# cold-deuu/Quadrotor_Manipulator_MPPI

Measured on AMD Instinct MI355X. Metric: MPPI rollouts/sec (K x H state-steps) + control-step p50 latency, K=4096 H=32, higher is better.
Workload: dtype f32

## Files before the change

quadrotor_manipulator_mppi_amd/csrc/mppi_aql.cpp:

```cpp
#include "mppi_aql.h"

#include <dlfcn.h>
#include <hip/hip_runtime.h>
#include <hsa/hsa.h>
#include <hsa/hsa_ext_amd.h>
#include <immintrin.h>
#include <stdio.h>
#include <stdlib.h>
#include <string.h>

#include <algorithm>
#include <atomic>
#include <chrono>
#include <map>
#include <mutex>
#include <unordered_map>
#include <vector>

namespace {

thread_local mppi::LaunchDesc* t_capture = nullptr;

struct Kern {
    uint64_t obj = 0;
// ... 36 lines not shown
    if (hsa_amd_memory_pool_get_info(pool, HSA_AMD_MEMORY_POOL_INFO_SEGMENT, &seg) != HSA_STATUS_SUCCESS ||
        seg != HSA_AMD_SEGMENT_GLOBAL)
        return HSA_STATUS_SUCCESS;
    if (hsa_amd_memory_pool_get_info(pool, HSA_AMD_MEMORY_POOL_INFO_GLOBAL_FLAGS, &flags) != HSA_STATUS_SUCCESS ||
        hsa_amd_memory_pool_get_info(pool, HSA_AMD_MEMORY_POOL_INFO_RUNTIME_ALLOC_ALLOWED, &alloc) != HSA_STATUS_SUCCESS ||
        !alloc)
        return HSA_STATUS_SUCCESS;
    if (hsa_amd_agent_memory_pool_get_info(pk->cpu, pool, HSA_AMD_AGENT_MEMORY_POOL_INFO_ACCESS, &acc) !=
            HSA_STATUS_SUCCESS || acc == HSA_AMD_MEMORY_POOL_ACCESS_NEVER_ALLOWED)
        return HSA_STATUS_SUCCESS;
    const int rank = (flags & HSA_AMD_MEMORY_POOL_GLOBAL_FLAG_KERNARG_INIT) ? 3
                     : (flags & HSA_AMD_MEMORY_POOL_GLOBAL_FLAG_FINE_GRAINED) ? 2 : 1;
    if (rank > pk->best_rank) { pk->best_rank = rank; pk->pool = pool; }
    return HSA_STATUS_SUCCESS;
}
std::mutex g_mu;
std::map<int, Device> g_dev;

const char* const kUnits[] = {"mppi_rollout_drone", "mppi_rollout_arm", "mppi_rollout_arm_h32", "mppi_rollout_arm32",
                              "mppi_rollout_wb",
                              "mppi_rollout_quad", "mppi_finalize"};

std::string hsa_msg(hsa_status_t s) {
    const char* m = nullptr;
    if (hsa_status_string(s, &m) != HSA_STATUS_SUCCESS || !m) return "HSA status " + std::to_string((int)s);
    return m;
}

struct AgentMatch {
    uint32_t domain, bdf;
    bool found;
    hsa_agent_t agent;
};
hsa_status_t match_agent(hsa_agent_t a, void* data) {
    auto* m = (AgentMatch*)data;
    hsa_device_type_t t;
    if (hsa_agent_get_info(a, HSA_AGENT_INFO_DEVICE, &t) != HSA_STATUS_SUCCESS || t != HSA_DEVICE_TYPE_GPU)
        return HSA_STATUS_SUCCESS;
    uint32_t bdf = 0, dom = 0;
    if (hsa_agent_get_info(a, (hsa_agent_info_t)HSA_AMD_AGENT_INFO_BDFID, &bdf) != HSA_STATUS_SUCCESS) return HSA_STATUS_SUCCESS;
    if (hsa_agent_get_info(a, (hsa_agent_info_t)HSA_AMD_AGENT_INFO_DOMAIN, &dom) != HSA_STATUS_SUCCESS) dom = 0;
    if (bdf == m->bdf && dom == m->domain && !m->found) { m->agent = a; m->found = true; }
    return HSA_STATUS_SUCCESS;
}

bool library_stem(std::string* stem) {
    Dl_info info;
    if (!dladdr((void*)&match_agent, &info) || !info.dli_fname) return false;
    std::string p = info.dli_fname;
    if (p.size() > 3 && p.compare(p.size() - 3, 3, ".so") == 0) p.resize(p.size() - 3);
    *stem = p;
    return true;
}

bool read_file(const std::string& path, std::vector<char>* out) {
    FILE* f = fopen(path.c_str(), "rb");
    if (!f) return false;
    char buf[1 << 16];
    size_t r;
    while ((r = fread(buf, 1, sizeof buf, f)) > 0) out->insert(out->end(), buf, buf + r);
    fclose(f);
    return !out->empty();
}

Device* device_for(int ordinal) {
    Device& d = g_dev[ordinal];
    if (d.tried) return &d;
    d.tried = true;
    char bus[64] = {0};
    unsigned dom = 0, b = 0, dv = 0, fn = 0;
    if (hipDeviceGetPCIBusId(bus, (int)sizeof bus, ordinal) != hipSuccess ||
        sscanf(bus, "%x:%x:%x.%x", &dom, &b, &dv, &fn) != 4) {
        d.why = "no PCI bus id for HIP device " + std::to_string(ordinal);
        return &d;
    }
    hsa_status_t st = hsa_init();
    if (st != HSA_STATUS_SUCCESS) { d.why = "hsa_init: " + hsa_msg(st); return &d; }
    AgentMatch m{dom, (b << 8) | (dv << 3) | fn, false, {}};
    hsa_iterate_agents(match_agent, &m);
    if (!m.found) { d.why = std::string("no HSA agent at ") + bus; return &d; }
    d.agent = m.agent;
    std::string stem;
    if (!library_stem(&stem)) { d.why = "cannot locate the library's own path"; return &d; }
    for (const char* u : kUnits) {
        const std::string path = stem + "." + u + ".co";
        std::vector<char> co;
        if (!read_file(path, &co)) { d.why = "missing code object " + path + " (python -m quadrotor_manipulator_mppi_amd.build)"; return &d; }
        hsa_code_object_reader_t rd;
        hsa_executable_t ex;
        if ((st = hsa_code_object_reader_create_from_memory(co.data(), co.size(), &rd)) != HSA_STATUS_SUCCESS ||
            (st = hsa_executable_create_alt(HSA_PROFILE_FULL, HSA_DEFAULT_FLOAT_ROUNDING_MODE_DEFAULT, nullptr, &ex)) !=
                HSA_STATUS_SUCCESS) {
            d.why = "loading " + path + ": " + hsa_msg(st);
            return &d;
        }
        static std::vector<std::vector<char>> keep;
        keep.push_back(std::move(co));
        if ((st = hsa_executable_load_agent_code_object(ex, d.agent, rd, nullptr, nullptr)) != HSA_STATUS_SUCCESS ||
            (st = hsa_executable_freeze(ex, nullptr)) != HSA_STATUS_SUCCESS) {
            d.why = "loading " + path + ": " + hsa_msg(st);
            return &d;
        }
        d.exes.push_back(ex);
    }
    hsa_agent_t cpu{};
    if (hsa_iterate_agents(first_cpu, &cpu) == HSA_STATUS_INFO_BREAK && !getenv("MPPI_AQL_CALL_HOSTMEM")) {
        PoolPick pk{cpu, 0, {}};
        hsa_amd_agent_iterate_memory_pools(d.agent, pick_pool, &pk);
        if (pk.best_rank > 0 &&
            hsa_agent_get_info(d.agent, (hsa_agent_info_t)HSA_AMD_AGENT_INFO_HDP_FLUSH, &d.hdp) == HSA_STATUS_SUCCESS &&
            d.hdp.HDP_MEM_FLUSH_CNTL) {
            d.vis_pool_ok = true;
            d.vis_pool = pk.pool;
            d.cpu = cpu;
            d.vis_pool_kind = pk.best_rank == 3 ? "device kernarg pool" : pk.best_rank == 2 ? "device fine-grained"
                                                                                             : "device coarse-grained";
        }
    }
    d.ok = true;
    return &d;
}

bool lookup(Device* d, const char* name, Kern* k, std::string* err) {
    std::string sym = std::string(name) + ".kd";
    auto it = d->syms.find(sym);
    if (it != d->syms.end()) { *k = it->second; return true; }
    for (hsa_executable_t ex : d->exes) {
        hsa_executable_symbol_t s;
        if (hsa_executable_get_symbol_by_name(ex, sym.c_str(), &d->agent, &s) != HSA_STATUS_SUCCESS) continue;
        Kern r;
        if (hsa_executable_symbol_get_info(s, HSA_EXECUTABLE_SYMBOL_INFO_KERNEL_OBJECT, &r.obj) != HSA_STATUS_SUCCESS ||
            hsa_executable_symbol_get_info(s, HSA_EXECUTABLE_SYMBOL_INFO_KERNEL_KERNARG_SEGMENT_SIZE, &r.kas) != HSA_STATUS_SUCCESS ||
            hsa_executable_symbol_get_info(s, HSA_EXECUTABLE_SYMBOL_INFO_KERNEL_GROUP_SEGMENT_SIZE, &r.gss) != HSA_STATUS_SUCCESS ||
            hsa_executable_symbol_get_info(s, HSA_EXECUTABLE_SYMBOL_INFO_KERNEL_PRIVATE_SEGMENT_SIZE, &r.pss) != HSA_STATUS_SUCCESS)
            break;
        d->syms[sym] = r;
        *k = r;
        return true;
    }
    *err = "kernel " + sym + " not in the code objects";
    return false;
}

}

extern "C" mppi::LaunchDesc* mppi_capture_target(void) { return t_capture; }

namespace mppi_aql {

constexpr uint32_t kQueueSize = 4096;
constexpr size_t kArgSlot = 4096;
constexpr uint32_t kCallSlots = 16;
constexpr uint32_t kBatchSlots = 4;
constexpr uint32_t kBatchBlocks = 3;

struct Step {
    Device* dev = nullptr;
    hsa_queue_t* q = nullptr;
    hsa_signal_t done{0};
    std::atomic<int> qerr{0};
    unsigned char* d_args = nullptr;
    uint32_t batch_slot = 0;
    unsigned char* h_call = nullptr;
    unsigned char* h_call_dev = nullptr;
    bool call_vis = false;
    uint32_t call_slot = 0;
    mppi::LaunchDesc fin_call{};
    Kern kc_r, kc_f;
    bool call_valid = false;
    bool call_unread = false;
    mppi::LaunchDesc roll{}, fin{};
    mppi::LaunchDesc fin_quiet{};
    Kern kr, kf, kfq;
    uint32_t step_off = 0, step_word = 0;
    bool valid = false;
    int64_t outstanding = 0;
    unsigned char* d_touch = nullptr;
    Kern kt;
    std::recursive_mutex mu;
};

void set_capture(mppi::LaunchDesc* d) { t_capture = d; }

static void queue_error(hsa_status_t status, hsa_queue_t*, void* data) {
    ((Step*)data)->qerr.store((int)status);
}

static bool probe_dispatch_ids(Step* s, std::string* why);

Step* step_create(int device, std::string* why) {
    Device* d = nullptr;
    {
        std::lock_guard<std::mutex> lk(g_mu);
        d = device_for(device);
        if (!d->ok) { *why = d->why; return nullptr; }
    }
    Step* s = new Step();
    s->dev = d;
    hsa_status_t st = hsa_queue_create(d->agent, kQueueSize, HSA_QUEUE_TYPE_SINGLE, queue_error, s, UINT32_MAX,
                                       UINT32_MAX, &s->q);
    if (st != HSA_STATUS_SUCCESS) { *why = "hsa_queue_create: " + hsa_msg(st); delete s; return nullptr; }
    if ((st = hsa_signal_create(0, 0, nullptr, &s->done)) != HSA_STATUS_SUCCESS) {
        *why = "hsa_signal_create: " + hsa_msg(st);
        hsa_queue_destroy(s->q);
        delete s;
        return nullptr;
    }
    if (d->vis_pool_ok) {
        void* p = nullptr;
        if (hsa_amd_memory_pool_allocate(d->vis_pool, kCallSlots * kArgSlot, 0, &p) == HSA_STATUS_SUCCESS) {
            if (hsa_amd_agents_allow_access(1, &d->cpu, nullptr, p) == HSA_STATUS_SUCCESS) {
                s->h_call = s->h_call_dev = (unsigned char*)p;
                s->call_vis = true;
            } else {
                hsa_amd_memory_pool_free(p);
            }
        }
    }
    if (hipMalloc(&s->d_args, (1 + kBatchBlocks * kBatchSlots) * kArgSlot) != hipSuccess ||
        (!s->call_vis &&
         (hipHostMalloc((void**)&s->h_call, kCallSlots * kArgSlot, hipHostMallocMapped | hipHostMallocCoherent) != hipSuccess ||
          hipHostGetDevicePointer((void**)&s->h_call_dev, s->h_call, 0) != hipSuccess))) {
        *why = "allocating the argument blocks failed";
        if (s->d_args) (void)hipFree(s->d_args);
        if (s->h_call) { if (s->call_vis) hsa_amd_memory_pool_free(s->h_call); else (void)hipHostFree(s->h_call); }
        hsa_signal_destroy(s->done);
        hsa_queue_destroy(s->q);
        delete s;
        return nullptr;
    }
    if (!probe_dispatch_ids(s, why)) {
        if (!step_destroy(s)) *why += " (and the probe's queue did not drain)";
        return nullptr;
    }
    {
        std::lock_guard<std::mutex> lk(g_mu);
        if (!lookup(s->dev, "k_dispatch_probe", &s->kt, why)) { (void)step_destroy(s); return nullptr; }
    }
    unsigned char h[128] = {};
    if (hipMalloc(&s->d_touch, 3 * 64) != hipSuccess) {
        s->d_touch = nullptr;
        *why = "touch buffer";
        (void)step_destroy(s);
        return nullptr;
    }
    unsigned char* outs[2] = {s->d_touch + 128, s->d_touch + 136};
    memcpy(h, &outs[0], 8);
    memcpy(h + 64, &outs[1], 8);
    if (hipMemcpy(s->d_touch, h, sizeof h, hipMemcpyHostToDevice) != hipSuccess) {
        *why = "touch upload";
        (void)step_destroy(s);
        return nullptr;
    }
    return s;
}

bool step_destroy(Step* s) {
    if (!s) return true;
    std::string e;
    if (s->outstanding && step_wait(s, 60000, &e) != 0) {
        hsa_queue_inactivate(s->q);
        fprintf(stderr, "[mppi aql] queue did not drain at destroy (%s): its buffers are leaked\n", e.c_str());
        return false;
    }
    hsa_signal_destroy(s->done);
    hsa_queue_destroy(s->q);
    (void)hipFree(s->d_args);
    if (s->d_touch) (void)hipFree(s->d_touch);
    if (s->call_vis) hsa_amd_memory_pool_free(s->h_call); else (void)hipHostFree(s->h_call);
    delete s;
    return true;
}

bool step_busy(Step* s) {
    if (!s) return false;
    std::lock_guard<std::recursive_mutex> qlk(s->mu);
    return s->outstanding > 0;
}

static bool check_launch(const mppi::LaunchDesc& l, const Kern& k, std::string* err) {
    if (k.kas < l.arg_bytes || k.kas - l.arg_bytes >= 16 || k.kas > kArgSlot) {
        *err = std::string(l.symbol) + ": kernel-argument segment " + std::to_string(k.kas) + " B vs " +
               std::to_string(l.arg_bytes) + " B packed";
        return false;
    }
    if (k.gss + l.lds > 160 * 1024) { *err = std::string(l.symbol) + ": LDS over 160 KB"; return false; }
    for (int i = 0; i < 3; ++i)
        if (l.grid[i] == 0 || l.block[i] == 0) { *err = std::string(l.symbol) + ": empty grid"; return false; }
    if ((uint64_t)l.block[0] * l.block[1] * l.block[2] > 1024) { *err = "block over 1024 threads"; return false; }
    return true;
}

static bool same_launch(const mppi::LaunchDesc& a, const mppi::LaunchDesc& b, uint32_t skip_off) {
    if (strcmp(a.symbol, b.symbol) != 0 || memcmp(a.grid, b.grid, sizeof a.grid) != 0 ||
        memcmp(a.block, b.block, sizeof a.block) != 0 || a.lds != b.lds || a.arg_bytes != b.arg_bytes)
        return false;
    if (skip_off >= a.arg_bytes || a.arg_bytes - skip_off < 4) return memcmp(a.args, b.args, a.arg_bytes) == 0;
    return memcmp(a.args, b.args, skip_off) == 0 &&
           memcmp(a.args + skip_off + 4, b.args + skip_off + 4, a.arg_bytes - skip_off - 4) == 0;
}

static unsigned char* batch_args(Step* s) { return s->d_args + (1 + kBatchBlocks * (size_t)s->batch_slot) * kArgSlot; }

int step_prepare(Step* s, const mppi::LaunchDesc& roll, const mppi::LaunchDesc& fin, const mppi::LaunchDesc& fin_quiet,
                 uint32_t step, uint32_t step_off, std::string* err) {
    std::lock_guard<std::recursive_mutex> qlk(s->mu);
    const uint32_t word = step - (uint32_t)(hsa_queue_load_write_index_relaxed(s->q) >> 1);
    if (s->valid && s->step_word == word && s->step_off == step_off && same_launch(roll, s->roll, step_off) &&
        same_launch(fin, s->fin, ~0u) && same_launch(fin_quiet, s->fin_quiet, ~0u))
        return 0;
    if (getenv("MPPI_AQL_PROFILE") && s->valid) {
        int first = -1;
        for (uint32_t i = 0; i < roll.arg_bytes && i < s->roll.arg_bytes; ++i)
            if ((i < step_off || i >= step_off + 4) && roll.args[i] != s->roll.args[i]) { first = (int)i; break; }
        int ffirst = -1;
        for (uint32_t i = 0; i < fin.arg_bytes && i < s->fin.arg_bytes; ++i)
            if (fin.args[i] != s->fin.args[i]) { ffirst = (int)i; break; }
        fprintf(stderr, "[mppi aql] re-upload: word %u vs %u, rollout args differ at %d, finalize at %d, sym %d/%d\n", word,
                s->step_word, first, ffirst, strcmp(roll.symbol, s->roll.symbol), strcmp(fin.symbol, s->fin.symbol));
    }
    Kern kr, kf, kfq;
    {
        std::lock_guard<std::mutex> lk(g_mu);
        if (!lookup(s->dev, roll.symbol, &kr, err) || !lookup(s->dev, fin.symbol, &kf, err) ||
            !lookup(s->dev, fin_quiet.symbol, &kfq, err))
            return -2;
    }
    if (!check_launch(roll, kr, err) || !check_launch(fin, kf, err) || !check_launch(fin_quiet, kfq, err)) return -2;
    if (step_off + 4 > roll.arg_bytes) { *err = "step counter outside the rollout's arguments"; return -2; }
    if (s->outstanding && step_wait(s, 60000, err) != 0) return -1;
    std::vector<unsigned char> h(kBatchBlocks * kArgSlot, 0);
    memcpy(h.data(), roll.args, roll.arg_bytes);
    memcpy(h.data() + step_off, &word, 4);
    memcpy(h.data() + kArgSlot, fin.args, fin.arg_bytes);
    memcpy(h.data() + 2 * kArgSlot, fin_quiet.args, fin_quiet.arg_bytes);
    s->batch_slot = (s->batch_slot + 1) % kBatchSlots;
    if (hipMemcpy(batch_args(s), h.data(), h.size(), hipMemcpyHostToDevice) != hipSuccess) {
        *err = "uploading the argument blocks failed";
        s->valid = false;
        return -1;
    }
    s->roll = roll;
    s->fin = fin;
    s->fin_quiet = fin_quiet;
    s->kr = kr;
    s->kf = kf;
    s->kfq = kfq;
    s->step_off = step_off;
    s->step_word = word;
    s->valid = true;
    return 0;
}

static int g_fence[4] = {-1, -1, -1, -1};
static void load_fences() {
    if (g_fence[0] >= 0) return;
    const char* f = getenv("MPPI_AQL_FENCES");
    const char* def = "0000";
    for (int i = 0; i < 4; ++i) g_fence[i] = (f && strlen(f) == 4 && f[i] >= '0' && f[i] <= '2') ? f[i] - '0' : def[i] - '0';
}
static const int kScope[3] = {HSA_FENCE_SCOPE_NONE, HSA_FENCE_SCOPE_AGENT, HSA_FENCE_SCOPE_SYSTEM};

static inline void put(hsa_queue_t* q, const Kern& k, const mppi::LaunchDesc& l, void* args, hsa_signal_t sig,
                       int acquire, int release, bool barrier = true) {
    const uint64_t idx = hsa_queue_add_write_index_relaxed(q, 1);
    while (idx - hsa_queue_load_read_index_scacquire(q) >= q->size) _mm_pause();
    auto* p = (hsa_kernel_dispatch_packet_t*)q->base_address + (idx & (q->size - 1));
    p->workgroup_size_x = (uint16_t)l.block[0];
    p->workgroup_size_y = (uint16_t)l.block[1];
    p->workgroup_size_z = (uint16_t)l.block[2];
    p->reserved0 = 0;
    p->grid_size_x = l.grid[0] * l.block[0];
    p->grid_size_y = l.grid[1] * l.block[1];
    p->grid_size_z = l.grid[2] * l.block[2];
    p->private_segment_size = k.pss;
    p->group_segment_size = k.gss + l.lds;
    p->kernel_object = k.obj;
    p->kernarg_address = args;
    p->reserved2 = 0;
    p->completion_signal = sig;
    const uint16_t header =
        (uint16_t)((HSA_PACKET_TYPE_KERNEL_DISPATCH << HSA_PACKET_HEADER_TYPE) | ((barrier ? 1 : 0) << HSA_PACKET_HEADER_BARRIER) |
                   (kScope[acquire] << HSA_PACKET_HEADER_SCACQUIRE_FENCE_SCOPE) |
                   (kScope[release] << HSA_PACKET_HEADER_SCRELEASE_FENCE_SCOPE));
    const uint32_t setup = 3u << HSA_KERNEL_DISPATCH_PACKET_SETUP_DIMENSIONS;
    __atomic_store_n((uint32_t*)p, (uint32_t)header | (setup << 16), __ATOMIC_RELEASE);
}

static bool probe_dispatch_ids(Step* s, std::string* why) {
    Kern k;
    {
        std::lock_guard<std::mutex> lk(g_mu);
        if (!lookup(s->dev, "k_dispatch_probe", &k, why)) return false;
    }
    unsigned long long* d_ids = nullptr;
    if (hipMalloc(&d_ids, 2 * sizeof(unsigned long long)) != hipSuccess) { *why = "probe buffer"; return false; }
    unsigned long long* args[2] = {d_ids, d_ids + 1};
    std::vector<unsigned char> h(2 * kArgSlot, 0);
    memcpy(h.data(), &args[0], 8);
    memcpy(h.data() + kArgSlot, &args[1], 8);
    bool ok = hipMemset(d_ids, 0xFF, 2 * sizeof(unsigned long long)) == hipSuccess &&
              hipMemcpy(s->d_args + kArgSlot, h.data(), h.size(), hipMemcpyHostToDevice) == hipSuccess;
    if (!ok) { (void)hipFree(d_ids); *why = "probe upload"; return false; }
    mppi::LaunchDesc l{};
    snprintf(l.symbol, sizeof l.symbol, "k_dispatch_probe");
    l.grid[0] = l.grid[1] = l.grid[2] = 1;
    l.block[0] = 64; l.block[1] = l.block[2] = 1;
    l.arg_bytes = 8;
    uint64_t idx[2];
    hsa_signal_add_relaxed(s->done, 1);
    ++s->outstanding;
    for (int i = 0; i < 2; ++i) {
        idx[i] = hsa_queue_load_write_index_relaxed(s->q);
        put(s->q, k, l, s->d_args + (1 + i) * kArgSlot, i == 1 ? s->done : hsa_signal_t{0}, 2, i == 1 ? 2 : 0);
    }
    hsa_signal_store_screlease(s->q->doorbell_signal, (hsa_signal_value_t)idx[1]);
    std::string err;
    unsigned long long got[2] = {~0ull, ~0ull};
    if (step_wait(s, 10000, &err) != 0) {
        char b[160];
        snprintf(b, sizeof b, " [signal %ld, read index %llu, write index %llu]", (long)hsa_signal_load_relaxed(s->done),
                 (unsigned long long)hsa_queue_load_read_index_relaxed(s->q),
                 (unsigned long long)hsa_queue_load_write_index_relaxed(s->q));
        *why = "dispatch-id probe: " + err + b;
        return false;
    }
    ok = hipMemcpy(got, d_ids, sizeof got, hipMemcpyDeviceToHost) == hipSuccess;
    (void)hipFree(d_ids);
    if (!ok) { *why = "dispatch-id probe readback"; return false; }
    if (const char* sk = getenv("MPPI_AQL_PROBE_SKEW")) {
        got[0] += (unsigned long long)atoll(sk);
        got[1] += (unsigned long long)atoll(sk);
    }
    if (got[0] != idx[0] || got[1] != idx[1]) {
        char b[256];
        snprintf(b, sizeof b, "the queue's dispatch ids (%llu, %llu) are not its packet indices (%llu, %llu): "
                 "intercepted by a tool", got[0], got[1], (unsigned long long)idx[0], (unsigned long long)idx[1]);
        *why = b;
        return false;
    }
    return true;
}

std::unique_lock<std::recursive_mutex> step_guard(Step* s) { return std::unique_lock<std::recursive_mutex>(s->mu); }

int step_dispatch(Step* s, int n, std::string* err, bool overlap) {
    std::lock_guard<std::recursive_mutex> qlk(s->mu);
    if (!s->valid) { *err = "step_dispatch before step_prepare"; return -1; }
    if (n <= 0) return 0;
    if (s->qerr.load()) { *err = "native queue error: " + hsa_msg((hsa_status_t)s->qerr.load()); return -1; }
    hsa_signal_add_relaxed(s->done, 1);
    ++s->outstanding;
    const hsa_signal_t none{0};
    void* ra = batch_args(s);
    void* fa = batch_args(s) + kArgSlot;
    void* fqa = batch_args(s) + 2 * kArgSlot;
    load_fences();
    for (int i = 0; i < n; ++i) {
        const bool last = i == n - 1;
        put(s->q, s->kr, s->roll, ra, none, i == 0 ? std::max(1, g_fence[0]) : g_fence[0], g_fence[1],
            !(overlap && i > 0));
        if (last) put(s->q, s->kf, s->fin, fa, s->done, g_fence[2], 2);
        else put(s->q, s->kfq, s->fin_quiet, fqa, none, g_fence[2], g_fence[3]);
        hsa_signal_store_screlease(s->q->doorbell_signal, (hsa_signal_value_t)hsa_queue_load_write_index_relaxed(s->q) - 1);
    }
    return 0;
}

int step_call(Step* s, const mppi::LaunchDesc& roll, const mppi::LaunchDesc& fin, uint32_t step,
              uint32_t step_off, uint32_t seq_off, uint32_t* seq, std::string* err) {
    std::lock_guard<std::recursive_mutex> qlk(s->mu);
    if (s->qerr.load()) { *err = "native queue error: " + hsa_msg((hsa_status_t)s->qerr.load()); return -1; }
    static const bool prof = getenv("MPPI_AQL_PROFILE") != nullptr;
    static double pacc[4] = {0, 0, 0, 0};
    static long pcn = 0;
    auto now = [] { return std::chrono::steady_clock::now(); };
    const auto p0 = now();
    Kern kr, kf;
    {
        std::lock_guard<std::mutex> lk(g_mu);
        if (!lookup(s->dev, roll.symbol, &kr, err) || !lookup(s->dev, fin.symbol, &kf, err)) return -2;
    }
    if (!check_launch(roll, kr, err) || !check_launch(fin, kf, err)) return -2;
    if (step_off + 4 > roll.arg_bytes || seq_off + 4 > roll.arg_bytes) { *err = "call words outside the arguments"; return -2; }
    if (s->call_unread && s->outstanding && step_wait(s, 60000, err) != 0) return -1;
    if (!s->call_valid || !same_launch(fin, s->fin_call, ~0u)) {
        if (s->outstanding && step_wait(s, 60000, err) != 0) return -1;
        std::vector<unsigned char> h(kArgSlot, 0);
        memcpy(h.data(), fin.args, fin.arg_bytes);
        if (hipMemcpy(s->d_args, h.data(), kArgSlot, hipMemcpyHostToDevice) != hipSuccess) {
            *err = "uploading the call's finalize arguments failed";
            s->call_valid = false;
            return -1;
        }
        s->fin_call = fin;
        s->call_valid = true;
    }
    s->kc_r = kr;
    s->kc_f = kf;
    const uint64_t r = hsa_queue_load_write_index_relaxed(s->q);
    const uint32_t word = step - (uint32_t)(r >> 1);
    *seq = 0x80000000u | (uint32_t)(r >> 1);
    const uint32_t slot = s->call_slot++ % kCallSlots;
    unsigned char* blk = s->h_call + (size_t)slot * kArgSlot;
    alignas(16) unsigned char tmp[kArgSlot];
    memcpy(tmp, roll.args, roll.arg_bytes);
    memcpy(tmp + step_off, &word, 4);
    memcpy(tmp + seq_off, seq, 4);
    const uint32_t nb = (roll.arg_bytes + 63) & ~63u;
    memset(tmp + roll.arg_bytes, 0, nb - roll.arg_bytes);
    const auto p1 = now();
    memcpy(blk, tmp, nb);
    const auto p2 = now();
    if (s->call_vis) {
        _mm_sfence();
        volatile uint32_t* f = s->dev->hdp.HDP_MEM_FLUSH_CNTL;
        *f = 1u;
        (void)*f;
    }
    std::atomic_thread_fence(std::memory_order_release);
    const auto p3 = now();
    hsa_signal_add_relaxed(s->done, 1);
    ++s->outstanding;
    s->call_unread = true;
    const hsa_signal_t none{0};
    load_fences();
    put(s->q, kr, roll, s->h_call_dev + (size_t)slot * kArgSlot, none, std::max(1, g_fence[0]), g_fence[1]);
    put(s->q, kf, fin, s->d_args, s->done, g_fence[2], 2);
    hsa_signal_store_screlease(s->q->doorbell_signal, (hsa_signal_value_t)hsa_queue_load_write_index_relaxed(s->q) - 1);
    if (prof) {
        const auto p4 = now();
        pacc[0] += std::chrono::duration<double, std::micro>(p1 - p0).count();
        pacc[1] += std::chrono::duration<double, std::micro>(p2 - p1).count();
        pacc[2] += std::chrono::duration<double, std::micro>(p3 - p2).count();
        pacc[3] += std::chrono::duration<double, std::micro>(p4 - p3).count();
        if (++pcn % 1000 == 0)
            fprintf(stderr, "[mppi aql] step_call (us): lookups+checks %.2f  block write %.2f  flush+readback %.2f  packets %.2f\n",
                    pacc[0] / pcn, pacc[1] / pcn, pacc[2] / pcn, pacc[3] / pcn);
    }
    return 0;
}

int step_touch(Step* s, bool if_free, std::string* err) {
    std::unique_lock<std::recursive_mutex> qlk(s->mu, std::defer_lock);
    if (if_free) {
        if (!qlk.try_lock()) return 1;
    } else {
        qlk.lock();
    }
    if (s->qerr.load()) { *err = "native queue error: " + hsa_msg((hsa_status_t)s->qerr.load()); return -1; }
    mppi::LaunchDesc l{};
    l.grid[0] = l.grid[1] = l.grid[2] = 1;
    l.block[0] = 64; l.block[1] = l.block[2] = 1;
    l.arg_bytes = 8;
    hsa_signal_add_relaxed(s->done, 1);
    ++s->outstanding;
    put(s->q, s->kt, l, s->d_touch, hsa_signal_t{0}, 1, 0);
    put(s->q, s->kt, l, s->d_touch + 64, s->done, 0, 0);
    hsa_signal_store_screlease(s->q->doorbell_signal, (hsa_signal_value_t)hsa_queue_load_write_index_relaxed(s->q) - 1);
    return 0;
}

void step_ring(Step* s) {
    const uint64_t w = hsa_queue_load_write_index_relaxed(s->q);
    if (w) hsa_signal_store_screlease(s->q->doorbell_signal, (hsa_signal_value_t)(w - 1));
}

int step_error(Step* s) { return s ? s->qerr.load() : 0; }

const char* step_call_memory(Step* s) {
    return !s ? "" : s->call_vis ? s->dev->vis_pool_kind.c_str() : "pinned host memory";
}

void step_call_read(Step* s) {
    if (!s) return;
    std::lock_guard<std::recursive_mutex> qlk(s->mu);
    s->call_unread = false;
}

int step_wait(Step* s, int timeout_ms, std::string* err) {
    if (!s) return 0;
    std::lock_guard<std::recursive_mutex> qlk(s->mu);
    if (!s->outstanding) return 0;
    const auto t0 = std::chrono::steady_clock::now();
    for (;;) {
        if (hsa_signal_load_scacquire(s->done) == 0) break;
        if (s->qerr.load()) {
            *err = "native queue error: " + hsa_msg((hsa_status_t)s->qerr.load());
            return -1;
        }
        if (std::chrono::steady_clock::now() - t0 > std::chrono::milliseconds(timeout_ms)) {
            *err = "native dispatch: no completion after " + std::to_string(timeout_ms) + " ms";
            return -1;
        }
        _mm_pause();
    }
    s->outstanding = 0;
    s->call_unread = false;
    return 0;
}

}
```

quadrotor_manipulator_mppi_amd/csrc/mppi_aql.h:

```cpp
#pragma once
#include <stdint.h>

#include <mutex>
#include <string>

#include "mppi_dev.h"

namespace mppi_aql {

struct Step;

Step* step_create(int device, std::string* why);
bool step_destroy(Step* s);

int step_prepare(Step* s, const mppi::LaunchDesc& roll, const mppi::LaunchDesc& fin, const mppi::LaunchDesc& fin_quiet,
                 uint32_t step, uint32_t step_off, std::string* err);
int step_dispatch(Step* s, int n, std::string* err, bool overlap = false);
std::unique_lock<std::recursive_mutex> step_guard(Step* s);
int step_call(Step* s, const mppi::LaunchDesc& roll, const mppi::LaunchDesc& fin, uint32_t step,
              uint32_t step_off, uint32_t seq_off, uint32_t* seq, std::string* err);
void step_call_read(Step* s);
const char* step_call_memory(Step* s);
int step_touch(Step* s, bool if_free, std::string* err);
void step_ring(Step* s);
int step_error(Step* s);
int step_wait(Step* s, int timeout_ms, std::string* err);
bool step_busy(Step* s);

void set_capture(mppi::LaunchDesc* d);

}
```

quadrotor_manipulator_mppi_amd/csrc/mppi_dev.h:

```cpp
#pragma once
#include <stddef.h>
#include <stdint.h>

#include "../../include/mppi_hip.h"

namespace mppi {

constexpr int kMaxA = MPPI_MAX_ACTION;
constexpr int kMaxJ = MPPI_MAX_JOINTS;
constexpr int kMaxW = MPPI_MAX_SAVGOL;
constexpr int kHdr = 4;
constexpr int kMaxCostRun = 4096;
constexpr inline int cost_run_stride(int nS) { return (nS + 3) & ~3; }

struct JointDev {
    int32_t type;
    int32_t q_index;
    int32_t axis_z;
    int32_t _pad;
    float O[12];
    float ax[3];
    float axx[9];
};

struct VehicleConst {
    double pos0[kMaxA];
    double vel0[kMaxA];
    float pos0f[kMaxA];
    float vel0f[kMaxA];
    float base[12];
    float tpos[3];
    float tR[9];
    float _pad[4];
    float qc[kMaxJ];
    float qlo[kMaxJ];
    float qhi[kMaxJ];
};
static_assert(sizeof(VehicleConst) % 16 == 0, "VehicleConst must be a 16-byte multiple");

struct KinOrigin { int p[3]; int s[3]; int tmask; };
constexpr KinOrigin kKinova[7] = {
    {{0, 1, 2}, {-1, 1, -1}, 4},
    {{0, 2, 1}, {-1, -1, -1}, 6},
    {{0, 2, 1}, {1, -1, 1}, 2},
    {{0, 2, 1}, {-1, 1, 1}, 4},
    {{0, 2, 1}, {-1, -1, -1}, 6},
    {{0, 2, 1}, {-1, 1, 1}, 4},
    {{0, 2, 1}, {-1, -1, -1}, 2},
};

struct DevParams {
    int32_t model, V, K, H, A;
    int32_t L;
    int32_t R;
    int32_t nch;
    int32_t nb;
    int32_t iters;
    int32_t nq;
    int32_t qoff;
    int32_t nj;
    int32_t noise_mode, state_f64, store_traj, store_noise;
    int32_t sigma_diag;
    int32_t j0;
    int32_t chain_fast;
    int32_t P;
    int32_t C;
    int32_t hp;
    uint32_t seed_lo, seed_hi;
    int64_t k_offset;
    float dt, dt2;
    double dt_d;
    float coef;
    float w_sp, w_so, w_tp, w_to;
    float sdiag[kMaxA];
    VehicleConst vc0;
    const JointDev* joints;
    const float* sigma;
    const VehicleConst* vc;
    const float* u_prev;
    const float* noise_in;
    uint32_t step_ctr;
    float* traj;
    float* noise_out;
    float* S;
    float* hdr;
    float* rdata;
    unsigned long long* stamps;
    int32_t cost_terms;
    float w_cov;
    float w_cen, w_jt, w_act, lim_pen;
    const float* sinv;
    const float* gamma_t;
    const float* jtraj;
    float q_inv_m;
    float q_iinv[3];
    float q_kd;
    float q_g;
    int32_t q_literal_jinv;
    const uint32_t* ovl;
    int32_t ovl_n;
    int32_t kern;
};
constexpr int kStamps = 16;

struct FinTail {
    float coef, dt, dt2;
    int32_t mode, model, qoff, nq, state_f64, out_dim, window;
    float* u_prev;
    const VehicleConst* vc;
    double* out;
    float* u0;
    float* stats;
    uint32_t* flags;
    float* wraw;
    float* wsmooth;
    float* dst;
    float* xbase;
    int64_t xslot;
    int32_t nslots, myslot, P, pad_;
    unsigned long long* const* xpeers;
    unsigned long long* xlocal;
    int32_t xn, xme;
    uint32_t* xerr;
    uint32_t* xstall;
    uint32_t* xovl;
    unsigned long long* xdec;
    float sg[kMaxW];
};
enum { kTailFinal = 0, kTailPack = 1, kTailScratch = 2, kTailReadback = 3, kTailSlots = 4 };

constexpr int kMaxPeers = 8;
constexpr int kXW = kHdr + 64;
constexpr int kXCtl = 16;
constexpr uint32_t kDecCommit = 1u;
constexpr uint64_t kDecGraceTicks = 10000ull;
constexpr int kVcStepWord = (int)(offsetof(VehicleConst, _pad) / 4) + 1;
constexpr int kVcEpochWord = kVcStepWord + 1;
constexpr uint32_t kTagValid = 0x80000000u;
constexpr inline uint32_t peer_tag(uint32_t step, uint32_t epoch) {
    return kTagValid | ((epoch & 0x3FFu) << 20) | (step & 0xFFFFFu);
}
constexpr uint64_t kPeerWaitTicks = 200000000ull;
constexpr uint32_t kSeqFromVc = 0xFFFFFFFFu;

struct LaunchDesc {
    char symbol[192];
    uint32_t grid[3];
    uint32_t block[3];
    uint32_t lds;
    uint32_t arg_bytes;
    alignas(16) unsigned char args[2048];
};

constexpr int32_t kFinKernGeneric = 1, kFinKernQuiet = 2;

struct FinParams {
    int32_t model, V, H, A, nq, qoff, state_f64;
    int32_t nrec;
    int32_t ts, tsz;
    const float* hdr;
    int64_t hdr_vs, hdr_rs;
    const float* dat;
    int64_t d_vs, d_as, d_rs;
    int32_t P;
    int32_t mode;
    int32_t window, half;
    float coef, dt, dt2;
    double dt_d;
    float sg[kMaxW];
    float* dst;
    float* xbase;
    int64_t xslot;
    int32_t nslots, myslot;
    unsigned long long* const* xpeers;
    unsigned long long* xlocal;
    int32_t xn, xme;
    uint32_t* xerr;
    uint32_t* xstall;
    uint32_t* xovl;
    unsigned long long* xdec;
    float* u_prev;
    const VehicleConst* vc;
    double* out;
    float* u0;
    float* stats;
    uint32_t* flags;
    uint32_t seq;
    float* wraw;
    float* wsmooth;
    int32_t out_dim;
    int32_t dbg;
    int32_t kern;
    unsigned long long* stamps;
    const FinTail* tail;
};

}

extern "C" {
int mppi_launch_rollout(const mppi::DevParams* p, int block_threads, void* stream);
int mppi_launch_rollout_arm64(const mppi::DevParams* p, int block_threads, void* stream);
int mppi_launch_rollout_arm64_h32(const mppi::DevParams* p, int block_threads, void* stream);
int mppi_launch_rollout_arm32(const mppi::DevParams* p, int block_threads, void* stream);
int mppi_launch_rollout_wb(const mppi::DevParams* p, int block_threads, void* stream);
int mppi_launch_rollout_quad(const mppi::DevParams* p, int block_threads, void* stream);
int mppi_launch_finalize(const mppi::FinParams* p, void* stream);
int mppi_launch_peer_probe(unsigned long long* const* peers, unsigned long long* local, int n, int me,
                           unsigned long long slot_words, uint32_t tag, unsigned long long ticks,
                           unsigned long long* out, void* stream);
int mppi_launch_weights(const float* S, const float* stats, float* w, int V, int K, float coef,
                        void* stream);
int mppi_launch_philox(uint64_t seed, uint32_t step, int vehicle, int64_t k0, int K, int H, int A,
                       float* z, uint32_t* raw, void* stream);
mppi::LaunchDesc* mppi_capture_target(void);
}
```

quadrotor_manipulator_mppi_amd/csrc/mppi_engine.cpp:

```cpp
#include <algorithm>
#include <cmath>
#include <cstdio>
#include <cstdlib>
#include <cstring>
#include <vector>

#include "mppi_engine.h"

using namespace mppi;

namespace mppi_host {

FinTail tail_of(const FinParams& f, int32_t mode) {
    FinTail t;
    std::memset(&t, 0, sizeof(t));
    t.coef = f.coef; t.dt = f.dt; t.dt2 = f.dt2;
    t.mode = mode; t.model = f.model; t.qoff = f.qoff; t.nq = f.nq; t.state_f64 = f.state_f64;
    t.out_dim = f.out_dim; t.window = f.window;
    t.u_prev = f.u_prev; t.vc = f.vc;
    t.out = f.out; t.u0 = f.u0; t.stats = f.stats; t.flags = f.flags; t.wraw = f.wraw; t.wsmooth = f.wsmooth;
    t.dst = f.dst; t.xbase = f.xbase; t.xslot = f.xslot; t.nslots = f.nslots; t.myslot = f.myslot; t.P = f.P;
    t.xpeers = f.xpeers; t.xlocal = f.xlocal; t.xn = f.xn; t.xme = f.xme; t.xerr = f.xerr;
    t.xstall = f.xstall; t.xovl = f.xovl; t.xdec = f.xdec;
    std::memcpy(t.sg, f.sg, sizeof(t.sg));
// ... 247 lines not shown
    CREATE_TRY(hipEventCreateWithFlags(&e->ev_vc, hipEventDisableTiming));
    CREATE_TRY(hipEventCreateWithFlags(&e->ev_out, hipEventDisableTiming));
    const size_t KH = (size_t)e->V * e->K * H;
    CREATE_TRY(hipMalloc(&e->d_joints, sizeof(JointDev) * kMaxJ));
    CREATE_TRY(hipMalloc(&e->d_vc, sizeof(VehicleConst) * e->V));
    CREATE_TRY(hipMalloc(&e->d_u_prev, sizeof(float) * e->V * H * e->A));
    CREATE_TRY(hipMalloc(&e->d_S, sizeof(float) * e->V * e->K));
    CREATE_TRY(hipMalloc(&e->d_w, sizeof(float) * e->V * e->K));
    CREATE_TRY(hipMalloc(&e->d_hdr, sizeof(float) * (size_t)e->V * nb * 4));
    CREATE_TRY(hipMalloc(&e->d_rdata, sizeof(float) * (size_t)e->V * e->A * nb * H));
    CREATE_TRY(hipMalloc(&e->d_wraw, sizeof(float) * e->V * H * e->A));
    CREATE_TRY(hipMalloc(&e->d_wsmooth, sizeof(float) * e->V * H * e->A));
    if (c.store_trajectory) CREATE_TRY(hipMalloc(&e->d_traj, sizeof(float) * traj_floats(e)));
    if (c.store_noise) CREATE_TRY(hipMalloc(&e->d_noise_out, sizeof(float) * KH * e->A));
    e->out_bytes = (int64_t)(off_xerr(e) + 16);
    CREATE_TRY(hipMalloc(&e->d_out, e->out_bytes));
    CREATE_TRY(hipHostMalloc((void**)&e->h_out, e->out_bytes, hipHostMallocMapped | hipHostMallocCoherent));
    CREATE_TRY(hipHostGetDevicePointer((void**)&e->h_out_dev, e->h_out, 0));
    std::memset(e->h_out, 0, e->out_bytes);
    CREATE_TRY(hipMalloc(&e->d_sigma, sizeof(float) * kMaxA * kMaxA));
    CREATE_TRY(hipMemcpy(e->d_sigma, c.sigma, sizeof(float) * e->A * e->A, hipMemcpyHostToDevice));
    if (c.cost_terms) {
        std::vector<double> m(e->A * 2 * e->A, 0.0);
        const int A = e->A, W2 = 2 * A;
        for (int i = 0; i < A; ++i) {
            for (int j = 0; j < A; ++j) m[i * W2 + j] = c.sigma[i * A + j];
            m[i * W2 + A + i] = 1.0;
        }
        for (int col = 0; col < A; ++col) {
            int piv = col;
            for (int r = col + 1; r < A; ++r)
                if (std::fabs(m[r * W2 + col]) > std::fabs(m[piv * W2 + col])) piv = r;
            if (std::fabs(m[piv * W2 + col]) < 1e-30) { mppi_destroy(e); return fail(MPPI_ERR_INVALID_ARG, "Sigma is singular"); }
            for (int j = 0; j < W2; ++j) std::swap(m[col * W2 + j], m[piv * W2 + j]);
            const double d = m[col * W2 + col];
            for (int j = 0; j < W2; ++j) m[col * W2 + j] /= d;
            for (int r = 0; r < A; ++r)
                if (r != col) {
                    const double f2 = m[r * W2 + col];
                    for (int j = 0; j < W2; ++j) m[r * W2 + j] -= f2 * m[col * W2 + j];
                }
        }
        std::vector<float> sinv(A * A), gam(H);
        for (int i = 0; i < A; ++i)
            for (int j = 0; j < A; ++j) sinv[i * A + j] = (float)m[i * W2 + A + j];
        for (int t = 0; t < H; ++t) gam[t] = std::pow(c.cost_gamma, (float)t);
        CREATE_TRY(hipMalloc(&e->d_sinv, sizeof(float) * A * A));
        CREATE_TRY(hipMalloc(&e->d_gamma, sizeof(float) * H));
        CREATE_TRY(hipMalloc(&e->d_jtraj, sizeof(float) * (size_t)e->V * H * std::max(1, e->nq)));
        CREATE_TRY(hipMemcpy(e->d_sinv, sinv.data(), sizeof(float) * A * A, hipMemcpyHostToDevice));
        CREATE_TRY(hipMemcpy(e->d_gamma, gam.data(), sizeof(float) * H, hipMemcpyHostToDevice));
        CREATE_TRY(hipMemset(e->d_jtraj, 0, sizeof(float) * (size_t)e->V * H * std::max(1, e->nq)));
    }
    CREATE_TRY(hipHostMalloc((void**)&e->h_vc, sizeof(VehicleConst) * e->V, hipHostMallocDefault));
    CREATE_TRY(hipMemsetAsync(e->d_u_prev, 0, sizeof(float) * e->V * H * e->A, e->stream));
    CREATE_TRY(hipMemsetAsync(e->d_out, 0, e->out_bytes, e->stream));

    std::vector<JointDev> jd(kMaxJ);
    for (int j = 0; j < c.n_joints; ++j) bake_joint(c.joints[j], jd[j]);
    const float I12[12] = {1, 0, 0, 0, 0, 1, 0, 0, 0, 0, 1, 0};
    std::memcpy(e->fixedM, I12, sizeof(I12));
    int j0 = 0;
    while (c.model != MPPI_MODEL_DRONE && j0 < c.n_joints && jd[j0].type == MPPI_JOINT_FIXED) {
        mul34(e->fixedM, jd[j0].O, e->fixedM);
        ++j0;
    }
    CREATE_TRY(hipMemcpy(e->d_joints, jd.data(), sizeof(JointDev) * kMaxJ, hipMemcpyHostToDevice));
    CREATE_TRY(hipStreamSynchronize(e->stream));
#undef CREATE_TRY

    DevParams& p = e->dp;
    std::memset(&p, 0, sizeof(p));
    p.model = c.model; p.V = e->V; p.K = e->K; p.H = H; p.A = e->A;
    p.L = L; p.R = R; p.nch = nch; p.nb = nb; p.iters = iters;
    p.nq = e->nq; p.qoff = e->qoff; p.nj = c.n_joints;
    p.noise_mode = c.noise_mode | (c.vehicle_offset << 16); p.state_f64 = c.state_f64;
    p.store_traj = c.store_trajectory; p.store_noise = c.store_noise;
    bool diag = true;
    for (int a = 0; a < e->A; ++a)
        for (int b = 0; b < e->A; ++b) {
            if (a == b) p.sdiag[a] = c.sigma[a * e->A + b];
            else if (c.sigma[a * e->A + b] != 0.0f) diag = false;
        }
    p.sigma_diag = diag;
    p.sigma = e->d_sigma;
    p.j0 = j0;
    {
        bool fast = c.model != MPPI_MODEL_DRONE && (c.n_joints - j0) == e->nq;
        for (int j = j0; fast && j < c.n_joints; ++j)
            fast = jd[j].type == MPPI_JOINT_REVOLUTE && jd[j].axis_z && jd[j].q_index == j - j0;
        p.chain_fast = fast;
        if (fast && e->nq == 7 && c.n_joints - j0 == 7) {
            bool kin = true;
            for (int j = 0; kin && j < 7; ++j) {
                const float* O = jd[j0 + j].O;
                const KinOrigin& k = kKinova[j];
                for (int col = 0; kin && col < 3; ++col)
                    for (int row = 0; kin && row < 3; ++row) {
                        const float want = (row == k.p[col]) ? (float)k.s[col] : 0.0f;
                        kin = std::fabs(O[4 * row + col] - want) <= 1e-6f;
                    }
                for (int d = 0; kin && d < 3; ++d) kin = ((k.tmask >> d) & 1) ? true : (O[4 * d + 3] == 0.0f);
            }
            if (kin && !getenv("MPPI_NO_KINOVA_PATH")) p.chain_fast = 2;
        }
    }
    p.P = P; p.C = e->C; p.hp = traj_pitch(e);
    p.seed_lo = (uint32_t)c.seed; p.seed_hi = (uint32_t)(c.seed >> 32);
    p.k_offset = (int64_t)c.shard_rank * e->K;
    p.dt = (float)c.dt; p.dt2 = (float)(c.dt * c.dt); p.dt_d = c.dt;
    p.coef = (float)(-1.0 / c.lambda_);
    p.w_sp = c.w_stage_pos; p.w_so = c.w_stage_ori; p.w_tp = c.w_term_pos; p.w_to = c.w_term_ori;
    p.joints = e->d_joints;
    p.cost_terms = c.cost_terms;
    p.w_cov = (float)((double)c.w_covar * (c.lambda_ * (1.0 - (double)c.cost_alpha)));
    p.w_cen = c.w_center; p.w_jt = c.w_joint_track; p.w_act = c.w_action; p.lim_pen = c.joint_limit_penalty;
    p.sinv = e->d_sinv; p.gamma_t = e->d_gamma; p.jtraj = e->d_jtraj;
    p.q_inv_m = (float)(1.0 / (double)c.quad_mass);
    for (int d = 0; d < 3; ++d) p.q_iinv[d] = (float)(1.0 / (double)c.quad_inertia[d]);
    p.q_kd = c.quad_kd; p.q_g = c.quad_gravity; p.q_literal_jinv = c.quad_literal_jinv ? 1 : 0;
    p.vc = e->d_vc; p.u_prev = e->d_u_prev;
    p.traj = e->d_traj; p.noise_out = e->d_noise_out; p.S = e->d_S; p.hdr = e->d_hdr; p.rdata = e->d_rdata;
#ifdef MPPI_STAMPS
    if (getenv("MPPI_STAMPS")) {
        const size_t nwaves = (size_t)e->V * nb * (e->threads / 64);
        if (hipMalloc(&e->d_stamps, nwaves * kStamps * 8) == hipSuccess) p.stamps = e->d_stamps;
        e->stamp_sum.assign(kStamps, 0.0);
        (void)hipMalloc(&e->d_fstamps, 2 * (size_t)e->V * e->A * ((H + 7) / 8) * kStamps * 8);
        e->fstamp_sum.assign(kStamps, 0.0);
    }
#endif

    FinParams& f = e->fp;
    std::memset(&f, 0, sizeof(f));
    f.model = c.model; f.V = e->V; f.H = H; f.A = e->A; f.nq = e->nq; f.qoff = e->qoff;
    f.state_f64 = c.state_f64; f.P = P;
    if (const char* z = getenv("MPPI_FIN_TSZ")) {
        const int tz = atoi(z);
        if (tz >= 1 && tz + 2 * (c.savgol_window / 2) <= 64) e->fin_tsz = tz;
    }
    f.tsz = e->fin_tsz; f.ts = e->fin_ts = (H + e->fin_tsz - 1) / e->fin_tsz;
    f.window = c.savgol_window; f.half = c.savgol_window / 2;
    for (int j = 0; j < c.savgol_window; ++j) f.sg[j] = e->sg_taps[c.savgol_window - 1 - j];
    f.coef = p.coef; f.dt = p.dt; f.dt2 = p.dt2; f.dt_d = c.dt;
    f.u_prev = e->d_u_prev; f.vc = e->d_vc;
    f.out = (double*)e->h_out_dev;
    f.u0 = (float*)(e->h_out_dev + off_u0(e));
    f.stats = (float*)(e->h_out_dev + off_stats(e));
    f.flags = (uint32_t*)(e->h_out_dev + off_flags(e));
    f.xerr = (uint32_t*)(e->h_out_dev + off_xerr(e));
    f.wraw = e->d_wraw; f.wsmooth = e->d_wsmooth; f.out_dim = e->out_dim;
    if (const char* dbg = getenv("MPPI_FIN_DEBUG")) f.dbg = atoi(dbg);
    if (const char* g = getenv("MPPI_GENERIC_KERNELS"))
        e->generic = !strcmp(g, "finalize") ? 1 : !strcmp(g, "quiet") ? 2 : !strcmp(g, "rollout") ? 4 : atoi(g) != 0 ? 7 : 0;
    f.kern = (e->generic & 1) ? kFinKernGeneric : 0;
    p.kern = (e->generic & 4) ? 1 : 0;
    e->event_wait = getenv("MPPI_EVENT_WAIT") && atoi(getenv("MPPI_EVENT_WAIT")) != 0;
    e->no_flag_dbg = e->event_wait && getenv("MPPI_DEBUG_NO_FLAG") && atoi(getenv("MPPI_DEBUG_NO_FLAG")) != 0;
    e->out_dbg = getenv("MPPI_DEBUG_OUT") ? atoi(getenv("MPPI_DEBUG_OUT")) : 0;
    if (const char* d = getenv("MPPI_DISPATCH")) e->aql_mode = !strcmp(d, "hip") ? 0 : !strcmp(d, "aql") ? 1 : 2;
    f.stamps = e->d_fstamps;
    e->overlap = getenv("MPPI_OVERLAP") && atoi(getenv("MPPI_OVERLAP")) != 0 && c.model != MPPI_MODEL_QUADROTOR;
    if (e->overlap) {
        const size_t n = (size_t)e->V * e->A * e->fin_ts;
        if (hipMalloc(&e->d_ovl, n * sizeof(uint32_t)) != hipSuccess || hipMemset(e->d_ovl, 0, n * sizeof(uint32_t)) != hipSuccess) {
            fail(MPPI_ERR_HIP, "overlap counters");
            mppi_destroy(e);
            return MPPI_ERR_HIP;
        }
        f.xovl = e->d_ovl;
        p.ovl = e->d_ovl;
        p.ovl_n = e->A * e->fin_ts;
    }
    {
        FinTail t[kTailSlots];
        t[kTailFinal] = tail_of(f, 0);
        t[kTailPack] = tail_of(f, 1);
        t[kTailScratch] = tail_of(f, 0);
        t[kTailScratch].out = (double*)e->d_out;
        t[kTailScratch].u0 = (float*)(e->d_out + off_u0(e));
        t[kTailScratch].stats = (float*)(e->d_out + off_stats(e));
        t[kTailScratch].flags = (uint32_t*)(e->d_out + off_flags(e));
        t[kTailScratch].xerr = (uint32_t*)(e->d_out + off_xerr(e));
        t[kTailScratch].wraw = nullptr;
        t[kTailScratch].wsmooth = nullptr;
        t[kTailFinal].wraw = nullptr;
        t[kTailFinal].wsmooth = nullptr;
        t[kTailReadback] = tail_of(f, 2);
        hipError_t te = hipMalloc(&e->d_tail, sizeof(t));
        if (te == hipSuccess) te = hipMemcpy(e->d_tail, t, sizeof(t), hipMemcpyHostToDevice);
        if (te != hipSuccess) {
            fail(MPPI_ERR_HIP, "finalize tail parameters: %s", hipGetErrorString(te));
            mppi_destroy(e);
            return MPPI_ERR_HIP;
        }
        f.tail = e->d_tail + kTailFinal;
    }
    *out = e;
    return MPPI_OK;
}

void mppi_destroy(mppi_engine* e) {
    if (!e) return;
    prewarm_stop(e);
    (void)hipSetDevice(e->cfg.device);
    if (e->aql && !mppi_aql::step_destroy(e->aql)) {
        fprintf(stderr, "[mppi] mppi_destroy: the engine's native queue did not drain; its device buffers are leaked\n");
        return;
    }
    e->aql = nullptr;
    if (e->d_stamps && e->stamp_n) {
        fprintf(stderr, "[mppi stamps] rollout avg cycles per wave over %lld waves:", (long long)e->stamp_n);
        for (size_t i = 1; i < kRollStampOrder.size(); ++i)
            fprintf(stderr, " %s=%.0f", kRollStampNames[i], e->stamp_sum[i] / e->stamp_n);
        fprintf(stderr, "\n[mppi stamps] finalize avg cycles per block over %lld blocks:", (long long)e->fstamp_n);
        for (size_t i = 1; i < kFinStampOrder.size(); ++i)
            fprintf(stderr, " %s=%.0f", kFinStampNames[i], e->fstamp_sum[i] / std::max<int64_t>(1, e->fstamp_n));
        fprintf(stderr, "\n");
    }
    if (e->stream) (void)hipStreamSynchronize(e->stream);
    for (auto& pr : e->roll_pairs) { (void)hipEventDestroy(pr.first); (void)hipEventDestroy(pr.second); }
    for (auto& pr : e->fin_pairs) { (void)hipEventDestroy(pr.first); (void)hipEventDestroy(pr.second); }
    for (auto ev : e->ev_pool) (void)hipEventDestroy(ev);
    exchange_release(e);
    void* dev[] = {e->d_xregion, e->d_xpeers, e->d_sigma, e->d_joints, e->d_vc, e->d_u_prev, e->d_noise_in, e->d_traj, e->d_noise_out,
                   e->d_S, e->d_hdr, e->d_rdata, e->d_out, e->d_wraw, e->d_wsmooth, e->d_w,
                   e->d_sinv, e->d_gamma, e->d_jtraj, e->d_xown, e->d_tail, e->d_stamps, e->d_fstamps, e->d_xstall, e->d_ovl, e->d_xdec};
    for (void* p : dev) if (p) (void)hipFree(p);
    if (e->h_out) (void)hipHostFree(e->h_out);
    if (e->h_vc) (void)hipHostFree(e->h_vc);
    if (e->ev_vc) (void)hipEventDestroy(e->ev_vc);
    if (e->ev_out) (void)hipEventDestroy(e->ev_out);
    if (e->own_stream) (void)hipStreamDestroy(e->own_stream);
    delete e;
}

mppi_status mppi_set_stream(mppi_engine* e, void* s) {
    if (!e) return fail(MPPI_ERR_INVALID_ARG, "null engine");
    if (use_device(e)) return MPPI_ERR_HIP;
    HIP_TRY(hipStreamSynchronize(e->stream));
    e->stream = s ? (hipStream_t)s : e->own_stream;
    return MPPI_OK;
}

mppi_status mppi_set_joint_trajectory(mppi_engine* e, int32_t v, const float* traj) {
    if (!e || v < 0 || v >= e->V) return fail(MPPI_ERR_INVALID_ARG, "mppi_set_joint_trajectory: bad arguments");
    if (!e->d_jtraj) return fail(MPPI_ERR_STATE, "engine created without cost_terms");
    if (use_device(e)) return MPPI_ERR_HIP;
    const size_t n = (size_t)e->H * e->nq;
    float* dst = e->d_jtraj + (size_t)v * n;
    if (traj) HIP_TRY(hipMemcpyAsync(dst, traj, n * sizeof(float), hipMemcpyHostToDevice, e->stream));
    else HIP_TRY(hipMemsetAsync(dst, 0, n * sizeof(float), e->stream));
    HIP_TRY(hipStreamSynchronize(e->stream));
    return MPPI_OK;
}

mppi_status mppi_set_target(mppi_engine* e, int32_t v, const float* pos, const float* quat) {
    if (!e || !pos || v < 0 || v >= e->V) return fail(MPPI_ERR_INVALID_ARG, "mppi_set_target: bad arguments");
    std::memcpy(&e->tpos[3 * v], pos, 3 * sizeof(float));
    if (quat) std::memcpy(&e->tquat[4 * v], quat, 4 * sizeof(float));
    if (e->state_set) {
        if (use_device(e)) return MPPI_ERR_HIP;
        return upload_consts(e);
    }
    return MPPI_OK;
}

mppi_status mppi_set_u_prev(mppi_engine* e, const float* u) {
    if (!e || !u) return fail(MPPI_ERR_INVALID_ARG, "null argument");
    if (use_device(e)) return MPPI_ERR_HIP;
    HIP_TRY(hipMemcpyAsync(e->d_u_prev, u, sizeof(float) * e->V * e->H * e->A, hipMemcpyHostToDevice, e->stream));
    HIP_TRY(hipStreamSynchronize(e->stream));
    return MPPI_OK;
}

mppi_status mppi_get_u_prev(mppi_engine* e, float* u) {
    if (!e || !u) return fail(MPPI_ERR_INVALID_ARG, "null argument");
    if (use_device(e)) return MPPI_ERR_HIP;
    HIP_TRY(hipMemcpyAsync(u, e->d_u_prev, sizeof(float) * e->V * e->H * e->A, hipMemcpyDeviceToHost, e->stream));
    HIP_TRY(hipStreamSynchronize(e->stream));
    return MPPI_OK;
}

mppi_status mppi_set_state(mppi_engine* e, const double* state) {
    if (!e || !state) return fail(MPPI_ERR_INVALID_ARG, "null argument");
    if (use_device(e)) return MPPI_ERR_HIP;
    std::memcpy(e->state.data(), state, sizeof(double) * e->state.size());
    e->state_set = true;
    return upload_consts(e);
}

mppi_status mppi_set_step_counter(mppi_engine* e, uint32_t step) {
    if (!e) return fail(MPPI_ERR_INVALID_ARG, "null engine");
    if (use_device(e)) return MPPI_ERR_HIP;
    e->step_ctr = step;
    if (e->peer) {
        ++e->x_epoch;
        return build_vehicle_consts(e);
    }
    return MPPI_OK;
}

mppi_status mppi_get_step_counter(mppi_engine* e, uint32_t* step) {
    if (!e || !step) return fail(MPPI_ERR_INVALID_ARG, "null argument");
    *step = e->step_ctr;
    return MPPI_OK;
}

mppi_status mppi_kernel_timing_ex(mppi_engine* e, int32_t n, double* rollout_us, double* finalize_us,
// ... 222 lines not shown
```

quadrotor_manipulator_mppi_amd/csrc/mppi_engine.h:

```cpp
#pragma once
#include <hip/hip_runtime.h>
#include <rccl/rccl.h>

#include <atomic>
#include <condition_variable>
#include <mutex>
#include <string>
#include <thread>
#include <utility>
#include <vector>

#include "mppi_aql.h"
#include "mppi_dev.h"

struct mppi_engine {
    mppi_config cfg;
    int K, H, A, V, nq, qoff, state_dim, out_dim, C, threads;
    int64_t out_bytes;
    mppi::DevParams dp;
    mppi::FinParams fp;
    float sg_taps[mppi::kMaxW];
    float fixedM[12];
    hipStream_t own_stream = nullptr, stream = nullptr;
    float* d_sigma = nullptr;
    mppi::JointDev* d_joints = nullptr;
    mppi::VehicleConst* d_vc = nullptr;
    float* d_u_prev = nullptr;
    float* d_noise_in = nullptr;
    uint32_t step_ctr = 0;
    uint32_t out_seq = 0;
    bool call_cached = false;
    int call_threads = 0;
    mppi::DevParams call_p{};
    mppi::FinParams call_f{};
    mppi::LaunchDesc call_roll{}, call_fin{};
    bool batch_cached = false;
    int batch_threads = 0;
    mppi::DevParams batch_p{};
    mppi::FinParams batch_f{};
    mppi::LaunchDesc batch_roll{}, batch_fin{};
    mppi::LaunchDesc batch_fin_quiet{};
    int generic = 0;
    std::string kern_batch = "none", kern_call = "none";
    int kern_batch_state = 0;
    bool kern_call_hip = false, kern_call_peer = false;
    std::vector<double> rec_out;
    std::vector<float> rec_u0, rec_stats;
    std::vector<float> fk_O, fk_ax;
    uint32_t seq_ctr = 0;
    bool event_wait = false;
    bool no_flag_dbg = false;
    int out_dbg = 0;
    float* d_traj = nullptr;
    float* d_noise_out = nullptr;
    float* d_S = nullptr;
    float* d_hdr = nullptr;
    float* d_rdata = nullptr;
    int fin_ts = 1, fin_tsz = 8;
    unsigned char* d_out = nullptr;
    mppi::FinTail* d_tail = nullptr;
    float* d_wraw = nullptr;
    float* d_wsmooth = nullptr;
    float* d_w = nullptr;
    float* d_sinv = nullptr;
    float* d_gamma = nullptr;
    float* d_jtraj = nullptr;
    float* d_exchange = nullptr;
    ncclComm_t comm = nullptr;
    float* d_xown = nullptr;
    bool peer = false;
    int x_connected = 0;
    unsigned long long* d_xregion = nullptr;
    size_t x_bytes = 0;
    std::vector<void*> x_opened;
    unsigned long long** d_xpeers = nullptr;
    uint32_t x_epoch = 0;
    uint32_t* d_xstall = nullptr;
    unsigned long long* d_xdec = nullptr;
    bool overlap = false;
    uint32_t* d_ovl = nullptr;
    mppi::VehicleConst* h_vc = nullptr;
    unsigned char* h_out = nullptr;
    unsigned char* h_out_dev = nullptr;
    hipEvent_t ev_vc = nullptr, ev_out = nullptr;
    bool vc_pending = false, state_set = false, out_pending = false;
    std::vector<float> tpos, tquat;
    std::vector<double> state;
    bool timing = false;
    std::vector<hipEvent_t> ev_pool;
    std::vector<std::pair<hipEvent_t, hipEvent_t>> roll_pairs, fin_pairs;
    double roll_ms = 0.0, fin_ms = 0.0;
    unsigned long long* d_stamps = nullptr;
    unsigned long long* d_fstamps = nullptr;
    std::vector<double> fstamp_sum;
    int64_t fstamp_n = 0;
    std::vector<double> stamp_sum;
    int64_t stamp_n = 0;
    double clk_sum = 0.0;
    int64_t roll_n = 0, fin_n = 0;
    mppi_aql::Step* aql = nullptr;
    int aql_mode = 2;
    bool aql_tried = false;
    bool aql_off = false;
    std::string aql_why = "no mppi_run_steps yet";
    bool aql_out = false;
    bool aql_call = false;
    bool calls_native = false;
    double call_wait_us = 0.0;
    std::thread pw_thr;
    std::mutex pw_mu;
    std::condition_variable pw_cv;
    std::atomic<int32_t> pw_us{0};
    std::atomic<bool> pw_stop{false};
    std::atomic<int64_t> pw_touches{0};
    std::atomic<int64_t> call_t[8];
    std::atomic<int64_t> call_n{0};
    bool pw_spin = false;
    std::atomic<bool> pw_native{false};
};

namespace mppi_host {

mppi_status fail(mppi_status st, const char* fmt, ...) __attribute__((format(printf, 2, 3)));

#define HIP_TRY(expr)                                                                              \
    do {                                                                                           \
        hipError_t _e = (expr);                                                                    \
        if (_e != hipSuccess)                                                                      \
            return ::mppi_host::fail(MPPI_ERR_HIP, "%s failed: %s (%s:%d)", #expr,                \
                                     hipGetErrorString(_e), __FILE__, __LINE__);                   \
    } while (0)

int nq_of(const mppi_config& c);
mppi_status validate(const mppi_config& c);
void rpy_to_R(float r, float p, float y, float* R);
void joint_origin(const mppi_joint& j, float* T16);
void unit_axis(const mppi_joint& j, float* a);
void base_from_xyzquat(const double* b, bool f64, float* T16);
void quat_xyzw_to_R(const float* q, float* R);
void euler_zyx(const float* m, float* ypr);
int savgol_taps(int window, int order, float* c);
void bake_joint(const mppi_joint& j, mppi::JointDev& d);
void mul34(const float* A, const float* B, float* C);
void fk_consts(const mppi_joint* joints, int nj, float* O16s, float* axes);
void host_fk_c(const mppi_joint* joints, int nj, const float* O16s, const float* axes, const double* q,
               const double* xyzquat, bool f64, float* out16);
void host_fk(const mppi_joint* joints, int nj, const double* q, const double* xyzquat, bool f64, float* out16);

inline bool sharded(const mppi_engine* e) { return (e->cfg.shard_count > 1 || e->comm) && !e->peer; }
mppi::FinTail tail_of(const mppi::FinParams& f, int32_t mode);
void pack_fields(const mppi_engine* e, mppi::FinParams& f);
mppi_status upload_pack_tail(mppi_engine* e);
int traj_pitch(const mppi_engine* e);
size_t traj_floats(const mppi_engine* e);
mppi_status aql_join(mppi_engine* e);
mppi_status use_device(mppi_engine* e);
mppi_status build_vehicle_consts(mppi_engine* e);
void quad_outputs(const mppi_engine* e, const double* s, const float* u0, double* out);
mppi_status upload_consts(mppi_engine* e);
hipEvent_t pool_event(mppi_engine* e);
mppi_status drain_timing(mppi_engine* e);

inline size_t off_u0(const mppi_engine* e) { return ((size_t)e->V * e->out_dim * sizeof(double) + 15) & ~size_t(15); }
inline size_t off_stats(const mppi_engine* e) {
    return (off_u0(e) + (size_t)e->V * e->A * sizeof(float) + 15) & ~size_t(15);
}
inline size_t off_flags(const mppi_engine* e) { return off_stats(e) + (size_t)e->V * 16; }
inline size_t rec_count(const mppi_engine* e) { return (size_t)e->V * (2 * e->A + 1); }
inline size_t off_xerr(const mppi_engine* e) { return off_flags(e) + rec_count(e) * 16; }
inline uint32_t sticky_timeout(const mppi_engine* e) {
    return e->h_out ? *(const volatile uint32_t*)(e->h_out + off_xerr(e)) : 0u;
}
inline unsigned long long* xdata(const mppi_engine* e) { return e->d_xregion + mppi::kXCtl; }

void block_records(const mppi_engine* e, mppi::FinParams& f);
void final_records(const mppi_engine* e, mppi::FinParams& f);

struct Rccl {
    bool ok = false;
    std::string why;
    ncclResult_t (*get_unique_id)(ncclUniqueId*) = nullptr;
    ncclResult_t (*init_rank)(ncclComm_t*, int, ncclUniqueId, int) = nullptr;
    ncclResult_t (*all_reduce)(const void*, void*, size_t, ncclDataType_t, ncclRedOp_t, ncclComm_t,
                               hipStream_t) = nullptr;
    ncclResult_t (*destroy)(ncclComm_t) = nullptr;
    const char* (*err)(ncclResult_t) = nullptr;
    ncclResult_t (*init_rank_config)(ncclComm_t*, int, ncclUniqueId, int, ncclConfig_t*) = nullptr;
    ncclResult_t (*async_error)(ncclComm_t, ncclResult_t*) = nullptr;
    ncclResult_t (*abort)(ncclComm_t) = nullptr;
    ncclResult_t (*count)(const ncclComm_t, int*) = nullptr;
    ncclResult_t (*user_rank)(const ncclComm_t, int*) = nullptr;
};
const Rccl& rccl();
void exchange_release(mppi_engine* e);
// ... 15 lines not shown
```

quadrotor_manipulator_mppi_amd/csrc/mppi_rollout.h:

```cpp
#pragma once
#include "mppi_device.h"

#ifndef MPPI_KO
#define MPPI_KO 0
#endif
#ifndef MPPI_ROLL_OCC_NCH2
#define MPPI_ROLL_OCC_NCH2 4
#endif
#ifndef MPPI_ROLL_OCC_NCH2_XC
#define MPPI_ROLL_OCC_NCH2_XC 2
#endif
#ifndef MPPI_ROLL_OCC_XC
#define MPPI_ROLL_OCC_XC 4
#endif
#ifndef MPPI_ROLL_OCC
#define MPPI_ROLL_OCC 4
#endif
#ifndef MPPI_PRIO
#define MPPI_PRIO 1
#endif
#ifndef MPPI_S_PLAIN
#define MPPI_S_PLAIN 0
#endif
#ifndef MPPI_EPS_STASH
// ... 320 lines not shown
#define STAMP(i) do { } while (0)
#define STAMPW(i) do { } while (0)
#define STAMPRT(i) do { } while (0)
#endif

#ifdef MPPI_SECTIONS
#define SECTION(name)                                        \
    do {                                                     \
        __builtin_amdgcn_sched_barrier(0);                   \
        asm volatile("; MPPI_SECTION " name ::: "memory");   \
        __builtin_amdgcn_sched_barrier(0);                   \
    } while (0)
#else
#define SECTION(name) do { } while (0)
#endif

template <int L>
__device__ __forceinline__ float seg_scan_f32(float x) {
    x += __int_as_float(__builtin_amdgcn_update_dpp(0, __float_as_int(x), 0x111, 0xF, 0xF, true));
    x += __int_as_float(__builtin_amdgcn_update_dpp(0, __float_as_int(x), 0x112, 0xF, 0xF, true));
    x += __int_as_float(__builtin_amdgcn_update_dpp(0, __float_as_int(x), 0x114, 0xF, 0xF, true));
    x += __int_as_float(__builtin_amdgcn_update_dpp(0, __float_as_int(x), 0x118, 0xF, 0xF, true));
    if (L >= 32) x += dpp_f32<0x142, 0xA>(x);
    if (L >= 64) x += dpp_f32<0x143, 0xC>(x);
    return x;
}


#ifndef MPPI_TRAJ_AUX
#define MPPI_TRAJ_AUX 18
#endif
__device__ __forceinline__ __amdgpu_buffer_rsrc_t traj_rsrc(float* planes_v, uint32_t plane_b, int C) {
    return __builtin_amdgcn_make_buffer_rsrc(planes_v, 0, (int)(plane_b * (uint32_t)C), 0x00020000);
}
__device__ __forceinline__ void traj_store(__amdgpu_buffer_rsrc_t rs, uint32_t voff, uint32_t soff, float x) {
    if (MPPI_KO & 16) return;
    __builtin_amdgcn_raw_buffer_store_b32(__float_as_uint(x), rs, (int)voff, (int)soff, MPPI_TRAJ_AUX);
}
#ifndef MPPI_REC_AUX
#define MPPI_REC_AUX 16
#endif
__device__ __forceinline__ void wt_store(float* base_uniform, uint32_t byte_off, float x) {
    const __amdgpu_buffer_rsrc_t rs = __builtin_amdgcn_make_buffer_rsrc(base_uniform, 0, (int)0xFFFFFFFFu, 0x00020000);
    __builtin_amdgcn_raw_buffer_store_b32(__float_as_uint(x), rs, (int)byte_off, 0, MPPI_REC_AUX);
}
__device__ __forceinline__ void wt_store4(float* base_uniform, uint32_t byte_off, float4 x) {
    const __amdgpu_buffer_rsrc_t rs = __builtin_amdgcn_make_buffer_rsrc(base_uniform, 0, (int)0xFFFFFFFFu, 0x00020000);
    typedef uint32_t u32x4 __attribute__((ext_vector_type(4)));
    const u32x4 v = {__float_as_uint(x.x), __float_as_uint(x.y), __float_as_uint(x.z), __float_as_uint(x.w)};
    __builtin_amdgcn_raw_buffer_store_b128(v, rs, (int)byte_off, 0, MPPI_REC_AUX);
}
__device__ __forceinline__ void drain_stores() {
    if (!(MPPI_KO & 512)) asm volatile("s_waitcnt vmcnt(0)" ::: "memory");
}

template <int L, int NA>
__device__ __forceinline__ void seg_scan_f32_multi(float (&x)[NA]) {
    if (MPPI_KO & 1) return;
#define MPPI_SCAN_STEP(CTRL, RM, BC)                                                    \
    _Pragma("unroll") for (int a = 0; a < NA; ++a) x[a] += __int_as_float(             \
        __builtin_amdgcn_update_dpp(0, __float_as_int(x[a]), CTRL, RM, 0xF, BC));
    MPPI_SCAN_STEP(0x111, 0xF, true)
    MPPI_SCAN_STEP(0x112, 0xF, true)
    MPPI_SCAN_STEP(0x114, 0xF, true)
    MPPI_SCAN_STEP(0x118, 0xF, true)
#undef MPPI_SCAN_STEP
    if (L >= 32) {
#pragma unroll
        for (int a = 0; a < NA; ++a)
            asm volatile("s_nop 1\n\tv_add_f32_dpp %0, %0, %0 row_bcast:15 row_mask:0xa bank_mask:0xf" : "+v"(x[a]));
    }
    if (L >= 64) {
#pragma unroll
        for (int a = 0; a < NA; ++a)
            asm volatile("s_nop 1\n\tv_add_f32_dpp %0, %0, %0 row_bcast:31 row_mask:0xc bank_mask:0xf" : "+v"(x[a]));
    }
}

template <int R>
__device__ __forceinline__ float seg_pick(float x, int sub, int l_in_seg, int L) {
    float r = read_lane_f32(x, l_in_seg);
#pragma unroll
    for (int s = 1; s < R; ++s) r = (sub == s) ? read_lane_f32(x, s * L + l_in_seg) : r;
    return r;
}

template <int L, int NA>
struct IntegGeom {
    static constexpr int R = 64 / L;
    static constexpr int S = R * NA;
    static constexpr int CPS = (S <= 4) ? 16 : (S <= 8) ? 8 : (S <= 16) ? 4 : (S <= 32) ? 2 : 1;
    static constexpr int CL = L / CPS;
    static constexpr int P = NA | 1;
    static_assert(S * CPS <= 64 && CPS <= L, "integrator lane map");
};

template <int NA, int NCH, int L>
constexpr int wave_slot_floats() {
    return (NCH == 1 && 64 * IntegGeom<L, NA>::P > 4 + NCH * 64 * NA) ? 64 * IntegGeom<L, NA>::P
                                                                     : 4 + NCH * 64 * NA;
}

template <int CTRL>
__device__ __forceinline__ float row_shr_f32(float x) {
    return __int_as_float(__builtin_amdgcn_update_dpp(0, __float_as_int(x), CTRL, 0xF, 0xF, true));
}

template <int L, int NA>
__device__ __forceinline__ void integrate_lds(const float (&act)[NA], float* xw, const int lane, const float dt,
                                              const float dt2h, const float* vel0f, float (&inc)[NA]) {
    using G = IntegGeom<L, NA>;
    constexpr int P = G::P, CPS = G::CPS, CL = G::CL, S = G::S;
#pragma unroll
    for (int a = 0; a < NA; ++a) xw[lane * P + a] = act[a];
    wave_lds_handoff();
    const int sr = lane / CPS, ch = lane & (CPS - 1);
    const bool on = sr < S;
    const int seg = sr / NA, a = sr - seg * NA;
    const int rb = on ? (seg * L + ch * CL) * P + a : 0;
    float lv = 0.0f, lp = 0.0f, loc[CL];
#pragma unroll
    for (int i = 0; i < CL; ++i) {
        const float x = xw[rb + i * P];
        lp += fmaf(lv, dt, x * dt2h);
        lv = fmaf(x, dt, lv);
        loc[i] = lp;
    }
    float V = lv, Q = lp;
#define MPPI_ISCAN(D, CTRL)                                                                if (CPS > D) {                                                                             const float vs = row_shr_f32<CTRL>(V), qs = row_shr_f32<CTRL>(Q);                       if (ch >= D) { Q = Q + fmaf((float)(D * CL) * dt, vs, qs); V = V + vs; }            }
    MPPI_ISCAN(1, 0x111)
    MPPI_ISCAN(2, 0x112)
    MPPI_ISCAN(4, 0x114)
    MPPI_ISCAN(8, 0x118)
#undef MPPI_ISCAN
    float Vx = row_shr_f32<0x111>(V), Qx = row_shr_f32<0x111>(Q);
    if (ch == 0) { Vx = 0.0f; Qx = 0.0f; }
    const float v0 = on ? vel0f[a] : 0.0f;
    const float q0 = fmaf((float)(ch * CL) * dt, v0, Qx);
    const float vb = dt * (Vx + v0);
    wave_lds_handoff();
    if (on) {
#pragma unroll
        for (int i = 0; i < CL; ++i) xw[rb + i * P] = fmaf((float)(i + 1), vb, q0 + loc[i]);
    }
    wave_lds_handoff();
#pragma unroll
    for (int a2 = 0; a2 < NA; ++a2) inc[a2] = xw[lane * P + a2];
}

template <int NCH, bool F64, bool XC, bool ONEG>
constexpr int roll_occ() {
    return (ONEG && !F64) ? 8 : (NCH >= 4 ? 2 : NCH == 2 ? (XC ? MPPI_ROLL_OCC_NCH2_XC : MPPI_ROLL_OCC_NCH2) : (XC ? MPPI_ROLL_OCC_XC : MPPI_ROLL_OCC));
}
template <int MODEL, int NA, int NCH, int LSEG, bool F64, bool VONE, bool XC, bool ONEG, bool B512>
__device__ __forceinline__ void rollout_body(const uint32_t seed_lo, const uint32_t seed_hi,
                                             const uint32_t step_arg, const uint32_t k_off,
                                             const int32_t noise_arg, const int32_t H_arg,
                                             const int32_t geo_arg,
                                             const float* __restrict__ u_prev,
                                             const JointDev* __restrict__ jtab, const DevParams& pk) {
    static_assert(!B512 || ONEG, "the fixed-block body is a single-group one");
    constexpr int R = 64 / LSEG;
    constexpr int QOFF = (MODEL == MPPI_MODEL_WHOLEBODY) ? 3 : 0;
    constexpr int NQ = (MODEL == MPPI_MODEL_DRONE) ? 0 : NA - QOFF;
    constexpr int kJW = (int)(sizeof(JointDev) * kMaxJ / 4);
    extern __shared__ __attribute__((aligned(16))) float smem[];
    __shared__ JointDev jnt[kMaxJ];
    __shared__ VehicleConst vcv;
    const DevParams& p = pk;
    const int v = blockIdx.y;
    const int nthr = B512 ? 512 : (geo_arg & 0xFFFF), iters = ONEG ? 1 : (geo_arg >> 16);
    const int tid = threadIdx.x, lane = tid & 63, wid = tid >> 6, nw = nthr >> 6;
    const int sub = lane / LSEG, t0 = lane & (LSEG - 1);
    const int32_t noise_mode = noise_arg & 0xFF;
    const uint32_t step_ctr = step_of(step_arg, noise_arg);
    const uint32_t vkey = (uint32_t)v + ((uint32_t)noise_arg >> 16);
    STAMPRT(13);
    STAMP(0);
    float* u_lds = smem;
    const int HA = H_arg * NA;
    const float* usrc = u_prev + (size_t)v * HA;
    constexpr int NU = B512 ? (LSEG * NCH * NA + 511) / 512 : 4, NJ = B512 ? (kJW + 511) / 512 : 2;
    float ur[NU];
    int jr[NJ];
    const bool ovl = !B512 && (noise_arg & kNoiseOverlap) != 0;
    auto load_u = [&]() __attribute__((always_inline)) {
        const __amdgpu_buffer_rsrc_t urs = __builtin_amdgcn_make_buffer_rsrc(
            const_cast<float*>(usrc), 0, (MPPI_KO & 128) ? 0 : HA * 4, 0x00020000);
#pragma unroll
        for (int j = 0; j < NU; ++j)
            ur[j] = __uint_as_float(__builtin_amdgcn_raw_buffer_load_b32(urs, (tid + j * nthr) * 4, 0, kAuxDev));
    };
    if (!ovl) load_u();
    if (MODEL != MPPI_MODEL_DRONE) {
        const int* js = (const int*)jtab;
#pragma unroll
        for (int j = 0; j < NJ; ++j) {
            const int i = tid + j * nthr;
            jr[j] = (i < kJW) ? js[i] : 0;
        }
    }
    constexpr int kVCW = (int)(sizeof(VehicleConst) / 4);
    const int vcr = (tid < kVCW) ? (VONE ? ((const int*)&pk.vc0)[tid] : ((const int*)(pk.vc + v))[tid]) : 0;
    uint32_t kwarm = 0u;
    {
        const uint32_t* kp = (const uint32_t*)&pk;
#pragma unroll
        for (int o = 0; o < (int)(offsetof(DevParams, sigma) / 4); o += 16) kwarm ^= kp[o];
    }
    STAMPW(9);
    float z0[NCH][NA];
    SECTION("prologue_philox");
    if (noise_mode != MPPI_NOISE_INJECTED) {
        const uint32_t kg = k_off + (uint32_t)((blockIdx.x * nw + wid) * R + sub);
#pragma unroll
        for (int c = 0; c < NCH; ++c)
            draw_normals<NA>(z0[c], kg, (uint32_t)(t0 + 64 * c), vkey, step_ctr, seed_lo, seed_hi);
    }
    if (ovl) {
        if (wid == 0) {
            const uint32_t* fl = pk.ovl + (size_t)v * pk.ovl_n;
            const int nfl = pk.ovl_n;
            for (;;) {
                bool ok = true;
                for (int i = lane; i < nfl; i += 64) ok &= (int32_t)(ld_dev(fl + i) - step_ctr) >= 0;
                if (__builtin_amdgcn_ballot_w64(!ok) == 0ull) break;
                __builtin_amdgcn_s_sleep(1);
            }
        }
        lds_barrier();
        load_u();
    }
    SECTION("prologue_staging");
    STAMP(10);
    asm volatile("" :: "s"(kwarm));
#pragma unroll
    for (int j = 0; j < NU; ++j) {
        const int i = tid + j * nthr;
        if (i < HA) u_lds[i] = ur[j];
    }
    if constexpr (!B512)
        for (int i = tid + 4 * nthr; i < HA; i += nthr) u_lds[i] = usrc[i];
    if (MODEL != MPPI_MODEL_DRONE) {
#pragma unroll
        for (int j = 0; j < NJ; ++j) {
            const int i = tid + j * nthr;
            if (i < kJW) ((int*)jnt)[i] = jr[j];
        }
        if constexpr (!B512)
            for (int i = tid + 2 * nthr; i < kJW; i += nthr) ((int*)jnt)[i] = ((const int*)jtab)[i];
    }
    if (tid < kVCW) {
        ((int*)&vcv)[tid] = vcr;
        if (VONE && blockIdx.x == 0)
            __hip_atomic_store((int*)pk.vc + tid, tid == kVcStepWord ? (int)step_ctr : vcr, __ATOMIC_RELAXED,
                               __HIP_MEMORY_SCOPE_AGENT);
    }
    if constexpr (!B512) {
        for (int i = tid + nthr; i < kVCW; i += nthr) {
            const int x = VONE ? ((const int*)&pk.vc0)[i] : ((const int*)(pk.vc + v))[i];
            ((int*)&vcv)[i] = x;
            if (VONE && blockIdx.x == 0)
                __hip_atomic_store((int*)pk.vc + i, i == kVcStepWord ? (int)step_ctr : x, __ATOMIC_RELAXED,
                                   __HIP_MEMORY_SCOPE_AGENT);
        }
    }
    STAMPW(8);
    if (!(MPPI_KO & 256)) lds_barrier();
    const VehicleConst& vc = vcv;
    const float* sdiag = pk.sdiag;
    const int H = H_arg, K = pk.K;
    constexpr int kWs = wave_slot_floats<NA, NCH, LSEG>();
    float* const xw = smem + ((HA + 3) & ~3) + wid * kWs;
    float* const s_stage = smem + ((HA + 3) & ~3) + 8 * kWs;
    STAMP(1);

    const int hp = pk.hp;
    const uint32_t plane_b = (uint32_t)K * (uint32_t)hp * 4u;
    const __amdgpu_buffer_rsrc_t trs = traj_rsrc(pk.traj + (size_t)v * pk.C * K * hp, plane_b, pk.C);

    float acc[NCH][NA];
#pragma unroll
    for (int c = 0; c < NCH; ++c)
#pragma unroll
        for (int a = 0; a < NA; ++a) acc[c][a] = 0.0f;
    float rho_w = INFINITY, eta_w = 0.0f, eta2_w = 0.0f;
    bool nan_w = false;

    auto group = [&](const int it) __attribute__((always_inline)) {
        asm volatile("" ::: "memory");
        SECTION("noise");
        const int g = blockIdx.x + it * p.nb;
        const int k = (g * nw + wid) * R + sub;
        const bool kval = k < K;
        const int kc = kval ? k : K - 1;
        const uint32_t kg = k_off + (uint32_t)k;

        float eps[NCH][NA], act[NCH][NA];
#pragma unroll
        for (int c = 0; c < NCH; ++c) {
            const int t = t0 + 64 * c;
            const bool val = kval && t < H;
            const int tc = (t < H) ? t : H - 1;
            if (noise_mode == MPPI_NOISE_INJECTED) {
                const float* src = p.noise_in + (((size_t)v * K + kc) * H + tc) * NA;
#pragma unroll
                for (int a = 0; a < NA; ++a) eps[c][a] = src[a];
            } else {
                float z[NA];
                if (it == 0) {
#pragma unroll
                    for (int a = 0; a < NA; ++a) z[a] = z0[c][a];
                } else {
                    draw_normals<NA>(z, kg, (uint32_t)t, vkey, step_ctr, seed_lo, seed_hi);
                }
                if (!XC || p.sigma_diag) {
#pragma unroll
                    for (int a = 0; a < NA; ++a) eps[c][a] = z[a] * sdiag[a];
                } else {
#pragma unroll
                    for (int b = 0; b < NA; ++b) {
                        float e = 0.0f;
#pragma unroll
                        for (int a = 0; a < NA; ++a) e += z[a] * p.sigma[a * NA + b];
                        eps[c][b] = e;
                    }
                }
            }
            float ur[NA];
#pragma unroll
            for (int a = 0; a < NA; ++a) ur[a] = u_lds[tc * NA + a];
#pragma unroll
            for (int a = 0; a < NA; ++a) {
                eps[c][a] = val ? eps[c][a] : 0.0f;
                act[c][a] = val ? ur[a] + eps[c][a] : 0.0f;
            }
            if (p.store_noise && val) {
                float* dst = p.noise_out + (((size_t)v * K + k) * H + t) * NA;
#pragma unroll
                for (int a = 0; a < NA; ++a) st_dev(dst + a, eps[c][a]);
            }
        }
        float ecov = 0.0f, eact = 0.0f, gts[NCH];
#pragma unroll
        for (int c = 0; c < NCH; ++c) gts[c] = 0.0f;
        if (XC && p.cost_terms) {
#pragma unroll
            for (int c = 0; c < NCH; ++c) {
                const int t = t0 + 64 * c;
                const bool val = kval && t < H;
                const int tc = (t < H) ? t : H - 1;
                gts[c] = val ? p.gamma_t[tc] : 0.0f;
                if (p.cost_terms & MPPI_COST_COVAR) {
                    float qd = 0.0f;
#pragma unroll
                    for (int a = 0; a < NA; ++a) {
                        float y = 0.0f;
                        if (p.sigma_diag) {
                            y = p.sinv[a * NA + a] * act[c][a];
                        } else {
#pragma unroll
                            for (int b = 0; b < NA; ++b) y = fmaf(p.sinv[a * NA + b], act[c][b], y);
                        }
                        qd = fmaf(u_lds[tc * NA + a], y, qd);
                    }
                    ecov += val ? qd : 0.0f;
                }
                if (p.cost_terms & MPPI_COST_ACTION) {
                    float s2 = 0.0f;
#pragma unroll
                    for (int a = 0; a < NA; ++a) s2 = fmaf(act[c][a], act[c][a], s2);
                    eact += val ? (p.w_act * s2) * gts[c] : 0.0f;
                }
            }
        }
        if (it == 0) STAMP(2);
        SECTION("integrator");

        float posf[NCH][NA];
        double posd[NCH][F64 ? NA : 1];
        if constexpr (NCH == 1 && !(MPPI_KO & 1)) {
            float inc[NA];
            integrate_lds<LSEG, NA>(act[0], xw, lane, p.dt, 0.5f * p.dt2, vc.vel0f, inc);
#pragma unroll
            for (int a = 0; a < NA; ++a) {
                if (!F64) {
                    posf[0][a] = inc[a] + vc.pos0f[a];
                } else {
                    posd[0][a] = (double)inc[a] + vc.pos0[a];
                    posf[0][a] = (float)posd[0][a];
                }
            }
        } else {
#pragma clang fp contract(off)
            float carry1[NA], carry2[NA], lastv[NA];
#pragma unroll
            for (int a = 0; a < NA; ++a) { carry1[a] = 0.0f; carry2[a] = 0.0f; lastv[a] = 0.0f; }
#pragma unroll
            for (int c = 0; c < NCH; ++c) {
                float c1[NA], c2[NA];
#pragma unroll
                for (int a = 0; a < NA; ++a) c1[a] = act[c][a] * p.dt;
                seg_scan_f32_multi<LSEG, NA>(c1);
#pragma unroll
                for (int a = 0; a < NA; ++a) {
                    if (NCH > 1) {
                        c1[a] += carry1[a];
                        carry1[a] = read_lane_f32(c1[a], 63);
                    }
                    const float h2 = act[c][a] * (0.5f * p.dt2);
                    const float velf = c1[a] + vc.vel0f[a];
                    float prev = dpp_f32<0x138, 0xF>(velf);
                    if (t0 == 0) prev = (c == 0) ? vc.vel0f[a] : lastv[a];
                    if (NCH > 1) lastv[a] = read_lane_f32(velf, 63);
                    c2[a] = prev * p.dt + h2;
                }
                seg_scan_f32_multi<LSEG, NA>(c2);
#pragma unroll
                for (int a = 0; a < NA; ++a) {
                    if (NCH > 1) {
                        c2[a] += carry2[a];
                        carry2[a] = read_lane_f32(c2[a], 63);
                    }
                    if (!F64) {
                        posf[c][a] = c2[a] + vc.pos0f[a];
                    } else {
                        posd[c][a] = (double)c2[a] + vc.pos0[a];
                        posf[c][a] = (float)posd[c][a];
                    }
                }
            }
        }
        if (it == 0) STAMP(3);
        SECTION("fk_chain");
        if (ONEG && MPPI_PRIO) set_wave_prio(2);

        constexpr bool kStash = MPPI_EPS_STASH && NA >= 7 && (XC || NCH > 1);
        constexpr int kESP = (NCH == 1) ? IntegGeom<LSEG, NA>::P : NA;
        if constexpr (kStash) {
#pragma unroll
            for (int c = 0; c < NCH; ++c)
#pragma unroll
                for (int a = 0; a < NA; ++a) xw[(c * 64 + lane) * kESP + a] = eps[c][a];
            asm volatile("" ::: "memory");
        }

        float xs[NCH];
        float ecen = 0.0f, ejt = 0.0f, elim = 0.0f;
#pragma unroll
        for (int c = 0; c < NCH; ++c) {
            const int t = t0 + 64 * c;
            const bool val = kval && t < H;
            const bool term = (t == H - 1);
            float x;
            const uint32_t toff = ((uint32_t)k * (uint32_t)hp + (uint32_t)t) * 4u;
            const bool stv = p.store_traj && kval && t < hp;
            if (MODEL == MPPI_MODEL_DRONE) {
                const float dx = posf[c][0] - vc.tpos[0], dy = posf[c][1] - vc.tpos[1],
                            dz = posf[c][2] - vc.tpos[2];
                x = dx * dx + dy * dy + dz * dz;
                if (stv) {
#pragma unroll
                    for (int a = 0; a < 3; ++a) traj_store(trs, toff, (uint32_t)a * plane_b, posf[c][a]);
                }
            } else {
                auto qang = [&](int cc_, int j) {
                    if constexpr (F64) return posd[cc_][QOFF + j]; else return posf[cc_][QOFF + j];
                };
                if (stv) {
#pragma unroll
                    for (int a = 0; a < NA; ++a) traj_store(trs, toff, (uint32_t)a * plane_b, posf[c][a]);
                }
                Mat34 T;
#pragma unroll
                for (int i = 0; i < 12; ++i) T.m[i] = vc.base[i];
                if (MODEL == MPPI_MODEL_WHOLEBODY) {
                    T.m[3] += posf[c][0]; T.m[7] += posf[c][1]; T.m[11] += posf[c][2];
                }
                if (MPPI_KO & 4) {
                    T.m[3] += posf[c][QOFF]; T.m[7] += posf[c][QOFF + 1];
                } else if (NQ == 7 && (!XC || p.chain_fast == 2)) {
                    kin_joint<0>(T, jnt[p.j0 + 0].O, qang(c, 0));
                    kin_joint<1>(T, jnt[p.j0 + 1].O, qang(c, 1));
                    kin_joint<2>(T, jnt[p.j0 + 2].O, qang(c, 2));
                    kin_joint<3>(T, jnt[p.j0 + 3].O, qang(c, 3));
                    kin_joint<4>(T, jnt[p.j0 + 4].O, qang(c, 4));
                    kin_joint<5>(T, jnt[p.j0 + 5].O, qang(c, 5));
                    kin_joint<6>(T, jnt[p.j0 + 6].O, qang(c, 6));
                } else if (!XC) {
                } else if (p.chain_fast) {
#pragma unroll
                    for (int j = 0; j < NQ; ++j) {
                        const JointDev& J = jnt[p.j0 + j];
                        mul_affine(T, J.O);
                        float s, cc;
                        sincos_joint(qang(c, j), s, cc);
                        const float omc = 1.0f - cc, r22 = cc + omc;
#pragma unroll
                        for (int i = 0; i < 3; ++i) {
                            const float a0 = T.m[4 * i], a1 = T.m[4 * i + 1];
                            T.m[4 * i] = a0 * cc + a1 * s;
                            T.m[4 * i + 1] = a1 * cc - a0 * s;
                            T.m[4 * i + 2] = T.m[4 * i + 2] * r22;
                        }
                    }
                } else {
                    for (int jn = p.j0; jn < p.nj; ++jn) {
                        const JointDev& J = jnt[jn];
                        mul_affine(T, J.O);
                        if (J.type == MPPI_JOINT_FIXED) continue;
                        double qd = 0.0;
                        float qf = 0.0f;
#pragma unroll
                        for (int a = 0; a < NQ; ++a)
                            if (a == J.q_index) {
                                qd = F64 ? posd[c][QOFF + a] : 0.0;
                                qf = posf[c][QOFF + a];
                            }
                        if (J.type == MPPI_JOINT_REVOLUTE) {
                            float s, cc;
                            if constexpr (F64) sincos_joint(qd, s, cc); else sincos_joint(qf, s, cc);
                            mul_revolute(T, J, cc, s);
                        } else {
                            mul_prismatic(T, J, qf);
                        }
                    }
                }
                const float wsp = uniform_f32(p.w_sp), wso = uniform_f32(p.w_so), wtp = uniform_f32(p.w_tp),
                            wto = uniform_f32(p.w_to);
                SECTION("pose_cost");
                x = (MPPI_KO & 8) ? T.m[3] + T.m[7] + T.m[11] + T.m[0] : pose_cost(T, vc, term ? wtp : wsp, term ? wto : wso);
                SECTION("traj_ee_stores");
                if (stv) {
#pragma unroll
                    for (int i = 0; i < 12; ++i) traj_store(trs, toff, (uint32_t)(NA + i) * plane_b, T.m[i]);
                }
            }
            xs[c] = val ? x : 0.0f;
            if (XC && (p.cost_terms & (MPPI_COST_CENTER | MPPI_COST_JOINT_TRACK | MPPI_COST_JOINT_LIMIT))) {
                const int tc = (t < H) ? t : H - 1;
                const float* jt = p.jtraj ? p.jtraj + ((size_t)v * H + tc) * NQ : nullptr;
                float sc = 0.0f, sj = 0.0f;
                bool out = false;
#pragma unroll
                for (int j = 0; j < NQ; ++j) {
                    const float qj = posf[c][QOFF + j];
                    const float dc = qj - vc.qc[j];
                    sc = fmaf(dc, dc, sc);
                    const float dj = qj - (jt ? jt[j] : 0.0f);
                    sj = fmaf(dj, dj, sj);
                    const double qd = F64 ? posd[c][QOFF + j] : (double)qj;
                    out |= (qd < (double)vc.qlo[j]) | (qd > (double)vc.qhi[j]);
                }
                if (val) {
                    if (p.cost_terms & MPPI_COST_CENTER) ecen += (p.w_cen * sc) * gts[c];
                    if (p.cost_terms & MPPI_COST_JOINT_TRACK) ejt += (p.w_jt * sj) * gts[c];
                    if ((p.cost_terms & MPPI_COST_JOINT_LIMIT) && out) elim += p.lim_pen * gts[c];
                }
            }
        }
        if (it == 0) STAMP(4);
        SECTION("cost_sum_softmin");
        if (ONEG && MPPI_PRIO) set_wave_prio(1);

        float st = 0.0f;
#pragma unroll
        for (int c = 0; c < NCH; ++c) st += (t0 + 64 * c < H - 1) ? xs[c] : 0.0f;
        st = seg_scan_f32<LSEG>(st);
        float xt = 0.0f;
#pragma unroll
        for (int c = 0; c < NCH; ++c)
            if (c == (H - 1) / 64) xt = xs[c];
        float S_seg[R];
#pragma unroll
        for (int s = 0; s < R; ++s) {
            const int ks = (g * nw + wid) * R + s;
            const float stage = read_lane_f32(st, s * LSEG + LSEG - 1);
            const float term = read_lane_f32(xt, s * LSEG + ((H - 1) & 63));
            float S = (MODEL == MPPI_MODEL_DRONE) ? (p.w_sp * stage) + (p.w_tp * term) : stage + term;
            S_seg[s] = (ks < K) ? S : INFINITY;
        }
        if (XC) {
            float tsum[5] = {ecov, ecen, ejt, eact, elim};
            const int bits[5] = {MPPI_COST_COVAR, MPPI_COST_CENTER, MPPI_COST_JOINT_TRACK, MPPI_COST_ACTION,
                                 MPPI_COST_JOINT_LIMIT};
#pragma unroll
            for (int i = 0; i < 5; ++i) {
                if (!(p.cost_terms & bits[i])) continue;
                const float ts = seg_scan_f32<LSEG>(tsum[i]);
#pragma unroll
                for (int s = 0; s < R; ++s) {
                    float add = read_lane_f32(ts, s * LSEG + LSEG - 1);
                    if (i == 0) add = p.w_cov * add;
                    S_seg[s] += add;
                }
            }
        }
        float S_mine = S_seg[0];
#pragma unroll
        for (int s = 1; s < R; ++s) S_mine = (sub == s) ? S_seg[s] : S_mine;
        if (MPPI_S_PLAIN) { if (kval && t0 == 0) p.S[(size_t)v * K + k] = S_mine; }
        else if (kval && t0 == 0) s_stage[it * cost_run_stride(nw * R) + wid * R + sub] = S_mine;

        float m = INFINITY;
#pragma unroll
        for (int s = 0; s < R; ++s) {
            const bool bad = S_seg[s] != S_seg[s];
            nan_w |= bad;
            if (!bad) m = fminf(m, S_seg[s]);
        }
        if (m < INFINITY) {
            const float rn = fminf(rho_w, m);
            const float f = (rho_w == INFINITY) ? 0.0f : __expf(p.coef * (rho_w - rn));
            float es = 0.0f, e2 = 0.0f;
#pragma unroll
            for (int s = 0; s < R; ++s) {
                const float e = (S_seg[s] < INFINITY) ? __expf(p.coef * (S_seg[s] - rn)) : 0.0f;
                es += e;
                e2 += e * e;
            }
            eta_w = eta_w * f + es;
            eta2_w = eta2_w * f * f + e2;
            const float e_mine = (kval && !(S_mine != S_mine)) ? __expf(p.coef * (S_mine - rn)) : 0.0f;
            if constexpr (kStash) {
                asm volatile("" ::: "memory");
#pragma unroll
                for (int c = 0; c < NCH; ++c)
#pragma unroll
                    for (int a = 0; a < NA; ++a) eps[c][a] = xw[(c * 64 + lane) * kESP + a];
            }
#pragma unroll
            for (int c = 0; c < NCH; ++c)
#pragma unroll
                for (int a = 0; a < NA; ++a) acc[c][a] = acc[c][a] * f + e_mine * eps[c][a];
            rho_w = rn;
        }
    };
    if (ONEG) {
        if (MPPI_PRIO) set_wave_prio(3);
        group(0);
        if (MPPI_PRIO) set_wave_prio(0);
    } else if (iters == 1) {
        group(0);
    } else {
        for (int it = 0; it < iters; ++it) {
            if (MPPI_PRIO) set_wave_prio(iters - 1 - it);
            group(it);
        }
        if (MPPI_PRIO) set_wave_prio(0);
    }
    STAMP(5);
    SECTION("block_combine_record");

    float* wsh = smem + ((HA + 3) & ~3);
    const int wstride = kWs;
    float* mine = wsh + wid * wstride;
    if (lane == 0) {
        mine[0] = rho_w; mine[1] = eta_w; mine[2] = eta2_w; mine[3] = nan_w ? 1.0f : 0.0f;
    }
    if constexpr (!B512)
        for (int i = nw * wstride + tid; i < 8 * wstride; i += nthr)
            wsh[i] = ((i - nw * wstride) % wstride == 0) ? INFINITY : 0.0f;
#pragma unroll
    for (int c = 0; c < NCH; ++c)
#pragma unroll
        for (int a = 0; a < NA; ++a) mine[4 + (c * 64 + lane) * NA + a] = acc[c][a];
    STAMPW(11);
    lds_barrier();
    STAMP(6);
    if (!MPPI_S_PLAIN && wid == nw - 1) {
        const int nS = nw * R, q = (nS + 3) >> 2;
        float* const Sv = uniform_ptr(p.S + (size_t)v * K);
        for (int i = lane; i < iters * q; i += 64) {
            const int it = i / q, k0 = (blockIdx.x + it * p.nb) * nS;
            st_dev_run(Sv, (uint32_t)k0, s_stage + it * cost_run_stride(nS), min(nS, K - k0), i - it * q);
        }
    }
    if (MPPI_COMB_EXIT && wid != 0 && wid * 64 >= HA) {
        drain_stores();
        return;
    }
    float rws[8], rho_b = INFINITY;
#pragma unroll
    for (int w = 0; w < 8; ++w) {
        rws[w] = wsh[w * wstride];
        rho_b = fminf(rho_b, rws[w]);
    }
    float fw[8];
    {
        float mine = INFINITY;
#pragma unroll
        for (int w = 0; w < 8; ++w) mine = ((lane & 7) == w) ? rws[w] : mine;
        const float f = (mine < INFINITY) ? __expf(p.coef * (mine - rho_b)) : 0.0f;
#pragma unroll
        for (int w = 0; w < 8; ++w) fw[w] = read_lane_f32(f, w);
    }
    STAMP(12);
    if (tid == 0) {
        float eta = 0.0f, eta2 = 0.0f, nanf = 0.0f;
#pragma unroll
        for (int w = 0; w < 8; ++w) {
            eta += fw[w] * wsh[w * wstride + 1];
            eta2 += fw[w] * fw[w] * wsh[w * wstride + 2];
            nanf = fmaxf(nanf, wsh[w * wstride + 3]);
        }
        wt_store4(uniform_ptr(p.hdr), ((uint32_t)v * (uint32_t)p.nb + blockIdx.x) * 16u, make_float4(rho_b, eta, eta2, nanf));
    }
    const float rH = __builtin_amdgcn_rcpf((float)H);
    float* const rdata_v = uniform_ptr(p.rdata + (size_t)v * NA * p.nb * H);
    const uint32_t rbase = blockIdx.x * (uint32_t)H;
    const uint32_t rstride = (uint32_t)p.nb * (uint32_t)H;
    for (int i = tid; i < ((MPPI_KO & 64) ? 0 : HA); i += nthr) {
        const int a = (int)(((float)i + 0.5f) * rH), t = i - a * H;
        const int c = t >> 6, tl = t & 63;
        float s = 0.0f;
#pragma unroll
        for (int w = 0; w < 8; ++w) {
            float sw = wsh[w * wstride + 4 + (c * 64 + tl) * NA + a];
#pragma unroll
            for (int sg = 1; sg < R; ++sg) sw += wsh[w * wstride + 4 + (c * 64 + sg * LSEG + tl) * NA + a];
            s += fw[w] * sw;
        }
        wt_store(rdata_v, (rbase + (uint32_t)a * rstride + (uint32_t)t) * 4u, s);
    }
    STAMP(7);
    STAMPRT(14);
    drain_stores();
}

template <int MODEL, int NA, int NCH, int LSEG, bool F64, bool VONE, bool XC, bool ONEG>
__global__ void __launch_bounds__(512, (roll_occ<NCH, F64, XC, ONEG>())) k_rollout(const uint32_t seed_lo, const uint32_t seed_hi,
                                                 const uint32_t step_arg, const uint32_t k_off,
                                                 const int32_t noise_arg, const int32_t H_arg,
                                                 const int32_t geo_arg,
                                                 const float* __restrict__ u_prev,
                                                 const JointDev* __restrict__ jtab, const DevParams pk) {
    rollout_body<MODEL, NA, NCH, LSEG, F64, VONE, XC, ONEG, false>(seed_lo, seed_hi, step_arg, k_off, noise_arg, H_arg,
                                                                   geo_arg, u_prev, jtab, pk);
}
template <int MODEL, int NA, int NCH, int LSEG, bool F64, bool VONE, bool XC>
__global__ void __launch_bounds__(512, (roll_occ<NCH, F64, XC, true>())) k_rollout_s(const uint32_t seed_lo, const uint32_t seed_hi,
                                                 const uint32_t step_arg, const uint32_t k_off,
                                                 const int32_t noise_arg, const int32_t H_arg,
                                                 const int32_t geo_arg,
                                                 const float* __restrict__ u_prev,
                                                 const JointDev* __restrict__ jtab, const DevParams pk) {
    rollout_body<MODEL, NA, NCH, LSEG, F64, VONE, XC, true, true>(seed_lo, seed_hi, step_arg, k_off, noise_arg, H_arg,
                                                                  geo_arg, u_prev, jtab, pk);
}

template <int MODEL, int NA, int NCH, int LSEG, bool F64, bool VONE, bool XC, bool ONEG>
inline void rollout_symbol(char* buf, size_t n) {
    snprintf(buf, n, "_Z9k_rolloutILi%dELi%dELi%dELi%dELb%dELb%dELb%dELb%dEEvjjjjiiiPKfPKN4mppi8JointDevENS2_9DevParamsE",
             MODEL, NA, NCH, LSEG, (int)F64, (int)VONE, (int)XC, (int)ONEG);
}

template <int MODEL, int NA, int NCH, int LSEG, bool F64, bool VONE, bool XC>
inline void rollout_s_symbol(char* buf, size_t n) {
    snprintf(buf, n, "_Z11k_rollout_sILi%dELi%dELi%dELi%dELb%dELb%dELb%dEEvjjjjiiiPKfPKN4mppi8JointDevENS2_9DevParamsE",
             MODEL, NA, NCH, LSEG, (int)F64, (int)VONE, (int)XC);
}

template <int MODEL, int NA, int NCH, int LSEG, bool F64, bool XC, bool ONEG>
inline int launch_rollout_g(const DevParams& p, int threads, hipStream_t s) {
    const int iters = ONEG ? 1 : p.iters;
    const int s_run = iters * cost_run_stride((threads / 64) * (64 / LSEG));
    if (threads <= 0 || threads > 512 || iters < 1 || s_run > kMaxCostRun) return -1;
    const size_t lds = (size_t)(((p.H * NA + 3) & ~3) + 8 * wave_slot_floats<NA, NCH, LSEG>() + s_run) * sizeof(float);
    const int32_t geo = threads | (iters << 16);
    if (p.V == 1)
        return go(k_rollout<MODEL, NA, NCH, LSEG, F64, true, XC, ONEG>,
                  rollout_symbol<MODEL, NA, NCH, LSEG, F64, true, XC, ONEG>, dim3(p.nb, p.V), dim3(threads), lds, s,
                  p.seed_lo, p.seed_hi, p.step_ctr, (uint32_t)p.k_offset, p.noise_mode, p.H, geo, p.u_prev,
                  p.joints, p);
    return go(k_rollout<MODEL, NA, NCH, LSEG, F64, false, XC, ONEG>,
              rollout_symbol<MODEL, NA, NCH, LSEG, F64, false, XC, ONEG>, dim3(p.nb, p.V), dim3(threads), lds, s,
              p.seed_lo, p.seed_hi, p.step_ctr, (uint32_t)p.k_offset, p.noise_mode, p.H, geo, p.u_prev, p.joints,
              p);
}

template <int MODEL, int NA, int NCH, int LSEG, bool F64, bool XC>
inline int launch_rollout_s(const DevParams& p, hipStream_t s) {
    constexpr int threads = 512;
    const int s_run = cost_run_stride((threads / 64) * (64 / LSEG));
    if (s_run > kMaxCostRun) return -1;
    const size_t lds = (size_t)(((p.H * NA + 3) & ~3) + 8 * wave_slot_floats<NA, NCH, LSEG>() + s_run) * sizeof(float);
    const int32_t geo = threads | (1 << 16);
    if (p.V == 1)
        return go(k_rollout_s<MODEL, NA, NCH, LSEG, F64, true, XC>, rollout_s_symbol<MODEL, NA, NCH, LSEG, F64, true, XC>,
                  dim3(p.nb, p.V), dim3(threads), lds, s, p.seed_lo, p.seed_hi, p.step_ctr, (uint32_t)p.k_offset,
                  p.noise_mode, p.H, geo, p.u_prev, p.joints, p);
    return go(k_rollout_s<MODEL, NA, NCH, LSEG, F64, false, XC>, rollout_s_symbol<MODEL, NA, NCH, LSEG, F64, false, XC>,
              dim3(p.nb, p.V), dim3(threads), lds, s, p.seed_lo, p.seed_hi, p.step_ctr, (uint32_t)p.k_offset,
              p.noise_mode, p.H, geo, p.u_prev, p.joints, p);
}

template <int MODEL, int NA, int NCH, int LSEG, bool F64, bool XC>
inline int launch_rollout_x(const DevParams& p, int threads, hipStream_t s) {
    if constexpr (!XC && NCH == 1)
        if (p.iters == 1) {
            if (threads == 512 && !p.kern && !(p.noise_mode & kNoiseOverlap) && p.H <= LSEG * NCH)
                return launch_rollout_s<MODEL, NA, NCH, LSEG, F64, XC>(p, s);
            return launch_rollout_g<MODEL, NA, NCH, LSEG, F64, XC, true>(p, threads, s);
        }
    return launch_rollout_g<MODEL, NA, NCH, LSEG, F64, XC, false>(p, threads, s);
}

template <int MODEL, int NA, int NCH, int LSEG, bool F64>
inline int launch_rollout_t(const DevParams& p, int threads, hipStream_t s) {
    const bool generic_chain = MODEL != MPPI_MODEL_DRONE && !(NA - (MODEL == MPPI_MODEL_WHOLEBODY ? 3 : 0) == 7 &&
                                                              p.chain_fast == 2);
    if (p.cost_terms || !p.sigma_diag || generic_chain)
        return launch_rollout_x<MODEL, NA, NCH, LSEG, F64, true>(p, threads, s);
    return launch_rollout_x<MODEL, NA, NCH, LSEG, F64, false>(p, threads, s);
}

template <int MODEL, int NA, bool F64>
inline int dispatch_geom(const DevParams& p, int threads, hipStream_t s) {
    if (p.nch == 1 && p.L == 32) return launch_rollout_t<MODEL, NA, 1, 32, F64>(p, threads, s);
    if (p.nch == 1 && p.L == 64) return launch_rollout_t<MODEL, NA, 1, 64, F64>(p, threads, s);
    if (p.nch == 2) return launch_rollout_t<MODEL, NA, 2, 64, F64>(p, threads, s);
    if (p.nch == 4) return launch_rollout_t<MODEL, NA, 4, 64, F64>(p, threads, s);
    return -1;
}
```

quadrotor_manipulator_mppi_amd/csrc/mppi_rollout_quad.hip:

```cpp
#include <type_traits>

#include "mppi_rollout.h"

namespace {

constexpr int kQA = 4;
constexpr int kQR = 16;
constexpr int kQWaves = 4;
constexpr int kQThreads = 64 * kQWaves;
constexpr int kQThreadsWide = 512;

template <int SRC>
__device__ __forceinline__ float qbc(float x) {
    return __int_as_float(__builtin_amdgcn_mov_dpp(__float_as_int(x), SRC * 0x55, 0xF, 0xF, false));
}
__device__ __forceinline__ float lane_sel(float a, float b, uint64_t m) {
    float r;
    asm("v_cndmask_b32_e64 %0, %1, %2, %3" : "=v"(r) : "v"(a), "v"(b), "s"(m));
    return r;
}
__device__ __forceinline__ float qsum(float x) {
    x += __int_as_float(__builtin_amdgcn_mov_dpp(__float_as_int(x), 0xB1, 0xF, 0xF, false));
    x += __int_as_float(__builtin_amdgcn_mov_dpp(__float_as_int(x), 0x4E, 0xF, 0xF, false));
    return x;
}
}

template <bool VONE, bool LIT, int NWD, int NT>
__global__ void __launch_bounds__(NT) k_rollout_quad(const uint32_t seed_lo, const uint32_t seed_hi,
                                                            const uint32_t step_arg, const uint32_t k_off,
                                                            const int32_t noise_arg, const int32_t H,
                                                            const float* __restrict__ u_prev, const DevParams pk) {
    static_assert(NWD == 1 || NWD == kQWaves, "dynamics waves per block");
    static_assert(NT == kQThreads || (NWD == 1 && NT == kQThreadsWide), "block size");
    constexpr int QR = kQR * NWD;
    constexpr int kQPitch = QR * kQA + 1;
    extern __shared__ __attribute__((aligned(16))) float qlds[];
    __shared__ float e_lds[QR];
    __shared__ __attribute__((aligned(16))) float s_lds[QR];
    __shared__ float wred[kQWaves][4];
    __shared__ float4 part[kQWaves][64];
    const DevParams& p = pk;
    const int tid = threadIdx.x, lane = tid & 63, wid = tid >> 6, v = blockIdx.y, b = blockIdx.x;
    const int32_t noise_mode = noise_arg & 0xFF;
    const uint32_t step_ctr = step_of(step_arg, noise_arg);
    const uint32_t vkey = (uint32_t)v + ((uint32_t)noise_arg >> 16);
    const int K = p.K;
    const int kb = b * QR;
    float* const eps_t = qlds;
    float* const u_t = qlds + (H + 1) * kQPitch;
    const VehicleConst& vc = VONE ? pk.vc0 : pk.vc[v];
    if (VONE && b == 0) {
        constexpr int kVCW = (int)(sizeof(VehicleConst) / 4);
        for (int i = tid; i < kVCW; i += NT)
            __hip_atomic_store((int*)pk.vc + i, i == kVcStepWord ? (int)step_ctr : ((const int*)&pk.vc0)[i],
                               __ATOMIC_RELAXED, __HIP_MEMORY_SCOPE_AGENT);
    }
    const float* up = u_prev + (size_t)v * H * kQA;
    const float u_r = (tid < H * kQA) ? ld_dev(up + tid) : 0.0f;
    float x6[6], v6[6], tg3[3], ii3[3];
#pragma unroll
    for (int d = 0; d < 6; ++d) { x6[d] = uniform_f32(vc.pos0f[d]); v6[d] = uniform_f32(vc.vel0f[d]); }
#pragma unroll
    for (int d = 0; d < 3; ++d) { tg3[d] = uniform_f32(vc.tpos[d]); ii3[d] = p.q_iinv[d]; }
    float sdt = p.dt, sim = p.q_inv_m, skd = p.q_kd, sg = p.q_g, swsp = p.w_sp, swtp = p.w_tp, scoef = p.coef;
    const int sstore = p.store_traj;
    asm volatile("" : "+s"(x6[0]), "+s"(x6[1]), "+s"(x6[2]), "+s"(x6[3]), "+s"(x6[4]), "+s"(x6[5]),
                      "+s"(v6[0]), "+s"(v6[1]), "+s"(v6[2]), "+s"(v6[3]), "+s"(v6[4]), "+s"(v6[5]),
                      "+s"(tg3[0]), "+s"(tg3[1]), "+s"(tg3[2]), "+s"(ii3[0]), "+s"(ii3[1]), "+s"(ii3[2]),
                      "+s"(sdt), "+s"(sim), "+s"(skd), "+s"(sg), "+s"(swsp), "+s"(swtp), "+s"(scoef));
    for (int i = tid; i < QR * H; i += NT) {
        const int r = i & (QR - 1), t = i / QR, k = kb + r;
        const bool kval = k < K;
        const int kc = kval ? k : K - 1;
        float eps[kQA];
        if (noise_mode == MPPI_NOISE_INJECTED) {
            const float4 n = *reinterpret_cast<const float4*>(p.noise_in + (((size_t)v * K + kc) * H + t) * kQA);
            eps[0] = n.x; eps[1] = n.y; eps[2] = n.z; eps[3] = n.w;
        } else {
            float z[kQA];
            draw_normals<kQA>(z, k_off + (uint32_t)kc, (uint32_t)t, vkey, step_ctr, seed_lo, seed_hi);
            if (p.sigma_diag) {
#pragma unroll
                for (int a = 0; a < kQA; ++a) eps[a] = z[a] * p.sdiag[a];
            } else {
#pragma unroll
                for (int c = 0; c < kQA; ++c) {
                    float e = 0.0f;
#pragma unroll
                    for (int a = 0; a < kQA; ++a) e += z[a] * p.sigma[a * kQA + c];
                    eps[c] = e;
                }
            }
        }
        float* dst = eps_t + t * kQPitch + r * kQA;
#pragma unroll
        for (int a = 0; a < kQA; ++a) dst[a] = eps[a];
        if (p.store_noise && kval) {
            float* dst = p.noise_out + (((size_t)v * K + k) * H + t) * kQA;
#pragma unroll
            for (int a = 0; a < kQA; ++a) st_dev(dst + a, eps[a]);
        }
    }
    if (tid < H * kQA) u_t[tid] = u_r;
    __syncthreads();
    if (wid >= NWD) { drain_stores(); return; }

    const int r = wid * kQR + (lane >> 2), j = lane & 3, jj = j < 3 ? j : 2;
    const int k = kb + r;
    const bool kval = k < K;
    const int kc = kval ? k : K - 1;
    constexpr uint64_t kM0 = 0x1111111111111111ull, kM1 = 0x2222222222222222ull;
    constexpr uint64_t kM2 = 0xCCCCCCCCCCCCCCCCull;
    auto axis = [&](const float* x3) { return lane_sel(lane_sel(x3[2], x3[1], kM1), x3[0], kM0); };
    const float dt = sdt, im = sim, kd = skd;
    const float gj = (j >= 2) ? -sg : 0.0f;
    const float ij = axis(ii3), tg = axis(tg3);
    float pj = axis(x6), ej = axis(x6 + 3), vj = axis(v6), wj = axis(v6 + 3);
    const float ox0 = v6[3], oy0 = v6[4], oz0 = v6[5];
    const int kp = pk.hp;
    const uint32_t plane_b = (uint32_t)kp * (uint32_t)H * 4u;
    const __amdgpu_buffer_rsrc_t trs = traj_rsrc(pk.traj + (size_t)v * pk.C * kp * H, plane_b, pk.C);
    const uint32_t off_p = (uint32_t)(k < kp ? k : kc) * 4u + (uint32_t)jj * plane_b, off_e = off_p + 3u * plane_b;
    const uint32_t tstep_b = (uint32_t)kp * 4u;
    const bool store = sstore != 0;
    float stage = 0.0f, term = 0.0f;
    const float a0 = (j == 0) ? 1.0f : 0.0f;
    const float* rowp = eps_t + r * kQA;
    const float* urp = u_t;
    float pu0 = urp[0], pe0 = rowp[0], pu1 = urp[1 + jj], pe1 = rowp[1 + jj];
    auto step = [&](const int t, auto first_c, auto last_c) {
        constexpr bool FIRST = decltype(first_c)::value, LAST = decltype(last_c)::value;
        const float thr = pu0 + pe0, tau = pu1 + pe1;
        rowp += kQPitch;
        urp += kQA;
        pu0 = urp[0]; pe0 = rowp[0]; pu1 = urp[1 + jj]; pe1 = rowp[1 + jj];
        wj = wj + dt * (ij * tau);
        float sj, cj;
        sincos_joint(ej, sj, cj);
        const float sr = qbc<0>(sj), cr = qbc<0>(cj), sp = qbc<1>(sj), cp = qbc<1>(cj);
        const float sy = qbc<2>(sj), cy = qbc<2>(cj);
        const float ox = FIRST ? ox0 : qbc<0>(wj), oy = FIRST ? oy0 : qbc<1>(wj), oz = FIRST ? oz0 : qbc<2>(wj);
        float dj;
        if (LIT && !FIRST) {
            const float d0 = ox - sp * oz;
            const float d1 = cr * oy + (sr * cp) * oz;
            const float d2 = (cr * cp) * oz - sr * oy;
            dj = lane_sel(lane_sel(d2, d1, kM1), d0, kM0);
        } else {
            const float ic = __builtin_amdgcn_rcpf(cp);
            const float f = ic * lane_sel(1.0f, sp, kM0);
            const float Bj = lane_sel(sr * f, cr, kM1), Cj = lane_sel(cr * f, -sr, kM1);
            dj = fmaf(Cj, oz, fmaf(Bj, oy, a0 * ox));
        }
        float en = ej + dt * dj;
        if (!FIRST) en = en - 6.283185307179586f * __builtin_rintf(en * 0.15915494309189535f);
        const float Pj = lane_sel(sy, cy, kM0), Qj = lane_sel(-cy, sy, kM0);
        const float rj = lane_sel(fmaf(Pj, sp * cr, Qj * sr), cp * cr, kM2);
        const float aj = gj + im * (rj * thr - kd * vj);
        const float nv = vj + dt * aj;
        pj = pj + dt * (FIRST ? vj : nv);
        vj = nv;
        ej = en;
        if (store) {
            const uint32_t o = (uint32_t)t * tstep_b;
            traj_store(trs, off_p, o, pj);
            traj_store(trs, off_e, o, ej);
        }
        const float dd = pj - tg;
        if (LAST) term = dd * dd; else stage = fmaf(dd, dd, stage);
    };
    using T_ = std::true_type;
    using F_ = std::false_type;
    step(0, T_{}, F_{});
    int t = 1;
    for (; t + 4 <= H - 1; t += 4) {
        step(t, F_{}, F_{}); step(t + 1, F_{}, F_{}); step(t + 2, F_{}, F_{}); step(t + 3, F_{}, F_{});
    }
    for (; t < H - 1; ++t) step(t, F_{}, F_{});
    step(H - 1, F_{}, T_{});
    stage = qbc<0>(stage) + qbc<1>(stage) + qbc<2>(stage);
    term = qbc<0>(term) + qbc<1>(term) + qbc<2>(term);
    const float S = kval ? (swsp * stage) + (swtp * term) : INFINITY;
    if (j == 0) s_lds[r] = S;
    const bool mine = kval && j == 0, bad = S != S;
    float rho = wave_fold_all((mine && !bad) ? S : INFINITY, OpMin());
    float nanf = wave_fold_all(mine && bad ? 1.0f : 0.0f, OpMax());
    if constexpr (NWD > 1) {
        if (lane == 0) { wred[wid][0] = rho; wred[wid][3] = nanf; }
        __syncthreads();
#pragma unroll
        for (int w = 0; w < NWD; ++w) { rho = fminf(rho, wred[w][0]); nanf = fmaxf(nanf, wred[w][3]); }
    }
    const float e = (mine && !bad && rho < INFINITY) ? __expf(scoef * (S - rho)) : 0.0f;
    float eta = wave_fold_all(e, OpAdd()), eta2 = wave_fold_all(e * e, OpAdd());
    if (j == 0) e_lds[r] = e;
    wave_lds_handoff();
    {
        const int k0 = kb + wid * kQR, n = min(kQR, K - k0);
        if (lane < 4) st_dev_run(uniform_ptr(p.S + (size_t)v * K), (uint32_t)k0, s_lds + wid * kQR, n, lane);
    }
    float n[kQA] = {0.0f, 0.0f, 0.0f, 0.0f};
    if (lane < H) {
        const float* row = eps_t + lane * kQPitch + wid * kQR * kQA;
#pragma unroll
        for (int rr = 0; rr < kQR; ++rr) {
            const float w = e_lds[wid * kQR + rr];
#pragma unroll
            for (int a = 0; a < kQA; ++a) n[a] = fmaf(w, row[rr * kQA + a], n[a]);
        }
    }
    if constexpr (NWD > 1) {
        if (lane == 0) { wred[wid][1] = eta; wred[wid][2] = eta2; }
        if (wid > 0 && lane < H) part[wid][lane] = make_float4(n[0], n[1], n[2], n[3]);
        __syncthreads();
        if (wid != 0) { drain_stores(); return; }
        eta = 0.0f; eta2 = 0.0f;
#pragma unroll
        for (int w = 0; w < NWD; ++w) { eta += wred[w][1]; eta2 += wred[w][2]; }
        if (lane < H) {
#pragma unroll
            for (int w = 1; w < NWD; ++w) {
                const float4 x = part[w][lane];
                n[0] += x.x; n[1] += x.y; n[2] += x.z; n[3] += x.w;
            }
        }
    }
    if (lane == 0)
        wt_store4(uniform_ptr(p.hdr), ((uint32_t)v * (uint32_t)p.nb + (uint32_t)b) * 16u, make_float4(rho, eta, eta2, nanf));
    if (lane < H) {
        float* const rdata_v = uniform_ptr(p.rdata + (size_t)v * kQA * p.nb * H);
#pragma unroll
        for (int a = 0; a < kQA; ++a)
            wt_store(rdata_v, (((uint32_t)a * (uint32_t)p.nb + (uint32_t)b) * (uint32_t)H + (uint32_t)lane) * 4u, n[a]);
    }
    drain_stores();
}

extern "C" int mppi_launch_rollout_quad(const DevParams* p, int threads, void* stream) {
    (void)threads;
    const int nwd = p->iters;
    if (p->H > 64 || p->A != kQA || (nwd != 1 && nwd != kQWaves) || p->nb * kQR * nwd < p->K) return -1;
    const size_t lds = (size_t)((p->H + 1) * (kQR * nwd * kQA + 1) + (p->H + 1) * kQA) * sizeof(float);
    hipStream_t s = (hipStream_t)stream;
    const bool wide = nwd == 1 && (size_t)p->nb * p->V <= 512;
#define MPPI_QUAD_GO(VO, LI, NW, NT)                                                                             \
    return go(k_rollout_quad<VO, LI, NW, NT>,                                                                    \
              [](char* b, size_t n) {                                                                            \
                  snprintf(b, n, "_Z14k_rollout_quadILb%dELb%dELi%dELi%dEEvjjjjiiPKfN4mppi9DevParamsE", (int)VO, \
                           (int)LI, NW, NT);                                                                     \
              },                                                                                                 \
              dim3(p->nb, p->V), dim3(NT), lds, s, p->seed_lo, p->seed_hi, p->step_ctr, (uint32_t)p->k_offset,   \
              p->noise_mode, p->H, p->u_prev, *p)
#define MPPI_QUAD_NW(VO, LI)                                                                                     \
    do {                                                                                                         \
        if (wide) MPPI_QUAD_GO(VO, LI, 1, kQThreadsWide);                                                        \
        else if (nwd == 1) MPPI_QUAD_GO(VO, LI, 1, kQThreads);                                                   \
        else MPPI_QUAD_GO(VO, LI, kQWaves, kQThreads);                                                           \
    } while (0)
    if (p->V == 1) {
        if (p->q_literal_jinv) MPPI_QUAD_NW(true, true); else MPPI_QUAD_NW(true, false);
    } else {
        if (p->q_literal_jinv) MPPI_QUAD_NW(false, true); else MPPI_QUAD_NW(false, false);
    }
#undef MPPI_QUAD_NW
#undef MPPI_QUAD_GO
    return -1;
}
```

quadrotor_manipulator_mppi_amd/csrc/mppi_step.cpp:

```cpp
#include <emmintrin.h>

#include <algorithm>
#include <atomic>
#include <chrono>
#include <cmath>
#include <cstddef>
#include <cstdio>
#include <cstdlib>
#include <cstring>
#include <string>
#include <vector>

#include "mppi_engine.h"

using namespace mppi;

namespace mppi_host {

void block_records(const mppi_engine* e, FinParams& f) {
    const int64_t nb = e->dp.nb, H = e->H;
    f.nrec = (int32_t)nb;
    f.hdr = e->d_hdr; f.hdr_vs = nb * 4; f.hdr_rs = 4;
    f.dat = e->d_rdata; f.d_vs = (int64_t)e->A * nb * H; f.d_as = nb * H; f.d_rs = H;
}

void final_records(const mppi_engine* e, FinParams& f) {
    if (sharded(e)) {
        const int64_t P = e->dp.P;
        f.nrec = e->cfg.shard_count;
        f.hdr = e->d_exchange; f.hdr_vs = P; f.hdr_rs = (int64_t)e->V * P;
        f.dat = e->d_exchange + kHdr; f.d_vs = P; f.d_as = e->H; f.d_rs = (int64_t)e->V * P;
    } else {
        block_records(e, f);
    }
}

}

using namespace mppi_host;

extern "C" {

mppi_status mppi_rollout(mppi_engine* e, const float* d_noise) {
    if (!e) return fail(MPPI_ERR_INVALID_ARG, "null engine");
    if (!e->state_set) return fail(MPPI_ERR_STATE, "mppi_rollout before mppi_set_state");
    if (e->cfg.noise_mode == MPPI_NOISE_INJECTED && !d_noise)
        return fail(MPPI_ERR_INVALID_ARG, "INJECTED noise mode needs a device noise buffer");
    if (sharded(e) && !e->d_exchange)
        return fail(MPPI_ERR_STATE, "shard_count > 1 needs mppi_bind_exchange or mppi_comm_init");
    if (use_device(e)) return MPPI_ERR_HIP;
    DevParams p = e->dp;
    p.noise_in = d_noise;
    p.vc0 = e->h_vc[0];
    p.step_ctr = e->step_ctr;
    hipEvent_t e0 = nullptr, e1 = nullptr;
    if (e->timing) { e0 = pool_event(e); e1 = pool_event(e); HIP_TRY(hipEventRecord(e0, e->stream)); }
    int rc = mppi_launch_rollout(&p, e->threads, e->stream);
    if (rc != 0) return fail(MPPI_ERR_HIP, "rollout launch failed (%d: %s)", rc,
                             rc > 0 ? hipGetErrorString((hipError_t)rc) : "no kernel for this model/A/H");
    if (e->timing) {
        HIP_TRY(hipEventRecord(e1, e->stream));
        e->roll_pairs.emplace_back(e0, e1);
        if (e->roll_pairs.size() >= 2048) { mppi_status st = drain_timing(e); if (st) return st; }
    }
    if (sharded(e)) {
        FinParams f = e->fp;
        pack_fields(e, f);
        f.tail = e->d_tail + kTailPack;
        if (f.stamps) f.stamps += (size_t)e->V * e->A * e->fin_ts * kStamps;
        block_records(e, f);
        rc = mppi_launch_finalize(&f, e->stream);
        if (rc != 0) return fail(MPPI_ERR_HIP, "pack launch failed (%d)", rc);
    }
    return MPPI_OK;
}

static bool quiet_steps(const mppi_engine* e) {
    return !(e->generic & 3) && !e->timing && !e->d_stamps && !e->d_fstamps && !e->out_dbg && !e->no_flag_dbg && !e->overlap;
}

static std::string fin_symbol(const FinParams& f) {
    LaunchDesc d{};
    mppi_aql::set_capture(&d);
    const int rc = mppi_launch_finalize(&f, nullptr);
    mppi_aql::set_capture(nullptr);
    return rc == 0 ? d.symbol : "?";
}
static std::string roll_symbol(const DevParams& p, int threads) {
    LaunchDesc d{};
    mppi_aql::set_capture(&d);
    const int rc = mppi_launch_rollout(&p, threads, nullptr);
    mppi_aql::set_capture(nullptr);
    return rc == 0 ? d.symbol : "?";
}
static std::string kernels_text(const std::string& roll, const std::string& fin, const std::string* quiet) {
    std::string s = "rollout " + roll + ", finalize " + fin;
    if (quiet) s += ", quiet finalize " + (*quiet == fin ? std::string("none") : *quiet);
    return s;
}

static mppi_status finalize_impl(mppi_engine* e, bool record_out, bool quiet = false) {
    if (use_device(e)) return MPPI_ERR_HIP;
    FinParams f = e->fp;
    f.mode = 0;
    if (quiet && !record_out && quiet_steps(e)) f.kern |= kFinKernQuiet;
    f.seq = 0u;
    if (record_out && !e->no_flag_dbg) {
        f.seq = ++e->seq_ctr & 0x7FFFFFFFu;
        if (f.seq == 0u) f.seq = ++e->seq_ctr & 0x7FFFFFFFu;
    }
    final_records(e, f);
    if (e->out_dbg == 1 && !record_out) f.tail = e->d_tail + kTailScratch;
    hipEvent_t e0 = nullptr, e1 = nullptr;
    if (e->timing) { e0 = pool_event(e); e1 = pool_event(e); HIP_TRY(hipEventRecord(e0, e->stream)); }
    int rc = mppi_launch_finalize(&f, e->stream);
    if (rc != 0) return fail(MPPI_ERR_HIP, "finalize launch failed (%d)", rc);
    if (e->timing) { HIP_TRY(hipEventRecord(e1, e->stream)); e->fin_pairs.emplace_back(e0, e1); }
    if (record_out) e->out_seq = f.seq;
    if (record_out) HIP_TRY(hipEventRecord(e->ev_out, e->stream));
    ++e->step_ctr;
    e->out_pending = record_out;
    e->aql_out = false;
    e->aql_call = false;
    return MPPI_OK;
}

mppi_status mppi_finalize(mppi_engine* e) {
    if (!e) return fail(MPPI_ERR_INVALID_ARG, "null engine");
    return finalize_impl(e, true);
}

static bool records_tagged(const mppi_engine* e, uint32_t want) {
    const volatile uint32_t* r = (const volatile uint32_t*)(e->h_out + off_flags(e));
    const size_t n = rec_count(e);
    for (size_t i = 0; i < n; ++i)
        if (r[4 * i + 3] != want) return false;
    return true;
}

static inline bool load_record(const mppi_engine* e, size_t i, uint32_t want, uint32_t (&w)[4]) {
    const __m128i x = _mm_load_si128((const __m128i*)(e->h_out + off_flags(e)) + i);
    _mm_storeu_si128((__m128i*)w, x);
    return w[3] == want;
}

static mppi_status wait_outputs(mppi_engine* e) {
    if (e->aql_out) return aql_join(e);
    if (e->aql_call) {
        const uint32_t want = e->out_seq;
        const auto t0 = std::chrono::steady_clock::now();
        for (uint64_t it = 1;; ++it) {
            if (records_tagged(e, want)) break;
            if ((it & 255u) == 0) {
                if (const int q = mppi_aql::step_error(e->aql)) return fail(MPPI_ERR_HIP, "native queue error %d", q);
                if (std::chrono::steady_clock::now() - t0 > std::chrono::seconds(60))
                    return fail(MPPI_ERR_HIP, "native control call: no outputs after 60 s");
            }
            __builtin_ia32_pause();
        }
        std::atomic_thread_fence(std::memory_order_acquire);
        mppi_aql::step_call_read(e->aql);
        e->call_wait_us = std::chrono::duration<double, std::micro>(std::chrono::steady_clock::now() - t0).count();
        return MPPI_OK;
    }
    if (!e->event_wait) {
        const uint32_t want = e->out_seq;
        for (uint64_t it = 1;; ++it) {
            if (records_tagged(e, want)) {
                std::atomic_thread_fence(std::memory_order_acquire);
                return MPPI_OK;
            }
            if ((it & 255u) == 0) {
                const hipError_t q = hipEventQuery(e->ev_out);
                if (q == hipSuccess) break;
                if (q != hipErrorNotReady) return fail(MPPI_ERR_HIP, "waiting for the step: %s", hipGetErrorString(q));
            }
            __builtin_ia32_pause();
        }
    }
    HIP_TRY(hipEventSynchronize(e->ev_out));
    return MPPI_OK;
}

static mppi_status assemble_records(mppi_engine* e) {
    const int V = e->V, A = e->A, od = e->out_dim, model = e->cfg.model;
    const uint32_t want = e->out_seq;
    e->rec_out.assign((const double*)e->h_out, (const double*)e->h_out + (size_t)V * od);
    e->rec_u0.resize((size_t)V * A);
    e->rec_stats.resize((size_t)V * 4);
    const int qoff = (model == MPPI_MODEL_WHOLEBODY) ? 3 : 0, nq = A - qoff;
    uint32_t w[4];
    for (int v = 0; v < V; ++v) {
        const size_t r0 = (size_t)v * (2 * A + 1);
        for (int a = 0; a < A; ++a) {
            double o1, o2;
            if (!load_record(e, r0 + 2 * a, want, w)) return fail(MPPI_ERR_STATE, "output record (%d,%d) not tagged", v, a);
            std::memcpy(&o1, w, 8);
            std::memcpy(&e->rec_u0[(size_t)v * A + a], &w[2], 4);
            if (!load_record(e, r0 + 2 * a + 1, want, w)) return fail(MPPI_ERR_STATE, "output record (%d,%d) not tagged", v, a);
            std::memcpy(&o2, w, 8);
            {
                float nf;
                std::memcpy(&nf, &w[2], 4);
                float& st3 = e->rec_stats[(size_t)v * 4 + 3];
                st3 = (a == 0 || nf > st3 || std::isnan(nf)) ? nf : st3;
            }
            double* ov = e->rec_out.data() + (size_t)v * od;
            if (model == MPPI_MODEL_QUADROTOR) continue;
            if (model == MPPI_MODEL_DRONE || (model == MPPI_MODEL_WHOLEBODY && a < 3)) {
                ov[a] = o1; ov[3 + a] = o2;
            } else {
                const int base = (model == MPPI_MODEL_WHOLEBODY) ? 6 : 0, j = a - qoff;
                ov[base + j] = o1; ov[base + nq + j] = o2;
            }
        }
        if (!load_record(e, r0 + 2 * A, want, w)) return fail(MPPI_ERR_STATE, "stats record %d not tagged", v);
        std::memcpy(&e->rec_stats[(size_t)v * 4], w, 12);
    }
    return MPPI_OK;
}

mppi_status mppi_read_outputs(mppi_engine* e, double* out, float* u0, mppi_stats* stats) {
    if (!e) return fail(MPPI_ERR_INVALID_ARG, "null engine");
    if (!e->out_pending) return fail(MPPI_ERR_STATE, "no finalised step to read");
    if (e->aql_call) HIP_TRY(hipSetDevice(e->cfg.device));
    else if (use_device(e)) return MPPI_ERR_HIP;
    {   mppi_status st = wait_outputs(e);
        if (st != MPPI_OK) return st; }
    if (e->d_stamps) {
        const size_t nwaves = (size_t)e->V * e->dp.nb * (e->threads / 64);
        std::vector<unsigned long long> st(nwaves * kStamps);
        HIP_TRY(hipMemcpy(st.data(), e->d_stamps, st.size() * 8, hipMemcpyDeviceToHost));
        for (size_t w = 0; w < nwaves; ++w) {
            const unsigned long long* x = &st[w * kStamps];
            for (size_t i = 1; i < kRollStampOrder.size(); ++i)
                e->stamp_sum[i] += (double)(x[kRollStampOrder[i]] - x[kRollStampOrder[i - 1]]);
        }
        e->stamp_n += (int64_t)nwaves;
        const size_t nfb = (size_t)e->V * e->A * e->fin_ts;
        std::vector<unsigned long long> fs(nfb * kStamps);
        HIP_TRY(hipMemcpy(fs.data(), e->d_fstamps, fs.size() * 8, hipMemcpyDeviceToHost));
        for (size_t b = 0; b < nfb; ++b) {
            const unsigned long long* x = &fs[b * kStamps];
            for (size_t i = 1; i < kFinStampOrder.size(); ++i)
                e->fstamp_sum[i] += (double)(x[kFinStampOrder[i]] - x[kFinStampOrder[i - 1]]);
        }
        e->fstamp_n += (int64_t)nfb;
    }
    const double* o = (const double*)e->h_out;
    const float* uu = (const float*)(e->h_out + off_u0(e));
    const float* st = (const float*)(e->h_out + off_stats(e));
    if (!e->aql_out && e->out_seq != 0u) {
        mppi_status rs = assemble_records(e);
        if (rs != MPPI_OK) return rs;
        o = e->rec_out.data();
        uu = e->rec_u0.data();
        st = e->rec_stats.data();
    }
    if (out) std::memcpy(out, o, sizeof(double) * e->V * e->out_dim);
    if (out && e->cfg.model == MPPI_MODEL_QUADROTOR)
        for (int v = 0; v < e->V; ++v)
            quad_outputs(e, e->state.data() + (size_t)v * e->state_dim, uu + (size_t)v * e->A, out + (size_t)v * e->out_dim);
    if (u0) std::memcpy(u0, uu, sizeof(float) * e->V * e->A);
    bool nonfinite = false;
    for (int v = 0; v < e->V; ++v) {
        int reach = 0;
        if (e->cfg.check_reach && e->cfg.model == MPPI_MODEL_ARM) {
            const double* s = e->state.data() + (size_t)v * e->state_dim;
            const double* qdes = o + (size_t)v * e->out_dim;
            float T16[16];
            host_fk_c(e->cfg.joints, e->cfg.n_joints, e->fk_O.data(), e->fk_ax.data(), qdes, s, e->cfg.state_f64 != 0,
                      T16);
            const float err = std::fabs(T16[3] - e->tpos[3 * v]) + std::fabs(T16[7] - e->tpos[3 * v + 1]) +
                              std::fabs(T16[11] - e->tpos[3 * v + 2]);
            reach = err < e->cfg.reach_tol;
        }
        const int nf = (st[4 * v + 3] >= 2.0f || (e->peer && sticky_timeout(e) != 0u)) ? 2
                       : ((st[4 * v + 3] > 0.0f) || !std::isfinite(st[4 * v]) || !std::isfinite(uu[(size_t)v * e->A]));
        nonfinite |= nf;
        if (stats) {
            stats[v].rho = st[4 * v];
            stats[v].eta = st[4 * v + 1];
            stats[v].ess = st[4 * v + 2];
            stats[v].nonfinite = nf;
            stats[v].reach = reach;
            stats[v]._pad = 0;
        }
    }
    (void)nonfinite;
    return MPPI_OK;
}

static mppi_status control_call_aql(mppi_engine* e, const double* state, bool* used);

mppi_status mppi_step(mppi_engine* e, const double* state, const float* h_noise, double* out, float* u0,
                      mppi_stats* stats) {
    if (!e) return fail(MPPI_ERR_INVALID_ARG, "null engine");
    note_call(e);
    if (sharded(e) && !e->comm)
        return fail(MPPI_ERR_STATE, "mppi_step on a shard needs mppi_comm_init (or use the split phases)");
    mppi_status st;
    if (e->cfg.noise_mode == MPPI_NOISE_PHILOX && e->V == 1 && !sharded(e)) {
        bool used = false;
        static const bool prof = getenv("MPPI_AQL_PROFILE") != nullptr;
        const auto c0 = std::chrono::steady_clock::now();
        if ((st = control_call_aql(e, state, &used)) != MPPI_OK) return st;
        e->calls_native = used;
        e->pw_native.store(used, std::memory_order_release);
        if (used) {
            if (!prof) return mppi_read_outputs(e, out, u0, stats);
            const auto c1 = std::chrono::steady_clock::now();
            st = mppi_read_outputs(e, out, u0, stats);
            const auto c2 = std::chrono::steady_clock::now();
            static double acc[3] = {0, 0, 0};
            static long cn = 0;
            const double pre = std::chrono::duration<double, std::micro>(c1 - c0).count();
            const double rd = std::chrono::duration<double, std::micro>(c2 - c1).count();
            acc[0] += pre; acc[1] += e->call_wait_us; acc[2] += rd - e->call_wait_us;
            if (++cn % 1000 == 0)
                fprintf(stderr, "[mppi aql] per call (us): before the doorbell %.2f  flag wait %.2f  outputs + check_reach %.2f\n",
                        acc[0] / cn, acc[1] / cn, acc[2] / cn);
            return st;
        }
    }
    e->calls_native = false;
    e->pw_native.store(false, std::memory_order_relaxed);
    if (state && (st = mppi_set_state(e, state)) != MPPI_OK) return st;
    const float* dn = nullptr;
    if (e->cfg.noise_mode == MPPI_NOISE_INJECTED) {
        if (!h_noise) return fail(MPPI_ERR_INVALID_ARG, "INJECTED noise mode needs noise");
        const size_t n = (size_t)e->V * e->K * e->H * e->A;
        if (use_device(e)) return MPPI_ERR_HIP;
        if (!e->d_noise_in) HIP_TRY(hipMalloc(&e->d_noise_in, n * sizeof(float)));
        HIP_TRY(hipMemcpyAsync(e->d_noise_in, h_noise, n * sizeof(float), hipMemcpyHostToDevice, e->stream));
        dn = e->d_noise_in;
    }
    if ((st = mppi_rollout(e, dn)) != MPPI_OK) return st;
    if (e->comm && (st = mppi_exchange(e)) != MPPI_OK) return st;
    if ((st = mppi_finalize(e)) != MPPI_OK) return st;
    if (!e->kern_call_hip || e->kern_call_peer != e->peer) {
        DevParams p = e->dp;
        p.noise_in = dn;
        p.vc0 = e->h_vc[0];
        FinParams f = e->fp;
        f.mode = 0;
        final_records(e, f);
        e->kern_call = kernels_text(roll_symbol(p, e->threads), fin_symbol(f), nullptr);
        e->kern_call_hip = true;
        e->kern_call_peer = e->peer;
    }
    return mppi_read_outputs(e, out, u0, stats);
}

static const char* aql_ineligible(const mppi_engine* e, bool batch = false) {
    if (e->aql_mode == 0) return "MPPI_DISPATCH=hip";
    if (sharded(e)) return "sharded step (its collective runs on the HIP stream)";
    if (e->timing) return "per-launch timing events (mppi_enable_timing)";
    if (e->d_stamps && !batch) return "stamps diagnostics";
    if (e->out_dbg || (e->no_flag_dbg && !batch)) return "output diagnostics";
    return nullptr;
}

constexpr uint32_t kRollStepOff = 8;
constexpr int32_t kNoiseStepFromId = 0x100;
constexpr int32_t kNoiseOverlap = 0x200;

static bool aql_ready(mppi_engine* e) {
    if (e->aql_off) return false;
    if (!e->aql && !e->aql_tried) {
        e->aql_tried = true;
        std::string why;
        if (hipSetDevice(e->cfg.device) == hipSuccess) e->aql = mppi_aql::step_create(e->cfg.device, &why);
        else why = "hipSetDevice failed";
        if (!e->aql) e->aql_why = why;
    }
    if (!e->aql) e->aql_off = true;
    return e->aql != nullptr;
}

static mppi_status run_steps_aql(mppi_engine* e, int32_t n, bool* used) {
    *used = false;
    if (const char* why = aql_ineligible(e, true)) { e->aql_why = why; return MPPI_OK; }
    if (!aql_ready(e)) return e->aql_mode == 1 ? fail(MPPI_ERR_STATE, "native dispatch: %s", e->aql_why.c_str()) : MPPI_OK;
    HIP_TRY(hipSetDevice(e->cfg.device));
    static const bool prof = getenv("MPPI_AQL_PROFILE") != nullptr;
    static double pt[4] = {0, 0, 0, 0};
    static long pn = 0;
    auto now = [] { return std::chrono::steady_clock::now(); };
    const auto c0 = now();
    const hipError_t q = hipStreamQuery(e->stream);
    if (q == hipErrorNotReady) HIP_TRY(hipStreamSynchronize(e->stream));
    else if (q != hipSuccess) return fail(MPPI_ERR_HIP, "engine stream: %s", hipGetErrorString(q));
    const auto c1 = now();
    LaunchDesc& roll = e->batch_roll;
    LaunchDesc& fin = e->batch_fin;
    LaunchDesc& finq = e->batch_fin_quiet;
    DevParams p = e->dp;
    p.noise_in = nullptr;
    p.vc0 = e->h_vc[0];
    p.step_ctr = 0u;
    p.noise_mode |= kNoiseStepFromId;
    const bool ovl = e->overlap && n > 1;
    if (ovl) p.noise_mode |= kNoiseOverlap;
    FinParams f = e->fp;
    f.mode = 0;
    f.seq = 0u;
    final_records(e, f);
    if (!(e->batch_cached && e->batch_threads == e->threads && std::memcmp(&p, &e->batch_p, sizeof(p)) == 0 &&
          std::memcmp(&f, &e->batch_f, sizeof(f)) == 0)) {
        e->batch_cached = false;
        e->kern_batch_state = 0;
        mppi_aql::set_capture(&roll);
        int rc = mppi_launch_rollout(&p, e->threads, e->stream);
        if (rc == 0) {
            mppi_aql::set_capture(&fin);
            rc = mppi_launch_finalize(&f, e->stream);
        }
        if (rc == 0) {
            FinParams fq = f;
            if (quiet_steps(e)) fq.kern |= kFinKernQuiet;
            mppi_aql::set_capture(&finq);
            rc = mppi_launch_finalize(&fq, e->stream);
        }
        mppi_aql::set_capture(nullptr);
        if (rc != 0) return fail(MPPI_ERR_HIP, "describing the step's launches failed (%d)", rc);
        e->batch_p = p;
        e->batch_f = f;
        e->batch_threads = e->threads;
        e->batch_cached = true;
    }
    std::string err;
    const auto c2 = now();
    const auto guard = mppi_aql::step_guard(e->aql);
    const int pr = mppi_aql::step_prepare(e->aql, roll, fin, finq, e->step_ctr, kRollStepOff, &err);
    const auto c3 = now();
    if (pr == -2) {
        e->aql_off = true;
        e->aql_why = err;
        return e->aql_mode == 1 ? fail(MPPI_ERR_STATE, "native dispatch: %s", err.c_str()) : MPPI_OK;
    }
    if (pr == 0 && ovl) {
        HIP_TRY(hipMemsetD32Async((hipDeviceptr_t)e->d_ovl, (int)e->step_ctr, (size_t)e->V * e->A * e->fin_ts,
                                  e->stream));
        HIP_TRY(hipStreamSynchronize(e->stream));
    }
    if (pr != 0 || mppi_aql::step_dispatch(e->aql, n, &err, ovl) != 0)
        return fail(MPPI_ERR_HIP, "native dispatch: %s", err.c_str());
    if (prof) {
        const auto c4 = now();
        const std::chrono::steady_clock::time_point cs[5] = {c0, c1, c2, c3, c4};
        for (int i = 0; i < 4; ++i) pt[i] += std::chrono::duration<double, std::micro>(cs[i + 1] - cs[i]).count();
        if (++pn % 200 == 0)
            fprintf(stderr, "[mppi aql] per batch (us): stream query %.2f  capture %.2f  prepare %.2f  packets %.2f\n",
                    pt[0] / pn, pt[1] / pn, pt[2] / pn, pt[3] / pn);
    }
    e->step_ctr += (uint32_t)n;
    e->out_pending = true;
    e->aql_out = true;
    e->aql_call = false;
    e->aql_why.clear();
    if (e->kern_batch_state != (n > 1 ? 2 : 1)) {
        const std::string q = n > 1 ? finq.symbol : fin.symbol;
        e->kern_batch = kernels_text(roll.symbol, fin.symbol, &q);
        e->kern_batch_state = n > 1 ? 2 : 1;
    }
    *used = true;
    return MPPI_OK;
}

static mppi_status control_call_aql(mppi_engine* e, const double* state, bool* used) {
    *used = false;
    if (aql_ineligible(e) || e->event_wait) return MPPI_OK;
    if (!aql_ready(e)) return e->aql_mode == 1 ? fail(MPPI_ERR_STATE, "native dispatch: %s", e->aql_why.c_str())
                                               : MPPI_OK;
    static const bool prof = getenv("MPPI_AQL_PROFILE") != nullptr;
    static double pacc[4] = {0, 0, 0, 0};
    static long pcn = 0;
    const auto q0 = std::chrono::steady_clock::now();
    HIP_TRY(hipSetDevice(e->cfg.device));
    const auto q1 = std::chrono::steady_clock::now();
    if (state) {
        std::memcpy(e->state.data(), state, sizeof(double) * e->state.size());
        e->state_set = true;
        mppi_status st = build_vehicle_consts(e);
        if (st != MPPI_OK) return st;
    }
    if (!e->state_set) return fail(MPPI_ERR_STATE, "mppi_step before mppi_set_state");
    const auto q2 = std::chrono::steady_clock::now();
    {
        const hipError_t q = hipStreamQuery(e->stream);
        if (q == hipErrorNotReady) HIP_TRY(hipStreamSynchronize(e->stream));
        else if (q != hipSuccess) return fail(MPPI_ERR_HIP, "engine stream: %s", hipGetErrorString(q));
    }
    const auto q3 = std::chrono::steady_clock::now();
    DevParams p = e->dp;
    p.noise_in = nullptr;
    p.vc0 = e->h_vc[0];
    p.step_ctr = 0u;
    p.noise_mode |= kNoiseStepFromId;
    FinParams f = e->fp;
    f.mode = 0;
    f.seq = kSeqFromVc;
    final_records(e, f);
    LaunchDesc& roll = e->call_roll;
    LaunchDesc& fin = e->call_fin;
    constexpr size_t kVo = offsetof(DevParams, vc0), kVn = sizeof(VehicleConst);
    const bool hit = e->call_cached && e->call_threads == e->threads &&
                     std::memcmp(&p, &e->call_p, kVo) == 0 &&
                     std::memcmp((const char*)&p + kVo + kVn, (const char*)&e->call_p + kVo + kVn,
                                 sizeof(DevParams) - kVo - kVn) == 0 &&
                     std::memcmp(&f, &e->call_f, sizeof(FinParams)) == 0;
    if (hit) {
        std::memcpy(roll.args + roll.arg_bytes - sizeof(DevParams) + kVo, &p.vc0, kVn);
    } else {
        e->call_cached = false;
        mppi_aql::set_capture(&roll);
        int rc = mppi_launch_rollout(&p, e->threads, e->stream);
        if (rc == 0) {
            mppi_aql::set_capture(&fin);
            rc = mppi_launch_finalize(&f, e->stream);
        }
        mppi_aql::set_capture(nullptr);
        if (rc != 0) return fail(MPPI_ERR_HIP, "describing the step's launches failed (%d)", rc);
        e->call_p = p;
        e->call_f = f;
        e->call_threads = e->threads;
        e->call_cached = true;
    }
    if (prof) {
        const auto q4 = std::chrono::steady_clock::now();
        const std::chrono::steady_clock::time_point qs[5] = {q0, q1, q2, q3, q4};
        for (int i = 0; i < 4; ++i) pacc[i] += std::chrono::duration<double, std::micro>(qs[i + 1] - qs[i]).count();
        if (++pcn % 1000 == 0)
            fprintf(stderr, "[mppi aql] call setup (us): hipSetDevice %.2f  vehicle constants %.2f  stream query %.2f  "
                            "capture %.2f\n", pacc[0] / pcn, pacc[1] / pcn, pacc[2] / pcn, pacc[3] / pcn);
    }
    const uint32_t seq_off = roll.arg_bytes - (uint32_t)sizeof(DevParams) + (uint32_t)offsetof(DevParams, vc0) +
                             (uint32_t)offsetof(VehicleConst, _pad);
    std::string err;
    uint32_t seq = 0;
    const int pr = mppi_aql::step_call(e->aql, roll, fin, e->step_ctr, kRollStepOff, seq_off, &seq, &err);
    if (pr == -2) {
        e->aql_off = true;
        e->aql_why = err;
        return e->aql_mode == 1 ? fail(MPPI_ERR_STATE, "native dispatch: %s", err.c_str()) : MPPI_OK;
    }
    if (pr != 0) return fail(MPPI_ERR_HIP, "native dispatch: %s", err.c_str());
    ++e->step_ctr;
    e->out_seq = seq;
    e->out_pending = true;
    e->aql_out = false;
    e->aql_call = true;
    if (!hit || e->kern_call_hip) e->kern_call = kernels_text(roll.symbol, fin.symbol, nullptr);
    e->kern_call_hip = false;
    *used = true;
    return MPPI_OK;
}

mppi_status mppi_run_steps(mppi_engine* e, int32_t n) {
    if (!e || n < 0) return fail(MPPI_ERR_INVALID_ARG, "mppi_run_steps: bad arguments");
    if (sharded(e) && !e->comm) return fail(MPPI_ERR_STATE, "mppi_run_steps on a shard needs mppi_comm_init");
    if (e->cfg.noise_mode != MPPI_NOISE_PHILOX) return fail(MPPI_ERR_STATE, "mppi_run_steps needs device noise");
    if (!e->state_set) return fail(MPPI_ERR_STATE, "mppi_run_steps before mppi_set_state");
    if (n == 0) return MPPI_OK;
    bool used = false;
    mppi_status st = run_steps_aql(e, n, &used);
    if (st != MPPI_OK || used) return st;
    for (int i = 0; i < n; ++i) {
        mppi_status st = mppi_rollout(e, nullptr);
        if (st != MPPI_OK) return st;
        if (e->comm && (st = mppi_exchange(e)) != MPPI_OK) return st;
        if ((st = finalize_impl(e, i == n - 1, true)) != MPPI_OK) return st;
    }
    {
        DevParams p = e->dp;
        p.vc0 = e->h_vc[0];
        FinParams f = e->fp;
        f.mode = 0;
        final_records(e, f);
        const std::string full = fin_symbol(f);
        if (n > 1 && quiet_steps(e)) f.kern |= kFinKernQuiet;
        const std::string q = fin_symbol(f);
        e->kern_batch = kernels_text(roll_symbol(p, e->threads), full, &q);
        e->kern_batch_state = 0;
    }
    return MPPI_OK;
}

mppi_status mppi_kernel_info(mppi_engine* e, char* buf, int32_t len) {
    if (!e || !buf || len <= 0) return fail(MPPI_ERR_INVALID_ARG, "mppi_kernel_info: bad arguments");
    snprintf(buf, (size_t)len, "batch: %s; call: %s%s", e->kern_batch.c_str(), e->kern_call.c_str(),
             e->generic == 7 ? "; MPPI_GENERIC_KERNELS" : e->generic ? "; MPPI_GENERIC_KERNELS (in part)" : "");
    return MPPI_OK;
}

mppi_status mppi_dispatch_info(mppi_engine* e, char* buf, int32_t len) {
    if (!e || !buf || len <= 0) return fail(MPPI_ERR_INVALID_ARG, "mppi_dispatch_info: bad arguments");
    snprintf(buf, (size_t)len, "%s%s; calls: %s%s%s", e->aql_why.empty() ? "aql" : "hip: ", e->aql_why.c_str(),
             e->calls_native ? "aql (arguments in " : "hip", e->calls_native ? mppi_aql::step_call_memory(e->aql) : "",
             e->calls_native ? ")" : "");
    return MPPI_OK;
}

int32_t mppi_debug_finalize_kernels(const int32_t* g, char* full, char* quiet, int32_t len) {
    if (!g || !full || !quiet || len <= 0) return MPPI_ERR_INVALID_ARG;
    static const FinTail tail{};
    static unsigned long long* const peers[1] = {nullptr};
    FinParams f;
    std::memset(&f, 0, sizeof(f));
    f.V = 1; f.A = g[0]; f.H = g[1]; f.tsz = g[2]; f.half = g[3]; f.ts = g[4]; f.window = g[5]; f.nrec = g[6];
    f.mode = g[7];
    f.tail = &tail;
    if (g[8]) f.xpeers = peers;
    f.kern = g[9] ? kFinKernGeneric : 0;
    const std::string a = fin_symbol(f);
    if (!g[9]) f.kern |= kFinKernQuiet;
    const std::string b = fin_symbol(f);
    snprintf(full, (size_t)len, "%s", a.c_str());
    snprintf(quiet, (size_t)len, "%s", b.c_str());
    return (a == "?" || b == "?") ? MPPI_ERR_INVALID_ARG : MPPI_OK;
}

mppi_status mppi_synchronize(mppi_engine* e) {
    if (!e) return fail(MPPI_ERR_INVALID_ARG, "null engine");
    if (use_device(e)) return MPPI_ERR_HIP;
    if (e->out_pending && !e->event_wait && !e->aql_out) {
        mppi_status st = wait_outputs(e);
        if (st != MPPI_OK) return st;
    }
    HIP_TRY(hipStreamSynchronize(e->stream));
    if (e->peer)
        if (const uint32_t t = sticky_timeout(e))
            return fail(MPPI_ERR_PEER_TIMEOUT, "peer exchange: a step was given up (tag %08x): this rank's "
                                               "warm start may differ from its peers' until mppi_peer_reset", t);
    return MPPI_OK;
}

int32_t mppi_debug_queue_touch(mppi_engine* e) {
    if (!e || !e->aql) return MPPI_ERR_INVALID_ARG;
    std::string err;
    const int r = mppi_aql::step_touch(e->aql, false, &err);
    return r == 0 ? MPPI_OK : fail(MPPI_ERR_HIP, "queue touch: %s", err.c_str());
}


int64_t mppi_debug_stamps(mppi_engine* e, unsigned long long* out, int64_t max_waves) {
    if (!e || !out) return MPPI_ERR_INVALID_ARG;
    if (!e->d_stamps) return 0;
    if (use_device(e)) return MPPI_ERR_HIP;
    const int64_t nwaves = std::min<int64_t>(max_waves, (int64_t)e->V * e->dp.nb * (e->threads / 64));
    if (hipStreamSynchronize(e->stream) != hipSuccess ||
        hipMemcpy(out, e->d_stamps, (size_t)nwaves * kStamps * 8, hipMemcpyDeviceToHost) != hipSuccess)
        return MPPI_ERR_HIP;
    return nwaves;
}

int64_t mppi_debug_fstamps(mppi_engine* e, unsigned long long* out, int64_t max_blocks, int32_t which) {
    if (!e || !out || which < 0 || which > 1) return MPPI_ERR_INVALID_ARG;
    if (!e->d_fstamps) return 0;
    if (use_device(e)) return MPPI_ERR_HIP;
    const int64_t nb = (int64_t)e->V * e->A * e->fin_ts;
    const int64_t n = std::min<int64_t>(max_blocks, nb);
    if (hipStreamSynchronize(e->stream) != hipSuccess ||
        hipMemcpy(out, e->d_fstamps + (size_t)which * nb * kStamps, (size_t)n * kStamps * 8, hipMemcpyDeviceToHost) !=
            hipSuccess)
        return MPPI_ERR_HIP;
    return n;
}

int32_t mppi_debug_queue_ring(mppi_engine* e) {
    if (!e || !e->aql) return MPPI_ERR_INVALID_ARG;
    if (e->pw_us.load()) return fail(MPPI_ERR_STATE, "mppi_debug_queue_ring: the prewarm thread also writes packets");
    mppi_aql::step_ring(e->aql);
    return MPPI_OK;
}

}
```

Before: 16.61 billion.

## Add quiet rollout kernel variant for non-final steps of batched runs

Adds a compile-time QUIET specialization of the rollout body that skips trajectory stores, per-sample cost writes and the vc handshake stores. Batched multi-step runs dispatch it for every step except the last, through a fourth argument block in the AQL path and a flag in the HIP fallback. The aim is to cut global-memory writes for intermediate steps whose outputs are never read. The cost is another kernel instantiation and argument upload, and a risk that a skipped output is in fact consumed by the quiet finalize.

```diff
diff --git a/quadrotor_manipulator_mppi_amd/csrc/mppi_aql.cpp b/quadrotor_manipulator_mppi_amd/csrc/mppi_aql.cpp
--- a/quadrotor_manipulator_mppi_amd/csrc/mppi_aql.cpp
+++ b/quadrotor_manipulator_mppi_amd/csrc/mppi_aql.cpp
@@ -212,7 +212,7 @@
 constexpr size_t kArgSlot = 4096;
 constexpr uint32_t kCallSlots = 16;
 constexpr uint32_t kBatchSlots = 4;
-constexpr uint32_t kBatchBlocks = 3;
+constexpr uint32_t kBatchBlocks = 4;
 
 struct Step {
     Device* dev = nullptr;
@@ -232,6 +232,8 @@
     mppi::LaunchDesc roll{}, fin{};
     mppi::LaunchDesc fin_quiet{};
     Kern kr, kf, kfq;
+    mppi::LaunchDesc roll_quiet{};
+    Kern krq;
     uint32_t step_off = 0, step_word = 0;
     bool valid = false;
     int64_t outstanding = 0;
@@ -362,12 +364,13 @@
 
 static unsigned char* batch_args(Step* s) { return s->d_args + (1 + kBatchBlocks * (size_t)s->batch_slot) * kArgSlot; }
 
-int step_prepare(Step* s, const mppi::LaunchDesc& roll, const mppi::LaunchDesc& fin, const mppi::LaunchDesc& fin_quiet,
-                 uint32_t step, uint32_t step_off, std::string* err) {
+int step_prepare(Step* s, const mppi::LaunchDesc& roll, const mppi::LaunchDesc& roll_quiet, const mppi::LaunchDesc& fin,
+                 const mppi::LaunchDesc& fin_quiet, uint32_t step, uint32_t step_off, std::string* err) {
     std::lock_guard<std::recursive_mutex> qlk(s->mu);
     const uint32_t word = step - (uint32_t)(hsa_queue_load_write_index_relaxed(s->q) >> 1);
     if (s->valid && s->step_word == word && s->step_off == step_off && same_launch(roll, s->roll, step_off) &&
-        same_launch(fin, s->fin, ~0u) && same_launch(fin_quiet, s->fin_quiet, ~0u))
+        same_launch(roll_quiet, s->roll_quiet, step_off) && same_launch(fin, s->fin, ~0u) &&
+        same_launch(fin_quiet, s->fin_quiet, ~0u))
         return 0;
     if (getenv("MPPI_AQL_PROFILE") && s->valid) {
         int first = -1;
@@ -379,21 +382,28 @@
         fprintf(stderr, "[mppi aql] re-upload: word %u vs %u, rollout args differ at %d, finalize at %d, sym %d/%d\n", word,
                 s->step_word, first, ffirst, strcmp(roll.symbol, s->roll.symbol), strcmp(fin.symbol, s->fin.symbol));
     }
-    Kern kr, kf, kfq;
+    Kern kr, kf, kfq, krq;
     {
         std::lock_guard<std::mutex> lk(g_mu);
         if (!lookup(s->dev, roll.symbol, &kr, err) || !lookup(s->dev, fin.symbol, &kf, err) ||
-            !lookup(s->dev, fin_quiet.symbol, &kfq, err))
+            !lookup(s->dev, fin_quiet.symbol, &kfq, err) || !lookup(s->dev, roll_quiet.symbol, &krq, err))
             return -2;
     }
-    if (!check_launch(roll, kr, err) || !check_launch(fin, kf, err) || !check_launch(fin_quiet, kfq, err)) return -2;
-    if (step_off + 4 > roll.arg_bytes) { *err = "step counter outside the rollout's arguments"; return -2; }
+    if (!check_launch(roll, kr, err) || !check_launch(fin, kf, err) || !check_launch(fin_quiet, kfq, err) ||
+        !check_launch(roll_quiet, krq, err))
+        return -2;
+    if (step_off + 4 > roll.arg_bytes || step_off + 4 > roll_quiet.arg_bytes) {
+        *err = "step counter outside the rollout's arguments";
+        return -2;
+    }
     if (s->outstanding && step_wait(s, 60000, err) != 0) return -1;
     std::vector<unsigned char> h(kBatchBlocks * kArgSlot, 0);
     memcpy(h.data(), roll.args, roll.arg_bytes);
     memcpy(h.data() + step_off, &word, 4);
     memcpy(h.data() + kArgSlot, fin.args, fin.arg_bytes);
     memcpy(h.data() + 2 * kArgSlot, fin_quiet.args, fin_quiet.arg_bytes);
+    memcpy(h.data() + 3 * kArgSlot, roll_quiet.args, roll_quiet.arg_bytes);
+    memcpy(h.data() + 3 * kArgSlot + step_off, &word, 4);
     s->batch_slot = (s->batch_slot + 1) % kBatchSlots;
     if (hipMemcpy(batch_args(s), h.data(), h.size(), hipMemcpyHostToDevice) != hipSuccess) {
         *err = "uploading the argument blocks failed";
@@ -403,6 +413,8 @@
     s->roll = roll;
     s->fin = fin;
     s->fin_quiet = fin_quiet;
+    s->roll_quiet = roll_quiet;
+    s->krq = krq;
     s->kr = kr;
     s->kf = kf;
     s->kfq = kfq;
@@ -515,11 +527,12 @@
     void* ra = batch_args(s);
     void* fa = batch_args(s) + kArgSlot;
     void* fqa = batch_args(s) + 2 * kArgSlot;
+    void* rqa = batch_args(s) + 3 * kArgSlot;
     load_fences();
     for (int i = 0; i < n; ++i) {
         const bool last = i == n - 1;
-        put(s->q, s->kr, s->roll, ra, none, i == 0 ? std::max(1, g_fence[0]) : g_fence[0], g_fence[1],
-            !(overlap && i > 0));
+        put(s->q, last ? s->kr : s->krq, last ? s->roll : s->roll_quiet, last ? ra : rqa, none,
+            i == 0 ? std::max(1, g_fence[0]) : g_fence[0], g_fence[1], !(overlap && i > 0));
         if (last) put(s->q, s->kf, s->fin, fa, s->done, g_fence[2], 2);
         else put(s->q, s->kfq, s->fin_quiet, fqa, none, g_fence[2], g_fence[3]);
         hsa_signal_store_screlease(s->q->doorbell_signal, (hsa_signal_value_t)hsa_queue_load_write_index_relaxed(s->q) - 1);
diff --git a/quadrotor_manipulator_mppi_amd/csrc/mppi_aql.h b/quadrotor_manipulator_mppi_amd/csrc/mppi_aql.h
--- a/quadrotor_manipulator_mppi_amd/csrc/mppi_aql.h
+++ b/quadrotor_manipulator_mppi_amd/csrc/mppi_aql.h
@@ -13,8 +13,8 @@
 Step* step_create(int device, std::string* why);
 bool step_destroy(Step* s);
 
-int step_prepare(Step* s, const mppi::LaunchDesc& roll, const mppi::LaunchDesc& fin, const mppi::LaunchDesc& fin_quiet,
-                 uint32_t step, uint32_t step_off, std::string* err);
+int step_prepare(Step* s, const mppi::LaunchDesc& roll, const mppi::LaunchDesc& roll_quiet, const mppi::LaunchDesc& fin,
+                 const mppi::LaunchDesc& fin_quiet, uint32_t step, uint32_t step_off, std::string* err);
 int step_dispatch(Step* s, int n, std::string* err, bool overlap = false);
 std::unique_lock<std::recursive_mutex> step_guard(Step* s);
 int step_call(Step* s, const mppi::LaunchDesc& roll, const mppi::LaunchDesc& fin, uint32_t step,
diff --git a/quadrotor_manipulator_mppi_amd/csrc/mppi_dev.h b/quadrotor_manipulator_mppi_amd/csrc/mppi_dev.h
--- a/quadrotor_manipulator_mppi_amd/csrc/mppi_dev.h
+++ b/quadrotor_manipulator_mppi_amd/csrc/mppi_dev.h
@@ -101,6 +101,7 @@
     int32_t ovl_n;
     int32_t kern;
 };
+constexpr int32_t kRollKernGeneric = 1, kRollKernQuiet = 2;
 constexpr int kStamps = 16;
 
 struct FinTail {
diff --git a/quadrotor_manipulator_mppi_amd/csrc/mppi_engine.cpp b/quadrotor_manipulator_mppi_amd/csrc/mppi_engine.cpp
--- a/quadrotor_manipulator_mppi_amd/csrc/mppi_engine.cpp
+++ b/quadrotor_manipulator_mppi_amd/csrc/mppi_engine.cpp
@@ -423,9 +423,10 @@
     f.wraw = e->d_wraw; f.wsmooth = e->d_wsmooth; f.out_dim = e->out_dim;
     if (const char* dbg = getenv("MPPI_FIN_DEBUG")) f.dbg = atoi(dbg);
     if (const char* g = getenv("MPPI_GENERIC_KERNELS"))
-        e->generic = !strcmp(g, "finalize") ? 1 : !strcmp(g, "quiet") ? 2 : !strcmp(g, "rollout") ? 4 : atoi(g) != 0 ? 7 : 0;
+        e->generic = !strcmp(g, "finalize") ? 1 : !strcmp(g, "quiet") ? 2 : !strcmp(g, "rollout") ? 4
+                     : !strcmp(g, "quiet_rollout") ? 8 : atoi(g) != 0 ? kGenericAll : 0;
     f.kern = (e->generic & 1) ? kFinKernGeneric : 0;
-    p.kern = (e->generic & 4) ? 1 : 0;
+    p.kern = (e->generic & 4) ? kRollKernGeneric : 0;
     e->event_wait = getenv("MPPI_EVENT_WAIT") && atoi(getenv("MPPI_EVENT_WAIT")) != 0;
     e->no_flag_dbg = e->event_wait && getenv("MPPI_DEBUG_NO_FLAG") && atoi(getenv("MPPI_DEBUG_NO_FLAG")) != 0;
     e->out_dbg = getenv("MPPI_DEBUG_OUT") ? atoi(getenv("MPPI_DEBUG_OUT")) : 0;
diff --git a/quadrotor_manipulator_mppi_amd/csrc/mppi_engine.h b/quadrotor_manipulator_mppi_amd/csrc/mppi_engine.h
--- a/quadrotor_manipulator_mppi_amd/csrc/mppi_engine.h
+++ b/quadrotor_manipulator_mppi_amd/csrc/mppi_engine.h
@@ -12,6 +12,8 @@
 
 #include "mppi_aql.h"
 #include "mppi_dev.h"
+
+constexpr int kGenericAll = 15;
 
 struct mppi_engine {
     mppi_config cfg;
@@ -40,6 +42,7 @@
     mppi::FinParams batch_f{};
     mppi::LaunchDesc batch_roll{}, batch_fin{};
     mppi::LaunchDesc batch_fin_quiet{};
+    mppi::LaunchDesc batch_roll_quiet{};
     int generic = 0;
     std::string kern_batch = "none", kern_call = "none";
     int kern_batch_state = 0;
diff --git a/quadrotor_manipulator_mppi_amd/csrc/mppi_rollout.h b/quadrotor_manipulator_mppi_amd/csrc/mppi_rollout.h
--- a/quadrotor_manipulator_mppi_amd/csrc/mppi_rollout.h
+++ b/quadrotor_manipulator_mppi_amd/csrc/mppi_rollout.h
@@ -496,7 +496,7 @@
 constexpr int roll_occ() {
     return (ONEG && !F64) ? 8 : (NCH >= 4 ? 2 : NCH == 2 ? (XC ? MPPI_ROLL_OCC_NCH2_XC : MPPI_ROLL_OCC_NCH2) : (XC ? MPPI_ROLL_OCC_XC : MPPI_ROLL_OCC));
 }
-template <int MODEL, int NA, int NCH, int LSEG, bool F64, bool VONE, bool XC, bool ONEG, bool B512>
+template <int MODEL, int NA, int NCH, int LSEG, bool F64, bool VONE, bool XC, bool ONEG, bool B512, bool QUIET = false>
 __device__ __forceinline__ void rollout_body(const uint32_t seed_lo, const uint32_t seed_hi,
                                              const uint32_t step_arg, const uint32_t k_off,
                                              const int32_t noise_arg, const int32_t H_arg,
@@ -504,6 +504,10 @@
                                              const float* __restrict__ u_prev,
                                              const JointDev* __restrict__ jtab, const DevParams& pk) {
     static_assert(!B512 || ONEG, "the fixed-block body is a single-group one");
+    static_assert(!QUIET || (!XC && NCH == 1), "the quiet body exists for the common one-chunk kernels");
+    constexpr bool kTraj = !QUIET && !(MPPI_KO & 16);
+    constexpr bool kCosts = !QUIET && !(MPPI_KO & 1024);
+    constexpr bool kHand = !QUIET && !(MPPI_KO & 2048);
     constexpr int R = 64 / LSEG;
     constexpr int QOFF = (MODEL == MPPI_MODEL_WHOLEBODY) ? 3 : 0;
     constexpr int NQ = (MODEL == MPPI_MODEL_DRONE) ? 0 : NA - QOFF;
@@ -596,7 +600,7 @@
     }
     if (tid < kVCW) {
         ((int*)&vcv)[tid] = vcr;
-        if (VONE && blockIdx.x == 0)
+        if (kHand && VONE && blockIdx.x == 0)
             __hip_atomic_store((int*)pk.vc + tid, tid == kVcStepWord ? (int)step_ctr : vcr, __ATOMIC_RELAXED,
                                __HIP_MEMORY_SCOPE_AGENT);
     }
@@ -604,7 +608,7 @@
         for (int i = tid + nthr; i < kVCW; i += nthr) {
             const int x = VONE ? ((const int*)&pk.vc0)[i] : ((const int*)(pk.vc + v))[i];
             ((int*)&vcv)[i] = x;
-            if (VONE && blockIdx.x == 0)
+            if (kHand && VONE && blockIdx.x == 0)
                 __hip_atomic_store((int*)pk.vc + i, i == kVcStepWord ? (int)step_ctr : x, __ATOMIC_RELAXED,
                                    __HIP_MEMORY_SCOPE_AGENT);
         }
@@ -619,9 +623,10 @@
     float* const s_stage = smem + ((HA + 3) & ~3) + 8 * kWs;
     STAMP(1);
 
-    const int hp = pk.hp;
+    const int hp = kTraj ? pk.hp : 0;
     const uint32_t plane_b = (uint32_t)K * (uint32_t)hp * 4u;
-    const __amdgpu_buffer_rsrc_t trs = traj_rsrc(pk.traj + (size_t)v * pk.C * K * hp, plane_b, pk.C);
+    const __amdgpu_buffer_rsrc_t trs = traj_rsrc(kTraj ? pk.traj + (size_t)v * pk.C * K * hp : nullptr, plane_b,
+                                                 kTraj ? pk.C : 0);
 
     float acc[NCH][NA];
 #pragma unroll
@@ -679,7 +684,7 @@
                 eps[c][a] = val ? eps[c][a] : 0.0f;
                 act[c][a] = val ? ur[a] + eps[c][a] : 0.0f;
             }
-            if (p.store_noise && val) {
+            if (!QUIET && p.store_noise && val) {
                 float* dst = p.noise_out + (((size_t)v * K + k) * H + t) * NA;
 #pragma unroll
                 for (int a = 0; a < NA; ++a) st_dev(dst + a, eps[c][a]);
@@ -798,7 +803,7 @@
             const bool term = (t == H - 1);
             float x;
             const uint32_t toff = ((uint32_t)k * (uint32_t)hp + (uint32_t)t) * 4u;
-            const bool stv = p.store_traj && kval && t < hp;
+            const bool stv = kTraj && p.store_traj && kval && t < hp;
             if (MODEL == MPPI_MODEL_DRONE) {
                 const float dx = posf[c][0] - vc.tpos[0], dy = posf[c][1] - vc.tpos[1],
                             dz = posf[c][2] - vc.tpos[2];
@@ -943,7 +948,8 @@
         float S_mine = S_seg[0];
 #pragma unroll
         for (int s = 1; s < R; ++s) S_mine = (sub == s) ? S_seg[s] : S_mine;
-        if (MPPI_S_PLAIN) { if (kval && t0 == 0) p.S[(size_t)v * K + k] = S_mine; }
+        if (!kCosts) { }
+        else if (MPPI_S_PLAIN) { if (kval && t0 == 0) p.S[(size_t)v * K + k] = S_mine; }
         else if (kval && t0 == 0) s_stage[it * cost_run_stride(nw * R) + wid * R + sub] = S_mine;
 
         float m = INFINITY;
@@ -1012,7 +1018,7 @@
     STAMPW(11);
     lds_barrier();
     STAMP(6);
-    if (!MPPI_S_PLAIN && wid == nw - 1) {
+    if (kCosts && !MPPI_S_PLAIN && wid == nw - 1) {
         const int nS = nw * R, q = (nS + 3) >> 2;
         float* const Sv = uniform_ptr(p.S + (size_t)v * K);
         for (int i = lane; i < iters * q; i += 64) {
@@ -1094,6 +1100,27 @@
 }
 
 template <int MODEL, int NA, int NCH, int LSEG, bool F64, bool VONE, bool XC, bool ONEG>
+__global__ void __launch_bounds__(512, (roll_occ<NCH, F64, XC, ONEG>())) k_rollout_ql(const uint32_t seed_lo, const uint32_t seed_hi,
+                                                 const uint32_t step_arg, const uint32_t k_off,
+                                                 const int32_t noise_arg, const int32_t H_arg,
+                                                 const int32_t geo_arg,
+                                                 const float* __restrict__ u_prev,
+                                                 const JointDev* __restrict__ jtab, const DevParams pk) {
+    rollout_body<MODEL, NA, NCH, LSEG, F64, VONE, XC, ONEG, false, true>(seed_lo, seed_hi, step_arg, k_off, noise_arg,
+                                                                         H_arg, geo_arg, u_prev, jtab, pk);
+}
+template <int MODEL, int NA, int NCH, int LSEG, bool F64, bool VONE, bool XC>
+__global__ void __launch_bounds__(512, (F64 ? 7 : roll_occ<NCH, F64, XC, true>())) k_rollout_q(const uint32_t seed_lo, const uint32_t seed_hi,
+                                                 const uint32_t step_arg, const uint32_t k_off,
+                                                 const int32_t noise_arg, const int32_t H_arg,
+                                                 const int32_t geo_arg,
+                                                 const float* __restrict__ u_prev,
+                                                 const JointDev* __restrict__ jtab, const DevParams pk) {
+    rollout_body<MODEL, NA, NCH, LSEG, F64, VONE, XC, true, true, true>(seed_lo, seed_hi, step_arg, k_off, noise_arg,
+                                                                        H_arg, geo_arg, u_prev, jtab, pk);
+}
+
+template <int MODEL, int NA, int NCH, int LSEG, bool F64, bool VONE, bool XC, bool ONEG>
 inline void rollout_symbol(char* buf, size_t n) {
     snprintf(buf, n, "_Z9k_rolloutILi%dELi%dELi%dELi%dELb%dELb%dELb%dELb%dEEvjjjjiiiPKfPKN4mppi8JointDevENS2_9DevParamsE",
              MODEL, NA, NCH, LSEG, (int)F64, (int)VONE, (int)XC, (int)ONEG);
@@ -1103,6 +1130,57 @@
 inline void rollout_s_symbol(char* buf, size_t n) {
     snprintf(buf, n, "_Z11k_rollout_sILi%dELi%dELi%dELi%dELb%dELb%dELb%dEEvjjjjiiiPKfPKN4mppi8JointDevENS2_9DevParamsE",
              MODEL, NA, NCH, LSEG, (int)F64, (int)VONE, (int)XC);
+}
+
+template <int MODEL, int NA, int NCH, int LSEG, bool F64, bool VONE, bool XC, bool ONEG>
+inline void rollout_ql_symbol(char* buf, size_t n) {
+    snprintf(buf, n, "_Z12k_rollout_qlILi%dELi%dELi%dELi%dELb%dELb%dELb%dELb%dEEvjjjjiiiPKfPKN4mppi8JointDevENS2_9DevParamsE",
+             MODEL, NA, NCH, LSEG, (int)F64, (int)VONE, (int)XC, (int)ONEG);
+}
+
+template <int MODEL, int NA, int NCH, int LSEG, bool F64, bool VONE, bool XC>
+inline void rollout_q_symbol(char* buf, size_t n) {
+    snprintf(buf, n, "_Z11k_rollout_qILi%dELi%dELi%dELi%dELb%dELb%dELb%dEEvjjjjiiiPKfPKN4mppi8JointDevENS2_9DevParamsE",
+             MODEL, NA, NCH, LSEG, (int)F64, (int)VONE, (int)XC);
+}
+
+template <int MODEL, int NCH, int LSEG, bool XC>
+constexpr bool quiet_geom() {
+    return !XC && NCH == 1 && LSEG == (MODEL == MPPI_MODEL_WHOLEBODY ? 64 : 32);
+}
+inline bool quiet_launch(const DevParams& p) {
+    return (p.kern & kRollKernQuiet) && (p.noise_mode & 0xFF) != MPPI_NOISE_INJECTED && !p.store_noise &&
+           !(p.noise_mode & kNoiseOverlap);
+}
+
+template <int MODEL, int NA, int NCH, int LSEG, bool F64, bool XC, bool ONEG>
+inline int launch_rollout_gq(const DevParams& p, int threads, hipStream_t s) {
+    const int iters = ONEG ? 1 : p.iters;
+    if (threads <= 0 || threads > 512 || iters < 1) return -1;
+    const size_t lds = (size_t)(((p.H * NA + 3) & ~3) + 8 * wave_slot_floats<NA, NCH, LSEG>()) * sizeof(float);
+    const int32_t geo = threads | (iters << 16);
+    if (p.V == 1)
+        return go(k_rollout_ql<MODEL, NA, NCH, LSEG, F64, true, XC, ONEG>,
+                  rollout_ql_symbol<MODEL, NA, NCH, LSEG, F64, true, XC, ONEG>, dim3(p.nb, p.V), dim3(threads), lds, s,
+                  p.seed_lo, p.seed_hi, p.step_ctr, (uint32_t)p.k_offset, p.noise_mode, p.H, geo, p.u_prev,
+                  p.joints, p);
+    return go(k_rollout_ql<MODEL, NA, NCH, LSEG, F64, false, XC, ONEG>,
+              rollout_ql_symbol<MODEL, NA, NCH, LSEG, F64, false, XC, ONEG>, dim3(p.nb, p.V), dim3(threads), lds, s,
+              p.seed_lo, p.seed_hi, p.step_ctr, (uint32_t)p.k_offset, p.noise_mode, p.H, geo, p.u_prev, p.joints,
+              p);
+}
+template <int MODEL, int NA, int NCH, int LSEG, bool F64, bool XC>
+inline int launch_rollout_sq(const DevParams& p, hipStream_t s) {
+    constexpr int threads = 512;
+    const size_t lds = (size_t)(((p.H * NA + 3) & ~3) + 8 * wave_slot_floats<NA, NCH, LSEG>()) * sizeof(float);
+    const int32_t geo = threads | (1 << 16);
+    if (p.V == 1)
+        return go(k_rollout_q<MODEL, NA, NCH, LSEG, F64, true, XC>, rollout_q_symbol<MODEL, NA, NCH, LSEG, F64, true, XC>,
+                  dim3(p.nb, p.V), dim3(threads), lds, s, p.seed_lo, p.seed_hi, p.step_ctr, (uint32_t)p.k_offset,
+                  p.noise_mode, p.H, geo, p.u_prev, p.joints, p);
+    return go(k_rollout_q<MODEL, NA, NCH, LSEG, F64, false, XC>, rollout_q_symbol<MODEL, NA, NCH, LSEG, F64, false, XC>,
+              dim3(p.nb, p.V), dim3(threads), lds, s, p.seed_lo, p.seed_hi, p.step_ctr, (uint32_t)p.k_offset,
+              p.noise_mode, p.H, geo, p.u_prev, p.joints, p);
 }
 
 template <int MODEL, int NA, int NCH, int LSEG, bool F64, bool XC, bool ONEG>
@@ -1141,12 +1219,21 @@
 
 template <int MODEL, int NA, int NCH, int LSEG, bool F64, bool XC>
 inline int launch_rollout_x(const DevParams& p, int threads, hipStream_t s) {
+    bool quiet = false;
+    if constexpr (quiet_geom<MODEL, NCH, LSEG, XC>()) quiet = quiet_launch(p);
     if constexpr (!XC && NCH == 1)
         if (p.iters == 1) {
-            if (threads == 512 && !p.kern && !(p.noise_mode & kNoiseOverlap) && p.H <= LSEG * NCH)
+            if (threads == 512 && !(p.kern & kRollKernGeneric) && !(p.noise_mode & kNoiseOverlap) && p.H <= LSEG * NCH) {
+                if constexpr (quiet_geom<MODEL, NCH, LSEG, XC>())
+                    if (quiet) return launch_rollout_sq<MODEL, NA, NCH, LSEG, F64, XC>(p, s);
                 return launch_rollout_s<MODEL, NA, NCH, LSEG, F64, XC>(p, s);
+            }
+            if constexpr (quiet_geom<MODEL, NCH, LSEG, XC>())
+                if (quiet) return launch_rollout_gq<MODEL, NA, NCH, LSEG, F64, XC, true>(p, threads, s);
             return launch_rollout_g<MODEL, NA, NCH, LSEG, F64, XC, true>(p, threads, s);
         }
+    if constexpr (quiet_geom<MODEL, NCH, LSEG, XC>())
+        if (quiet) return launch_rollout_gq<MODEL, NA, NCH, LSEG, F64, XC, false>(p, threads, s);
     return launch_rollout_g<MODEL, NA, NCH, LSEG, F64, XC, false>(p, threads, s);
 }
 
diff --git a/quadrotor_manipulator_mppi_amd/csrc/mppi_rollout_quad.hip b/quadrotor_manipulator_mppi_amd/csrc/mppi_rollout_quad.hip
--- a/quadrotor_manipulator_mppi_amd/csrc/mppi_rollout_quad.hip
+++ b/quadrotor_manipulator_mppi_amd/csrc/mppi_rollout_quad.hip
@@ -26,12 +26,14 @@
 }
 }
 
-template <bool VONE, bool LIT, int NWD, int NT>
-__global__ void __launch_bounds__(NT) k_rollout_quad(const uint32_t seed_lo, const uint32_t seed_hi,
-                                                            const uint32_t step_arg, const uint32_t k_off,
-                                                            const int32_t noise_arg, const int32_t H,
-                                                            const float* __restrict__ u_prev, const DevParams pk) {
+template <bool VONE, bool LIT, int NWD, int NT, bool QUIET>
+__device__ __forceinline__ void rollout_quad_body(const uint32_t seed_lo, const uint32_t seed_hi,
+                                                  const uint32_t step_arg, const uint32_t k_off,
+                                                  const int32_t noise_arg, const int32_t H,
+                                                  const float* __restrict__ u_prev, const DevParams& pk) {
     static_assert(NWD == 1 || NWD == kQWaves, "dynamics waves per block");
+    constexpr bool kTraj = !QUIET && !(MPPI_KO & 16), kCosts = !QUIET && !(MPPI_KO & 1024),
+                   kHand = !QUIET && !(MPPI_KO & 2048);
     static_assert(NT == kQThreads || (NWD == 1 && NT == kQThreadsWide), "block size");
     constexpr int QR = kQR * NWD;
     constexpr int kQPitch = QR * kQA + 1;
@@ -50,7 +52,7 @@
     float* const eps_t = qlds;
     float* const u_t = qlds + (H + 1) * kQPitch;
     const VehicleConst& vc = VONE ? pk.vc0 : pk.vc[v];
-    if (VONE && b == 0) {
+    if (kHand && VONE && b == 0) {
         constexpr int kVCW = (int)(sizeof(VehicleConst) / 4);
         for (int i = tid; i < kVCW; i += NT)
             __hip_atomic_store((int*)pk.vc + i, i == kVcStepWord ? (int)step_ctr : ((const int*)&pk.vc0)[i],
@@ -64,7 +66,7 @@
 #pragma unroll
     for (int d = 0; d < 3; ++d) { tg3[d] = uniform_f32(vc.tpos[d]); ii3[d] = p.q_iinv[d]; }
     float sdt = p.dt, sim = p.q_inv_m, skd = p.q_kd, sg = p.q_g, swsp = p.w_sp, swtp = p.w_tp, scoef = p.coef;
-    const int sstore = p.store_traj;
+    const int sstore = kTraj ? p.store_traj : 0;
     asm volatile("" : "+s"(x6[0]), "+s"(x6[1]), "+s"(x6[2]), "+s"(x6[3]), "+s"(x6[4]), "+s"(x6[5]),
                       "+s"(v6[0]), "+s"(v6[1]), "+s"(v6[2]), "+s"(v6[3]), "+s"(v6[4]), "+s"(v6[5]),
                       "+s"(tg3[0]), "+s"(tg3[1]), "+s"(tg3[2]), "+s"(ii3[0]), "+s"(ii3[1]), "+s"(ii3[2]),
@@ -96,7 +98,7 @@
         float* dst = eps_t + t * kQPitch + r * kQA;
 #pragma unroll
         for (int a = 0; a < kQA; ++a) dst[a] = eps[a];
-        if (p.store_noise && kval) {
+        if (!QUIET && p.store_noise && kval) {
             float* dst = p.noise_out + (((size_t)v * K + k) * H + t) * kQA;
 #pragma unroll
             for (int a = 0; a < kQA; ++a) st_dev(dst + a, eps[a]);
@@ -118,12 +120,13 @@
     const float ij = axis(ii3), tg = axis(tg3);
     float pj = axis(x6), ej = axis(x6 + 3), vj = axis(v6), wj = axis(v6 + 3);
     const float ox0 = v6[3], oy0 = v6[4], oz0 = v6[5];
-    const int kp = pk.hp;
+    const int kp = kTraj ? pk.hp : 0;
     const uint32_t plane_b = (uint32_t)kp * (uint32_t)H * 4u;
-    const __amdgpu_buffer_rsrc_t trs = traj_rsrc(pk.traj + (size_t)v * pk.C * kp * H, plane_b, pk.C);
+    const __amdgpu_buffer_rsrc_t trs = traj_rsrc(kTraj ? pk.traj + (size_t)v * pk.C * kp * H : nullptr, plane_b,
+                                                 kTraj ? pk.C : 0);
     const uint32_t off_p = (uint32_t)(k < kp ? k : kc) * 4u + (uint32_t)jj * plane_b, off_e = off_p + 3u * plane_b;
     const uint32_t tstep_b = (uint32_t)kp * 4u;
-    const bool store = sstore != 0;
+    const bool store = kTraj && sstore != 0;
     float stage = 0.0f, term = 0.0f;
     const float a0 = (j == 0) ? 1.0f : 0.0f;
     const float* rowp = eps_t + r * kQA;
@@ -182,7 +185,7 @@
     stage = qbc<0>(stage) + qbc<1>(stage) + qbc<2>(stage);
     term = qbc<0>(term) + qbc<1>(term) + qbc<2>(term);
     const float S = kval ? (swsp * stage) + (swtp * term) : INFINITY;
-    if (j == 0) s_lds[r] = S;
+    if (kCosts && j == 0) s_lds[r] = S;
     const bool mine = kval && j == 0, bad = S != S;
     float rho = wave_fold_all((mine && !bad) ? S : INFINITY, OpMin());
     float nanf = wave_fold_all(mine && bad ? 1.0f : 0.0f, OpMax());
@@ -196,7 +199,7 @@
     float eta = wave_fold_all(e, OpAdd()), eta2 = wave_fold_all(e * e, OpAdd());
     if (j == 0) e_lds[r] = e;
     wave_lds_handoff();
-    {
+    if constexpr (kCosts) {
         const int k0 = kb + wid * kQR, n = min(kQR, K - k0);
         if (lane < 4) st_dev_run(uniform_ptr(p.S + (size_t)v * K), (uint32_t)k0, s_lds + wid * kQR, n, lane);
     }
@@ -235,6 +238,21 @@
             wt_store(rdata_v, (((uint32_t)a * (uint32_t)p.nb + (uint32_t)b) * (uint32_t)H + (uint32_t)lane) * 4u, n[a]);
     }
     drain_stores();
+}
+
+template <bool VONE, bool LIT, int NWD, int NT>
+__global__ void __launch_bounds__(NT) k_rollout_quad(const uint32_t seed_lo, const uint32_t seed_hi,
+                                                            const uint32_t step_arg, const uint32_t k_off,
+                                                            const int32_t noise_arg, const int32_t H,
+                                                            const float* __restrict__ u_prev, const DevParams pk) {
+    rollout_quad_body<VONE, LIT, NWD, NT, false>(seed_lo, seed_hi, step_arg, k_off, noise_arg, H, u_prev, pk);
+}
+template <bool VONE, bool LIT, int NWD, int NT>
+__global__ void __launch_bounds__(NT) k_rollout_quad_q(const uint32_t seed_lo, const uint32_t seed_hi,
+                                                              const uint32_t step_arg, const uint32_t k_off,
+                                                              const int32_t noise_arg, const int32_t H,
+                                                              const float* __restrict__ u_prev, const DevParams pk) {
+    rollout_quad_body<VONE, LIT, NWD, NT, true>(seed_lo, seed_hi, step_arg, k_off, noise_arg, H, u_prev, pk);
 }
 
 extern "C" int mppi_launch_rollout_quad(const DevParams* p, int threads, void* stream) {
@@ -244,14 +262,25 @@
     const size_t lds = (size_t)((p->H + 1) * (kQR * nwd * kQA + 1) + (p->H + 1) * kQA) * sizeof(float);
     hipStream_t s = (hipStream_t)stream;
     const bool wide = nwd == 1 && (size_t)p->nb * p->V <= 512;
+    const bool quiet = quiet_launch(*p);
 #define MPPI_QUAD_GO(VO, LI, NW, NT)                                                                             \
+    do {                                                                                                         \
+    if (quiet)                                                                                                   \
+        return go(k_rollout_quad_q<VO, LI, NW, NT>,                                                              \
+                  [](char* b, size_t n) {                                                                        \
+                      snprintf(b, n, "_Z16k_rollout_quad_qILb%dELb%dELi%dELi%dEEvjjjjiiPKfN4mppi9DevParamsE",    \
+                               (int)VO, (int)LI, NW, NT);                                                        \
+                  },                                                                                             \
+                  dim3(p->nb, p->V), dim3(NT), lds, s, p->seed_lo, p->seed_hi, p->step_ctr,                      \
+                  (uint32_t)p->k_offset, p->noise_mode, p->H, p->u_prev, *p);                                    \
     return go(k_rollout_quad<VO, LI, NW, NT>,                                                                    \
               [](char* b, size_t n) {                                                                            \
                   snprintf(b, n, "_Z14k_rollout_quadILb%dELb%dELi%dELi%dEEvjjjjiiPKfN4mppi9DevParamsE", (int)VO, \
                            (int)LI, NW, NT);                                                                     \
               },                                                                                                 \
               dim3(p->nb, p->V), dim3(NT), lds, s, p->seed_lo, p->seed_hi, p->step_ctr, (uint32_t)p->k_offset,   \
-              p->noise_mode, p->H, p->u_prev, *p)
+              p->noise_mode, p->H, p->u_prev, *p);                                                               \
+    } while (0)
 #define MPPI_QUAD_NW(VO, LI)                                                                                     \
     do {                                                                                                         \
         if (wide) MPPI_QUAD_GO(VO, LI, 1, kQThreadsWide);                                                        \
diff --git a/quadrotor_manipulator_mppi_amd/csrc/mppi_step.cpp b/quadrotor_manipulator_mppi_amd/csrc/mppi_step.cpp
--- a/quadrotor_manipulator_mppi_amd/csrc/mppi_step.cpp
+++ b/quadrotor_manipulator_mppi_amd/csrc/mppi_step.cpp
@@ -39,9 +39,15 @@
 
 using namespace mppi_host;
 
-extern "C" {
-
-mppi_status mppi_rollout(mppi_engine* e, const float* d_noise) {
+static bool quiet_steps(const mppi_engine* e) {
+    return !(e->generic & 3) && !e->timing && !e->d_stamps && !e->d_fstamps && !e->out_dbg && !e->no_flag_dbg && !e->overlap;
+}
+
+static bool quiet_rollout(const mppi_engine* e) {
+    return quiet_steps(e) && !(e->generic & 8) && !e->peer && !sharded(e);
+}
+
+static mppi_status rollout_impl(mppi_engine* e, const float* d_noise, bool quiet) {
     if (!e) return fail(MPPI_ERR_INVALID_ARG, "null engine");
     if (!e->state_set) return fail(MPPI_ERR_STATE, "mppi_rollout before mppi_set_state");
     if (e->cfg.noise_mode == MPPI_NOISE_INJECTED && !d_noise)
@@ -53,6 +59,7 @@
     p.noise_in = d_noise;
     p.vc0 = e->h_vc[0];
     p.step_ctr = e->step_ctr;
+    if (quiet && quiet_rollout(e)) p.kern |= kRollKernQuiet;
     hipEvent_t e0 = nullptr, e1 = nullptr;
     if (e->timing) { e0 = pool_event(e); e1 = pool_event(e); HIP_TRY(hipEventRecord(e0, e->stream)); }
     int rc = mppi_launch_rollout(&p, e->threads, e->stream);
@@ -75,9 +82,9 @@
     return MPPI_OK;
 }
 
-static bool quiet_steps(const mppi_engine* e) {
-    return !(e->generic & 3) && !e->timing && !e->d_stamps && !e->d_fstamps && !e->out_dbg && !e->no_flag_dbg && !e->overlap;
-}
+extern "C" {
+
+mppi_status mppi_rollout(mppi_engine* e, const float* d_noise) { return rollout_impl(e, d_noise, false); }
 
 static std::string fin_symbol(const FinParams& f) {
     LaunchDesc d{};
@@ -93,9 +100,11 @@
     mppi_aql::set_capture(nullptr);
     return rc == 0 ? d.symbol : "?";
 }
-static std::string kernels_text(const std::string& roll, const std::string& fin, const std::string* quiet) {
+static std::string kernels_text(const std::string& roll, const std::string& fin, const std::string* quiet,
+                                const std::string* roll_quiet = nullptr) {
     std::string s = "rollout " + roll + ", finalize " + fin;
     if (quiet) s += ", quiet finalize " + (*quiet == fin ? std::string("none") : *quiet);
+    if (roll_quiet) s += ", quiet rollout " + (*roll_quiet == roll ? std::string("none") : *roll_quiet);
     return s;
 }
 
@@ -395,6 +404,7 @@
     LaunchDesc& roll = e->batch_roll;
     LaunchDesc& fin = e->batch_fin;
     LaunchDesc& finq = e->batch_fin_quiet;
+    LaunchDesc& rollq = e->batch_roll_quiet;
     DevParams p = e->dp;
     p.noise_in = nullptr;
     p.vc0 = e->h_vc[0];
@@ -413,6 +423,12 @@
         mppi_aql::set_capture(&roll);
         int rc = mppi_launch_rollout(&p, e->threads, e->stream);
         if (rc == 0) {
+            DevParams pq = p;
+            if (quiet_rollout(e)) pq.kern |= kRollKernQuiet;
+            mppi_aql::set_capture(&rollq);
+            rc = mppi_launch_rollout(&pq, e->threads, e->stream);
+        }
+        if (rc == 0) {
             mppi_aql::set_capture(&fin);
             rc = mppi_launch_finalize(&f, e->stream);
         }
@@ -432,7 +448,7 @@
     std::string err;
     const auto c2 = now();
     const auto guard = mppi_aql::step_guard(e->aql);
-    const int pr = mppi_aql::step_prepare(e->aql, roll, fin, finq, e->step_ctr, kRollStepOff, &err);
+    const int pr = mppi_aql::step_prepare(e->aql, roll, rollq, fin, finq, e->step_ctr, kRollStepOff, &err);
     const auto c3 = now();
     if (pr == -2) {
         e->aql_off = true;
@@ -460,8 +476,8 @@
     e->aql_call = false;
     e->aql_why.clear();
     if (e->kern_batch_state != (n > 1 ? 2 : 1)) {
-        const std::string q = n > 1 ? finq.symbol : fin.symbol;
-        e->kern_batch = kernels_text(roll.symbol, fin.symbol, &q);
+        const std::string q = n > 1 ? finq.symbol : fin.symbol, rq = n > 1 ? rollq.symbol : roll.symbol;
+        e->kern_batch = kernels_text(roll.symbol, fin.symbol, &q, &rq);
         e->kern_batch_state = n > 1 ? 2 : 1;
     }
     *used = true;
@@ -567,7 +583,7 @@
     mppi_status st = run_steps_aql(e, n, &used);
     if (st != MPPI_OK || used) return st;
     for (int i = 0; i < n; ++i) {
-        mppi_status st = mppi_rollout(e, nullptr);
+        mppi_status st = rollout_impl(e, nullptr, i < n - 1);
         if (st != MPPI_OK) return st;
         if (e->comm && (st = mppi_exchange(e)) != MPPI_OK) return st;
         if ((st = finalize_impl(e, i == n - 1, true)) != MPPI_OK) return st;
@@ -580,8 +596,10 @@
         final_records(e, f);
         const std::string full = fin_symbol(f);
         if (n > 1 && quiet_steps(e)) f.kern |= kFinKernQuiet;
-        const std::string q = fin_symbol(f);
-        e->kern_batch = kernels_text(roll_symbol(p, e->threads), full, &q);
+        const std::string q = fin_symbol(f), roll = roll_symbol(p, e->threads);
+        if (n > 1 && quiet_rollout(e)) p.kern |= kRollKernQuiet;
+        const std::string rq = roll_symbol(p, e->threads);
+        e->kern_batch = kernels_text(roll, full, &q, &rq);
         e->kern_batch_state = 0;
     }
     return MPPI_OK;
@@ -590,7 +608,7 @@
 mppi_status mppi_kernel_info(mppi_engine* e, char* buf, int32_t len) {
     if (!e || !buf || len <= 0) return fail(MPPI_ERR_INVALID_ARG, "mppi_kernel_info: bad arguments");
     snprintf(buf, (size_t)len, "batch: %s; call: %s%s", e->kern_batch.c_str(), e->kern_call.c_str(),
-             e->generic == 7 ? "; MPPI_GENERIC_KERNELS" : e->generic ? "; MPPI_GENERIC_KERNELS (in part)" : "");
+             e->generic == kGenericAll ? "; MPPI_GENERIC_KERNELS" : e->generic ? "; MPPI_GENERIC_KERNELS (in part)" : "");
     return MPPI_OK;
 }
 
@@ -621,6 +639,24 @@
     return (a == "?" || b == "?") ? MPPI_ERR_INVALID_ARG : MPPI_OK;
 }
 
+int32_t mppi_debug_rollout_kernels(const int32_t* g, char* full, char* quiet, int32_t len) {
+    if (!g || !full || !quiet || len <= 0) return MPPI_ERR_INVALID_ARG;
+    DevParams p;
+    std::memset(&p, 0, sizeof(p));
+    p.model = g[0]; p.A = g[1]; p.H = g[2]; p.L = g[3]; p.nch = g[4]; p.iters = g[5]; p.V = g[7];
+    p.R = p.L > 0 ? 64 / p.L : 0;
+    p.state_f64 = g[8]; p.noise_mode = g[9]; p.store_noise = g[10]; p.cost_terms = g[11]; p.sigma_diag = !g[12];
+    p.nb = 16; p.K = 16; p.store_traj = 1;
+    p.chain_fast = 2;
+    p.kern = g[14] ? kRollKernGeneric : 0;
+    const std::string a = roll_symbol(p, g[6]);
+    if (!g[13] && !g[14]) p.kern |= kRollKernQuiet;
+    const std::string b = roll_symbol(p, g[6]);
+    snprintf(full, (size_t)len, "%s", a.c_str());
+    snprintf(quiet, (size_t)len, "%s", b.c_str());
+    return (a == "?" || b == "?") ? MPPI_ERR_INVALID_ARG : MPPI_OK;
+}
+
 mppi_status mppi_synchronize(mppi_engine* e) {
     if (!e) return fail(MPPI_ERR_INVALID_ARG, "null engine");
     if (use_device(e)) return MPPI_ERR_HIP;
```

After: 17.21 billion, median of 6. 1.04x the previous value.
